# YannDubs/disentangling-vae

Measured on AMD Instinct MI355X. Metric: images/sec (whole node) at 64x64x3, btcvae loss, higher is better.
Workload: dtype f32; 1 GPU; btcvae_celeba (BASELINE.json configs[3]): Burgess VAE 64x64x3, btcvae loss, z=10, tensor handed to _train_iteration B=1024 global (1024 per GPU), Adam lr 0.0005, n_data=202599, fwd+loss+bwd+Adam; batch_per_gpu=1024, global_batch=1024, parallelism=dp1

## Files before the change

disentangling-vae_amd/csrc/capi.hip:

```cpp
#include <mutex>
#include <stdlib.h>
#include "common.h"
#include "last_error.h"

namespace dvae {

bool use_generic_only() {
  const char* e = getenv("DVAE_FORCE_GENERIC");
  return e && e[0] == '1';
}

static int check_layout(int l) { return l == DVAE_NCHW || l == DVAE_NHWC; }

static int run_down(const ConvArgs& a, hipStream_t s) {
  if (!use_generic_only()) {
    int r = launch_down_mfma32(a, s);
    if (r <= 0) return r;
    r = launch_down_thin(a, s);
    if (r <= 0) return r;
  }
  return launch_down_generic(a, s);
}
static int run_up(const ConvArgs& a, hipStream_t s) {
  if (!use_generic_only()) {
    int r = 1;
    static const bool no_ws = env_off("DVAE_UP_WS");
    if (!no_ws) {
      r = launch_up_mfma32_ws(a, s);
      if (r <= 0) return r;
    }
    r = launch_up_mfma32(a, s);
    if (r <= 0) return r;
    r = launch_up_thin(a, s);
    if (r <= 0) return r;
  }
  return launch_up_generic(a, s);
}
static int run_wgrad(const float* big, int big_layout, const float* small, int small_layout, float* dw, float* db,
                     int bias_from_big, int N, int Cb, int Cs, int Hs, int Ws, float* ws, hipStream_t s) {
  if (!use_generic_only() && ws != nullptr && Hs == Ws && Cs == 32 && Cb == 32 && big_layout == DVAE_NHWC && Hs == 4 &&
      small_layout == DVAE_NCHW)
    return launch_wgrad_mfma32(big, small, dw, db, bias_from_big, N, Hs, ws, s, 1);
  if (!use_generic_only() && ws != nullptr && Hs == Ws && Cs == 32 && small_layout == DVAE_NHWC) {
    if (Cb == 32 && big_layout == DVAE_NHWC && (Hs == 4 || Hs == 8 || Hs == 16))
      return launch_wgrad_mfma32(big, small, dw, db, bias_from_big, N, Hs, ws, s, 0);
    if ((Cb == 1 || Cb == 3) && Hs == 32 && big_layout == DVAE_NCHW)
      return launch_wgrad_thin(big, small, dw, db, bias_from_big, N, Cb, Hs, ws, s);
  }
  return launch_wgrad_generic(big, big_layout, small, small_layout, dw, db, bias_from_big, N, Cb, Cs, Hs, Ws, ws,
                              dvae_conv_wgrad_ws_floats(), s);
}

}

using namespace dvae;

extern "C" {

int dvae_version(void) { return DVAE_VERSION; }
const char* dvae_last_error(void) { return last_error(); }

int dvae_conv4s2_fwd(const float* x, int x_layout, const float* w, const float* b, float* y, int y_layout, int N,
                     int Cin, int H, int W, int Cout, int act, void* stream) {
  DVAE_CHECK_ARG(x && w && y && N > 0 && Cin > 0 && Cout > 0 && H > 0 && W > 0 && (H % 2 == 0) && (W % 2 == 0));
  DVAE_CHECK_ARG(check_layout(x_layout) && check_layout(y_layout));
  ConvArgs a{x, x_layout, nullptr, 0, w, b, nullptr, y, y_layout, N, Cin, Cout, H / 2, W / 2, act};
  return run_down(a, (hipStream_t)stream);
}

int dvae_conv4s2_dgrad(const float* dy, int dy_layout, const float* w, const float* x_act, float* dx, int dx_layout,
                       int N, int Cin, int H, int W, int Cout, void* stream) {
  DVAE_CHECK_ARG(dy && w && dx && N > 0 && Cin > 0 && Cout > 0 && (H % 2 == 0) && (W % 2 == 0));
  DVAE_CHECK_ARG(check_layout(dy_layout) && check_layout(dx_layout));
  ConvArgs a{nullptr, 0, dy, dy_layout, w, nullptr, x_act, dx, dx_layout, N, Cin, Cout, H / 2, W / 2, DVAE_ACT_NONE};
  return run_up(a, (hipStream_t)stream);
}

int dvae_conv4s2_wgrad(const float* x, int x_layout, const float* dy, int dy_layout, float* dw, float* db, int N,
                       int Cin, int H, int W, int Cout, float* ws, void* stream) {
  DVAE_CHECK_ARG(x && dy && dw && N > 0 && (H % 2 == 0) && (W % 2 == 0));
  const int rc = run_wgrad(x, x_layout, dy, dy_layout, dw, db, 0, N, Cin, Cout, H / 2, W / 2, ws,
                   (hipStream_t)stream);
  return rc;
}

int dvae_convT4s2_fwd(const float* x, int x_layout, const float* w, const float* b, float* y, int y_layout, int N,
                      int Cin, int H, int W, int Cout, int act, void* stream) {
  DVAE_CHECK_ARG(x && w && y && N > 0 && Cin > 0 && Cout > 0 && H > 0 && W > 0);
  DVAE_CHECK_ARG(check_layout(x_layout) && check_layout(y_layout));
  ConvArgs a{nullptr, 0, x, x_layout, w, b, nullptr, y, y_layout, N, Cout, Cin, H, W, act};
  return run_up(a, (hipStream_t)stream);
}

int dvae_convT4s2_dgrad(const float* dy, int dy_layout, const float* w, const float* x_act, float* dx, int dx_layout,
                        int N, int Cin, int H, int W, int Cout, void* stream) {
  DVAE_CHECK_ARG(dy && w && dx && N > 0 && Cin > 0 && Cout > 0);
  DVAE_CHECK_ARG(check_layout(dy_layout) && check_layout(dx_layout));
  ConvArgs a{dy, dy_layout, nullptr, 0, w, nullptr, x_act, dx, dx_layout, N, Cout, Cin, H, W, DVAE_ACT_NONE};
  return run_down(a, (hipStream_t)stream);
}

int dvae_convT4s2_wgrad(const float* x, int x_layout, const float* dy, int dy_layout, float* dw, float* db, int N,
                        int Cin, int H, int W, int Cout, float* ws, void* stream) {
  DVAE_CHECK_ARG(x && dy && dw && N > 0);
  const int rc = run_wgrad(dy, dy_layout, x, x_layout, dw, db, 1, N, Cout, Cin, H, W, ws,
                   (hipStream_t)stream);
  return rc;
}

int dvae_convT4s2_sigmoid_recon_fwd(const float* x, int x_layout, const float* w, const float* b, const float* target,
                                    float* recon, float* g, int dist, const float* coef, float* partials, int N,
                                    int Cin, int H, int W, int Cout, void* stream) {
  DVAE_CHECK_ARG(x && w && target && recon && g && coef && partials && N > 0 && Cin > 0 && Cout > 0 && H > 0 && W > 0);
  DVAE_CHECK_ARG(check_layout(x_layout));
  DVAE_CHECK_ARG(dist == DVAE_REC_BERNOULLI || dist == DVAE_REC_GAUSSIAN || dist == DVAE_REC_LAPLACE);
  ConvArgs a{nullptr, 0, x, x_layout, w, b, nullptr, recon, DVAE_NCHW, N, Cout, Cin, H, W, DVAE_ACT_SIGMOID};
  static const bool two_pass = env_on("DVAE_RECON_TWO_PASS");
  if (!use_generic_only() && !two_pass) {
    int r = launch_up_thin_recon(a, target, g, dist, coef, partials, (hipStream_t)stream);
    if (r <= 0) return r;
  }
  int r = run_up(a, (hipStream_t)stream);
  if (r) return r;
  const long n = (long)N * Cout * 4 * H * W;
  DVAE_CHECK_ARG(n % 4 == 0);
  return launch_recon_loss(recon, target, n, dist, coef, partials, g, 1, (hipStream_t)stream);
}

static bool u8_fused_shape(int C, int H, int W, int Cout) { return (C == 1 || C == 3) && H == 64 && W == 64 && Cout == 32; }

int dvae_u8_to_f32(const uint8_t* src, float* dst, long n, void* stream) {
  DVAE_CHECK_ARG(src && dst && n > 0 && (((uintptr_t)src & 15) == 0) && (((uintptr_t)dst & 15) == 0));
  return launch_u8_to_f32(src, dst, n, (hipStream_t)stream);
}

int dvae_image_grid_u8(const float* imgs, long n, int C, int H, int W, int nrow, int padding, float pad_value, int upsample,
                       uint8_t* out, void* stream) {
  DVAE_CHECK_ARG(imgs && out && n > 0 && (C == 1 || C == 3) && H > 0 && W > 0 && nrow > 0 && padding >= 0 && upsample >= 1);
  return launch_image_grid_u8(imgs, n, C, H, W, nrow, padding, pad_value, upsample, out, (hipStream_t)stream);
}

int dvae_image_grid_shape(long n, int H, int W, int nrow, int padding, int upsample, long* height, long* width) {
  DVAE_CHECK_ARG(height && width && n > 0 && H > 0 && W > 0 && nrow > 0 && padding >= 0 && upsample >= 1);
  long gh, gw;
  int xmaps, pad;
  if (image_grid_geom(n, H, W, nrow, padding, upsample, &gh, &gw, &xmaps, &pad) != 0) {
    set_error("dvae_image_grid_shape: grid of %ld images of %dx%d (nrow %d, padding %d, upsample %d) is too large", n, H, W,
              nrow, padding, upsample);
    return -1;
  }
  *height = gh;
  *width = gw;
  return 0;
}

int dvae_recon_rows_ws_floats(long n_img, int K, long row_elems, long* floats) {
  DVAE_CHECK_ARG(floats && n_img > 0 && K > 0 && row_elems > 0 && row_elems % 4 == 0);
  *floats = recon_rows_ws_floats(n_img, K, row_elems);
  return 0;
}

int dvae_recon_rows(const float* recon, const void* target, int target_u8, long n_img, int K, long row_elems, int dist,
                    float* ws, float* rec_rows, void* stream) {
  DVAE_CHECK_ARG(recon && target && rec_rows && n_img > 0 && K > 0 && row_elems > 0 && row_elems % 4 == 0);
  DVAE_CHECK_ARG(dist == DVAE_REC_BERNOULLI || dist == DVAE_REC_GAUSSIAN || dist == DVAE_REC_LAPLACE);
  DVAE_CHECK_ARG(((uintptr_t)recon & 15) == 0 && ((uintptr_t)target & (target_u8 ? 3 : 15)) == 0);
  return launch_recon_rows(recon, target, target_u8 ? 1 : 0, n_img, K, row_elems, dist, ws, rec_rows, (hipStream_t)stream);
}

int dvae_iw_loglik(const float* mu, const float* logvar, const float* z, const float* eps, const float* rec_rows, long n_img,
                   int nk, int D, int K, int first, int last, float* state, float* loglik, float* kl, void* stream) {
  DVAE_CHECK_ARG(mu && logvar && n_img > 0 && D > 0 && (state || kl));
  DVAE_CHECK_ARG(!state || (z && eps && rec_rows && nk > 0 && K >= nk && (!last || loglik)));
  return launch_iw_loglik(mu, logvar, z, eps, rec_rows, n_img, nk, D, K, first ? 1 : 0, last ? 1 : 0, state, loglik, kl,
                          (hipStream_t)stream);
}

int dvae_u8_fused_supported(int C, int H, int W) { return u8_fused_shape(C, H, W, 32) ? 1 : 0; }

int dvae_conv4s2_fwd_u8(const uint8_t* x, const float* w, const float* b, float* y, int N, int Cin, int H, int W,
                        int Cout, int act, void* stream) {
  DVAE_CHECK_ARG(x && w && y && N > 0);
  DVAE_CHECK_ARG(u8_fused_shape(Cin, H, W, Cout));
  DVAE_CHECK_ARG(act == DVAE_ACT_NONE || act == DVAE_ACT_RELU);
  return launch_down_thin_u8(x, w, b, y, nullptr, N, Cin, act, (hipStream_t)stream);
}

int dvae_conv4s2_wgrad_u8(const uint8_t* x, const float* dy, float* dw, float* db, int N, int Cin, int H, int W,
                          int Cout, float* ws, void* stream) {
  DVAE_CHECK_ARG(x && dy && dw && ws && N > 0);
  DVAE_CHECK_ARG(u8_fused_shape(Cin, H, W, Cout));
  return launch_wgrad_thin_u8(x, dy, dw, db, N, Cin, ws, (hipStream_t)stream);
}

int dvae_convT4s2_sigmoid_recon_fwd_u8(const float* x, const float* w, const float* b, const uint8_t* target,
                                       float* recon, float* g, int dist, const float* coef, float* partials, int N,
                                       int Cin, int H, int W, int Cout, void* stream) {
  DVAE_CHECK_ARG(x && w && target && recon && g && coef && partials && N > 0);
  DVAE_CHECK_ARG(Cin == 32 && u8_fused_shape(Cout, 2 * H, 2 * W, 32));
  DVAE_CHECK_ARG(dist == DVAE_REC_BERNOULLI || dist == DVAE_REC_GAUSSIAN || dist == DVAE_REC_LAPLACE);
  ConvArgs a{nullptr, 0, x, DVAE_NHWC, w, b, nullptr, recon, DVAE_NCHW, N, Cout, Cin, H, W, DVAE_ACT_SIGMOID};
  return launch_up_thin_recon_u8(a, target, g, dist, coef, partials, (hipStream_t)stream);
}

size_t dvae_conv_wgrad_ws_floats(void) {
  size_t a = wgrad32_ws_floats(), b = wgrad_thin_ws_floats();
  return a > b ? a : b;
}

int dvae_relayout(const float* src, int src_layout, float* dst, int N, int C, int H, int W, void* stream) {
  DVAE_CHECK_ARG(src && dst && check_layout(src_layout) && N > 0 && C > 0 && H > 0 && W > 0);
  return launch_relayout(src, src_layout, dst, N, C, H, W, (hipStream_t)stream);
}

int dvae_linear_fwd(const float* x, const float* w, const float* b, float* y, int M, int K, int N, int act, float* ws,
                    void* stream) {
  DVAE_CHECK_ARG(x && w && y && M > 0 && K > 0 && N > 0);
  DVAE_CHECK_ARG(act == DVAE_ACT_NONE || act == DVAE_ACT_RELU || act == DVAE_ACT_LEAKY02);
  return launch_linear_fwd(x, w, b, y, M, K, N, act, ws, dvae_conv_wgrad_ws_floats(), (hipStream_t)stream);
}

int dvae_linear_dgrad(const float* dy, const float* w, const float* x_act, int act, float* dx, int M, int K, int N,
                      float* ws, void* stream) {
  DVAE_CHECK_ARG(dy && w && dx && M > 0 && K > 0 && N > 0);
  return launch_linear_dgrad(dy, w, x_act, act, dx, M, K, N, ws, dvae_conv_wgrad_ws_floats(), (hipStream_t)stream);
}

int dvae_linear_wgrad(const float* x, const float* dy, float* dw, float* db, int M, int K, int N, float* ws,
                      void* stream) {
  DVAE_CHECK_ARG(x && dy && dw && M > 0 && K > 0 && N > 0);
  return launch_linear_wgrad(x, dy, dw, db, M, K, N, ws, dvae_conv_wgrad_ws_floats(), (hipStream_t)stream);
}

int dvae_linear_wgrad_grouped(const dvae_linear_wgrad_desc* descs, int n, void* stream) {
  DVAE_CHECK_ARG(descs && n >= 1 && n <= DVAE_FCW_MAX);
  for (int q = 0; q < n; ++q)
    DVAE_CHECK_ARG(descs[q].x && descs[q].dy && descs[q].dw && descs[q].M > 0 && descs[q].K > 0 && descs[q].N > 0);
  return launch_linear_wgrad_grouped(descs, n, (hipStream_t)stream);
}

size_t dvae_latent_entropy_ws_floats(long N, int D, int S) {
  if (N <= 0 || D <= 0 || S <= 0) return 0;
  return latent_entropy_ws_floats(N, D, S);
}

int dvae_latent_entropy(const float* z_ds, const float* mean, const float* logvar, long N, int D, int S, float* ws,
                        float* H, void* stream) {
  DVAE_CHECK_ARG(z_ds && mean && logvar && ws && H && N > 0 && D > 0 && D <= 65535 && S > 0);
  return launch_latent_entropy(z_ds, mean, logvar, N, D, S, ws, H, (hipStream_t)stream);
}

int dvae_reparam_kl_fwd(const float* ml, const float* eps, float* mu, float* logvar, float* z, float* kl_dim,
                        const float* coef, int B, int D, void* stream) {
  DVAE_CHECK_ARG(ml && mu && logvar && z && B > 0 && D > 0);
  DVAE_CHECK_ARG(D <= DVAE_MAX_D || ((!kl_dim || coef) && D <= DVAE_KL_FLOATS));
  return launch_reparam_kl_fwd(ml, eps, mu, logvar, z, kl_dim, coef, B, D, (hipStream_t)stream);
}

int dvae_reparam_kl_bwd(const float* dz, const float* dz2, const float* dz3, const float* dmu_x, const float* dlv_x,
                        const float* mu, const float* logvar, const float* eps, const float* scal, const float* coef,
                        float* dml, int B, int D, void* stream) {
  DVAE_CHECK_ARG(mu && logvar && scal && coef && dml && B > 0 && D > 0);
  return launch_reparam_kl_bwd(dz, dz2, dz3, dmu_x, dlv_x, mu, logvar, eps, scal, coef, dml, B, D, (hipStream_t)stream);
}

int dvae_kl_normal_bwd(const float* g_dim, const float* mu, const float* logvar, float* dmu, float* dlogvar, int B, int D,
                       void* stream) {
  DVAE_CHECK_ARG(g_dim && mu && logvar && dmu && dlogvar && B > 0 && D > 0);
  return launch_kl_normal_bwd(g_dim, mu, logvar, dmu, dlogvar, B, D, (hipStream_t)stream);
}

int dvae_reduce_sum(const float* src, long n, float scale, float* dst, void* stream) {
  DVAE_CHECK_ARG(src && dst && n > 0);
  return launch_reduce_sum(src, n, scale, dst, (hipStream_t)stream);
}

int dvae_recon_loss(const float* recon, const float* target, long n, int dist, const float* coef, float* partials,
                    float* g, int wrt_logit, void* stream) {
  DVAE_CHECK_ARG(recon && target && coef && partials && n > 0 && (n % 4 == 0));
  DVAE_CHECK_ARG(dist == DVAE_REC_BERNOULLI || dist == DVAE_REC_GAUSSIAN || dist == DVAE_REC_LAPLACE);
  return launch_recon_loss(recon, target, n, dist, coef, partials, g, wrt_logit, (hipStream_t)stream);
}

int dvae_sigmoid_bwd(const float* grad_y, const float* y, float* out, long n, void* stream) {
  DVAE_CHECK_ARG(grad_y && y && out && n > 0);
  return launch_sigmoid_bwd(grad_y, y, out, n, (hipStream_t)stream);
}

int dvae_btcvae_fwd(const float* z, const float* mu, const float* logvar, int Bg, int D, int row0, int Bl, int is_mss,
                    const float* log_w, float* tmp, float* rowstats, void* stream) {
  DVAE_CHECK_ARG(z && mu && logvar && tmp && rowstats && Bg > 1 && D >= 1 && row0 >= 0 && Bl > 0 && row0 + Bl <= Bg);
  DVAE_CHECK_ARG(D <= DVAE_WIDE_MAX_D );
  DVAE_CHECK_ARG(!is_mss || log_w);
  return launch_btcvae_fwd(z, mu, logvar, Bg, D, row0, Bl, is_mss, log_w, tmp, rowstats, (hipStream_t)stream);
}

int dvae_btcvae_bwd(const float* z, const float* mu, const float* logvar, const float* rowstats, int Bg, int D,
                    int row0, int Bl, int is_mss, const float* log_w, const float* coef, const float* tmp, float* dz,
                    float* dmu_all, float* dlv_all, void* stream) {
  DVAE_CHECK_ARG(z && mu && logvar && rowstats && coef && tmp && dz && dmu_all && dlv_all && Bg > 1 && D >= 1);
  DVAE_CHECK_ARG(D <= DVAE_WIDE_MAX_D );
  DVAE_CHECK_ARG(row0 >= 0 && Bl > 0 && row0 + Bl <= Bg && (!is_mss || log_w));
  return launch_btcvae_bwd(z, mu, logvar, rowstats, Bg, D, row0, Bl, is_mss, log_w, coef, tmp, dz, dmu_all, dlv_all,
                           (hipStream_t)stream);
}

int dvae_permute_dims(const float* z, const int64_t* perm, float* out, int B, int D, void* stream) {
  DVAE_CHECK_ARG(z && perm && out && B > 0 && D > 0);
  return launch_permute_dims(z, perm, out, B, D, (hipStream_t)stream);
}

int dvae_disc_losses(const float* dlogits, int Bh, const float* coef, float* sums, float* g_dtc, float* g_tc,
                     void* stream) {
  DVAE_CHECK_ARG(dlogits && coef && sums && g_dtc && Bh > 0);
  return launch_disc_losses(dlogits, Bh, coef, sums, g_dtc, g_tc, (hipStream_t)stream);
}

int dvae_loss_pack(const float* rec_partials, const float* kl_dim, int D, const float* rowstats, int Bl,
                   const float* disc_sums, float* packed, void* stream) {
  DVAE_CHECK_ARG(rec_partials && packed && D >= 0);
  return launch_loss_pack(rec_partials, kl_dim, D, rowstats, Bl, disc_sums, packed, (hipStream_t)stream);
}

int dvae_loss_epilogue(int kind, const float* rec_partials, const float* kl_dim, int kl_blocks, int D, const float* rowstats,
                       int Bl, const float* disc_sums, int Bg, const float* coef, float* packed, float* scal,
                       void* stream) {
  DVAE_CHECK_ARG(rec_partials && packed && coef && D >= 0 && Bl >= 0 && Bg > 0);
  DVAE_CHECK_ARG(kl_blocks >= 0 && kl_blocks <= DVAE_KL_MAX_BLOCKS && (D <= DVAE_MAX_D || kl_blocks == 0));
  DVAE_CHECK_ARG(kind >= DVAE_LOSS_BETAH && kind <= DVAE_LOSS_FACTOR);
  return launch_loss_epilogue(kind, rec_partials, kl_dim, kl_blocks, D, rowstats, Bl, disc_sums, Bg, coef, packed, scal,
                              (hipStream_t)stream);
}

int dvae_reparam_kl_blocks(int B) { return B > 0 ? reparam_kl_blocks(B) : 0; }

int dvae_kl_finish(float* kl_dim, int kl_blocks, const float* coef, int D, void* stream) {
  DVAE_CHECK_ARG(kl_dim && coef && kl_blocks > 0 && kl_blocks <= DVAE_KL_MAX_BLOCKS && D > 0 && D <= DVAE_MAX_D);
  return launch_kl_finish(kl_dim, kl_blocks, coef, D, (hipStream_t)stream);
}

int dvae_stage_weights(const dvae_conv_image_desc* conv, int n_conv, const dvae_fc_image_desc* fc, int n_fc,
                       const dvae_thin_image_desc* thin, float* coef, const float* coef_vals, void* stream) {
  DVAE_CHECK_ARG(n_conv >= 0 && n_conv <= DVAE_STAGE_MAX_CONV && n_fc >= 0 && n_fc <= DVAE_STAGE_MAX_FC);
  DVAE_CHECK_ARG((n_conv == 0 || conv) && (n_fc == 0 || fc));
  for (int q = 0; q < n_conv; ++q) DVAE_CHECK_ARG(conv[q].w);
  for (int q = 0; q < n_fc; ++q) DVAE_CHECK_ARG(fc[q].w && fc[q].N > 0 && fc[q].K > 0);
  if (thin) DVAE_CHECK_ARG(thin->w && (thin->C == 1 || thin->C == 3));
  return launch_stage_weights(conv, n_conv, fc, n_fc, thin, coef, coef_vals, (hipStream_t)stream);
}

int dvae_convT3_fwd_staged(const float* x, const float* img_pairs, const float* b, const void* target, int target_is_u8,
                           float* recon, float* g, int dist, const float* coef, float* partials, int N, int C,
                           void* stream) {
  DVAE_CHECK_ARG(x && img_pairs && recon && N > 0 && (C == 1 || C == 3));
  if (target) {
    DVAE_CHECK_ARG(g && coef && partials);
    DVAE_CHECK_ARG(dist == DVAE_REC_BERNOULLI || dist == DVAE_REC_GAUSSIAN || dist == DVAE_REC_LAPLACE);
  }
  return launch_up_thin_staged(x, img_pairs, b, target, target_is_u8, recon, g, dist, coef, partials, N, C, DVAE_ACT_SIGMOID,
                               (hipStream_t)stream);
}

int dvae_conv32_down(const float* big, const float* img_down, const float* bias, const float* mask, float* out,
                     int out_layout, int N, int Hs, int act, void* stream) {
  DVAE_CHECK_ARG(big && img_down && out && N > 0 && (Hs == 4 || Hs == 8 || Hs == 16) && check_layout(out_layout));
  DVAE_CHECK_ARG(out_layout == DVAE_NHWC || Hs == 4);
  DVAE_CHECK_ARG(act == DVAE_ACT_NONE || act == DVAE_ACT_RELU);
  ConvArgs a{big, DVAE_NHWC, nullptr, 0, img_down, bias, mask, out, out_layout, N, 32, 32, Hs, Hs, act, 1};
  const int r = launch_down_mfma32(a, (hipStream_t)stream);
  if (r > 0) { set_error("dvae_conv32_down: geometry not covered"); return -1; }
  return r;
}

int dvae_conv32_up(const float* small, int small_layout, const float* img_up, const float* bias, const float* mask,
                   float* out, int N, int Hs, int act, void* stream) {
  DVAE_CHECK_ARG(small && img_up && out && N > 0 && (Hs == 4 || Hs == 8 || Hs == 16) && check_layout(small_layout));
  DVAE_CHECK_ARG(small_layout == DVAE_NHWC || Hs == 4);
  DVAE_CHECK_ARG(act == DVAE_ACT_NONE || act == DVAE_ACT_RELU);
  ConvArgs a{nullptr, 0, small, small_layout, img_up, bias, mask, out, DVAE_NHWC, N, 32, 32, Hs, Hs, act, 1};
  int r = launch_up_mfma32_ws(a, (hipStream_t)stream);
  if (r > 0) r = launch_up_mfma32(a, (hipStream_t)stream);
  if (r > 0) { set_error("dvae_conv32_up: geometry not covered"); return -1; }
  return r;
}

int dvae_conv1_fwd_bits(const void* x, int x_is_u8, const float* w, const float* b, float* y, uint32_t* y_bits, int N,
                        int Cin, void* stream) {
  DVAE_CHECK_ARG(x && w && y && y_bits && N > 0 && (Cin == 1 || Cin == 3));
  if (x_is_u8) return launch_down_thin_u8((const uint8_t*)x, w, b, y, y_bits, N, Cin, DVAE_ACT_RELU, (hipStream_t)stream);
  ConvArgs a{(const float*)x, DVAE_NCHW, nullptr, 0, w, b, nullptr, y, DVAE_NHWC, N, Cin, 32, 32, 32, DVAE_ACT_RELU, 0};
  a.out_bits = y_bits;
  const int r = launch_down_thin(a, (hipStream_t)stream);
  if (r > 0) { set_error("dvae_conv1_fwd_bits: geometry not covered"); return -1; }
  return r;
}

int dvae_conv32_up_bits(const float* small, const float* img_up, const float* bias, const uint32_t* mask_bits, float* out,
                        uint32_t* out_bits, int N, int act, void* stream) {
  DVAE_CHECK_ARG(small && img_up && out && N > 0 && (mask_bits != nullptr) != (out_bits != nullptr));
  DVAE_CHECK_ARG(act == DVAE_ACT_NONE || act == DVAE_ACT_RELU);
  DVAE_CHECK_ARG(!out_bits || act == DVAE_ACT_RELU);
  ConvArgs a{nullptr, 0, small, DVAE_NHWC, img_up, bias, nullptr, out, DVAE_NHWC, N, 32, 32, 16, 16, act, 1};
  a.mask_bits = mask_bits;
  a.out_bits = out_bits;
  const int r = launch_up_mfma32_ws(a, (hipStream_t)stream);
  if (r > 0) { set_error("dvae_conv32_up_bits: geometry not covered"); return -1; }
  return r;
}

int dvae_convT3_dgrad_bits(const float* dy, const float* w, const uint32_t* x_act_bits, float* dx, int N, int Cout,
                           void* stream) {
  DVAE_CHECK_ARG(dy && w && x_act_bits && dx && N > 0 && (Cout == 1 || Cout == 3));
  ConvArgs a{dy, DVAE_NCHW, nullptr, 0, w, nullptr, nullptr, dx, DVAE_NHWC, N, Cout, 32, 32, 32, DVAE_ACT_NONE, 0};
  a.mask_bits = x_act_bits;
  const int r = launch_down_thin(a, (hipStream_t)stream);
  if (r > 0) { set_error("dvae_convT3_dgrad_bits: geometry not covered"); return -1; }
  return r;
}

int dvae_fc_chain_fwd(const dvae_fc_chain_fwd_args* a, void* stream) {
  DVAE_CHECK_ARG(a && a->a_flat && a->w_e1 && a->w_e2 && a->w_ml && a->b_e1 && a->b_e2 && a->b_ml);
  DVAE_CHECK_ARG(a->h1 && a->h2 && a->ml && a->mu && a->logvar && a->z);
  DVAE_CHECK_ARG(a->D >= 1 && a->D <= DVAE_MAX_D && a->n_enc > 0 && a->n_enc <= 8 * DVAE_KL_MAX_BLOCKS);
  DVAE_CHECK_ARG(a->n_kl >= 0 && a->n_kl <= a->n_enc && a->n_dec >= 0 && a->n_dec <= a->n_enc);
  if (a->n_dec > 0) DVAE_CHECK_ARG(a->w_d1 && a->w_d2 && a->w_d3 && a->b_d1 && a->b_d2 && a->b_d3 && a->d1 && a->d2 && a->d3);
  if (a->conv_in) DVAE_CHECK_ARG(a->conv_w && a->conv_b && ((((uintptr_t)a->conv_in | (uintptr_t)a->conv_w) & 15) == 0));
  if (a->convT_w) DVAE_CHECK_ARG(a->conv_in && a->convT_b && a->convT_out && a->n_dec > 0 && (((uintptr_t)a->convT_w & 15) == 0));
  return launch_fc_chain_fwd(a, (hipStream_t)stream);
}

int dvae_fc_chain_rows(int n) { return fc_chain_rows(n); }

int dvae_fc_chain_bwd(const dvae_fc_chain_bwd_args* a, void* stream) {
  DVAE_CHECK_ARG(a && a->gd3 && a->w_d3 && a->w_d2 && a->w_d1 && a->w_ml && a->w_e2 && a->w_e1);
  DVAE_CHECK_ARG(a->d2 && a->d1 && a->h2 && a->h1 && a->a_flat && a->mu && a->logvar && a->scal && a->coef);
  DVAE_CHECK_ARG(a->gd2 && a->gd1 && a->dml && a->gh2 && a->gh1 && a->ga_flat);
  DVAE_CHECK_ARG(a->D >= 1 && a->D <= DVAE_MAX_D && a->n > 0);
  if (a->convT_gout) DVAE_CHECK_ARG(a->convT_w && a->d3 && ((((uintptr_t)a->convT_gout | (uintptr_t)a->convT_w) & 15) == 0));
  if (a->conv_w) DVAE_CHECK_ARG(a->convT_gout && a->conv_act && a->conv_gin && (((uintptr_t)a->conv_w & 15) == 0));
  return launch_fc_chain_bwd(a, (hipStream_t)stream);
}

int dvae_loss_finalize(int kind, const float* packed, int D, int Bg, const float* coef, float* scal, void* stream) {
  DVAE_CHECK_ARG(packed && coef && scal && D >= 0 && Bg > 0);
  DVAE_CHECK_ARG(kind >= DVAE_LOSS_BETAH && kind <= DVAE_LOSS_FACTOR);
  return launch_loss_finalize(kind, packed, D, Bg, coef, scal, (hipStream_t)stream);
}

int dvae_set_coef(float* coef, float c0, float c1, float c2, float c3, float c4, float c5, float c6, float c7,
                  void* stream) {
  DVAE_CHECK_ARG(coef);
  const float v[8] = {c0, c1, c2, c3, c4, c5, c6, c7};
  return launch_set_coef(coef, v, (hipStream_t)stream);
}

int dvae_stream_create(void** stream) {
  DVAE_CHECK_ARG(stream);
  hipStream_t s = nullptr;
  if (hipStreamCreateWithFlags(&s, hipStreamNonBlocking) != hipSuccess) {
    set_error("dvae_stream_create: %s", hipGetErrorString(hipGetLastError()));
    return -2;
  }
  *stream = (void*)s;
  return 0;
}

int dvae_stream_order(void* earlier, void* later) {
  constexpr int NEV = 256, NDEV = 32;
  static hipEvent_t pool[NDEV][NEV];
  static int made[NDEV] = {}, next[NDEV] = {};
  static std::mutex mu;
  std::lock_guard<std::mutex> lock(mu);
  int d = 0;
  if (hipGetDevice(&d) != hipSuccess || d < 0 || d >= NDEV) { set_error("dvae_stream_order: no current device"); return -2; }
  if (!made[d]) {
    for (int k = 0; k < NEV; ++k)
      if (hipEventCreateWithFlags(&pool[d][k], hipEventDisableTiming | hipEventReleaseToDevice) != hipSuccess) {
        set_error("dvae_stream_order: hipEventCreateWithFlags failed");
        return -2;
      }
    made[d] = 1;
  }
  hipEvent_t ev = pool[d][next[d]];
  next[d] = (next[d] + 1) % NEV;
  if (hipEventRecord(ev, (hipStream_t)earlier) != hipSuccess || hipStreamWaitEvent((hipStream_t)later, ev, 0) != hipSuccess) {
    set_error("dvae_stream_order: %s", hipGetErrorString(hipGetLastError()));
    return -2;
  }
  return 0;
}

static hipEvent_t* event_slot(int slot, const char* who) {
  constexpr int NDEV = 32;
  static hipEvent_t pool[NDEV][DVAE_EVENT_SLOTS];
  static int made[NDEV] = {};
  static std::mutex mu;
  std::lock_guard<std::mutex> lock(mu);
  int d = 0;
  if (hipGetDevice(&d) != hipSuccess || d < 0 || d >= NDEV) { set_error("%s: no current device", who); return nullptr; }
  if (slot < 0 || slot >= DVAE_EVENT_SLOTS) { set_error("%s: slot %d outside [0, %d)", who, slot, DVAE_EVENT_SLOTS); return nullptr; }
  if (!made[d]) {
    for (int k = 0; k < DVAE_EVENT_SLOTS; ++k)
      if (hipEventCreateWithFlags(&pool[d][k], hipEventDisableTiming | hipEventReleaseToDevice) != hipSuccess) {
        set_error("%s: hipEventCreateWithFlags failed", who);
        return nullptr;
      }
    made[d] = 1;
  }
  return &pool[d][slot];
}

int dvae_event_record(int slot, void* stream) {
  hipEvent_t* ev = event_slot(slot, "dvae_event_record");
  if (!ev) return -2;
  if (hipEventRecord(*ev, (hipStream_t)stream) != hipSuccess) { set_error("dvae_event_record: %s", hipGetErrorString(hipGetLastError())); return -2; }
  return 0;
}

int dvae_event_wait(int slot, void* stream) {
  hipEvent_t* ev = event_slot(slot, "dvae_event_wait");
  if (!ev) return -2;
  if (hipStreamWaitEvent((hipStream_t)stream, *ev, 0) != hipSuccess) { set_error("dvae_event_wait: %s", hipGetErrorString(hipGetLastError())); return -2; }
  return 0;
}

int dvae_add(const float* a, const float* b, float* out, long n, void* stream) {
  DVAE_CHECK_ARG(a && b && out && n > 0);
  return launch_add(a, b, out, n, (hipStream_t)stream);
}

int dvae_adam_step(const dvae_adam_tensor* tensors, int nt, float step_new, double lr, double beta1, double beta2,
                   double eps, double weight_decay, void* stream) {
  DVAE_CHECK_ARG(tensors && nt > 0 && step_new >= 1.f && lr >= 0. && beta1 >= 0. && beta1 < 1. && beta2 >= 0. && beta2 < 1.);
  DVAE_CHECK_ARG(eps >= 0. && weight_decay >= 0.);
  for (int i = 0; i < nt; ++i) DVAE_CHECK_ARG(tensors[i].p && tensors[i].g && tensors[i].m && tensors[i].v && tensors[i].n >= 0);
  return launch_adam(tensors, nt, step_new, lr, beta1, beta2, eps, weight_decay, (hipStream_t)stream);
}

int dvae_axpby(float* out, const float* a, float alpha, const float* b, float beta, long n, void* stream) {
  DVAE_CHECK_ARG(out && a && n > 0);
  return launch_axpby(out, a, alpha, b, beta, n, (hipStream_t)stream);
}

int dvae_swap_outer(const float* src, float* dst, int A, int Bn, long inner, void* stream) {
  DVAE_CHECK_ARG(src && dst && src != dst && A > 0 && Bn > 0 && inner > 0 && inner < (1L << 31) && (long)A * Bn < (1L << 31));
  return launch_swap_outer(src, dst, A, Bn, inner, (hipStream_t)stream);
}

}
```

disentangling-vae_amd/csrc/common.h:

```cpp
#pragma once
#include <hip/hip_runtime.h>
#include <stdint.h>
#include <stdio.h>
#include <stdlib.h>
#include <string.h>
#include "../../include/dvae_hip.h"
#include "wave_spec.h"

namespace dvae {

void set_error(const char* fmt, ...);

#define DVAE_CHECK_ARG(cond)                                                            \
  do {                                                                                  \
    if (!(cond)) {                                                                      \
      dvae::set_error("%s:%d: invalid argument: %s", __FILE__, __LINE__, #cond);        \
      return -1;                                                                        \
    }                                                                                   \
  } while (0)

#define DVAE_CHECK_LAUNCH()                                                             \
  do {                                                                                  \
    hipError_t e__ = hipGetLastError();                                                 \
    if (e__ != hipSuccess) {                                                            \
      dvae::set_error("%s:%d: launch failed: %s", __FILE__, __LINE__,                   \
                      hipGetErrorString(e__));                                          \
      return -2;                                                                        \
    }                                                                                   \
  } while (0)

struct Strides {
  long n, c, h, w;
};
static inline Strides make_strides(int layout, int C, int H, int W) {
  Strides s;
  if (layout == DVAE_NHWC) {
    s.n = (long)H * W * C; s.h = (long)W * C; s.w = C; s.c = 1;
  } else {
    s.n = (long)C * H * W; s.c = (long)H * W; s.h = W; s.w = 1;
  }
  return s;
}

struct DeviceOnce {
  bool done[32] = {};
  bool first() {
    int d = 0;
    if (hipGetDevice(&d) != hipSuccess || d < 0 || d >= 32) return true;
    if (done[d]) return false;
    done[d] = true;
    return true;
  }
};

typedef float f32x4 __attribute__((ext_vector_type(4)));
typedef float f32x16 __attribute__((ext_vector_type(16)));

__device__ __forceinline__ float wave_sum(float v) {
#pragma unroll
  for (int o = 32; o > 0; o >>= 1) v += __shfl_xor(v, o, 64);
  return v;
}
__device__ __forceinline__ float wave_max(float v) {
#pragma unroll
  for (int o = 32; o > 0; o >>= 1) v = fmaxf(v, __shfl_xor(v, o, 64));
  return v;
}

__device__ __forceinline__ float recon_elem(float p, float x, int dist, float* gl, float* gr) {
  const float q1 = 1.f - p;
  const float qq = q1 * p;
  float term;
  if (dist == DVAE_REC_BERNOULLI) {
    const float lp = p < 1e-30f ? logf(p) : __logf(p);
    term = (x - 1.f) * fmaxf(__logf(q1), -100.f) - x * fmaxf(lp, -100.f);
    const float d = p - x;
    *gl = qq >= 1e-12f ? d : d * 1e12f * qq;
    *gr = d / fmaxf(qq, 1e-12f);
  } else if (dist == DVAE_REC_GAUSSIAN) {
    const float d = p * 255.f - x * 255.f;
    term = d * d / 255.f;
    *gr = 2.f * d;
    *gl = *gr * qq;
  } else {
    const float d = p - x;
    term = 3.f * fabsf(d);
    *gr = d > 0.f ? 3.f : (d < 0.f ? -3.f : 0.f);
    *gl = *gr * qq;
  }
  return term;
}

#define DVAE_SIGMOID_ZERO_BELOW (-88.72283935546875f)
__device__ __forceinline__ float sigmoid_aten(float v) {
  const float e = __expf(-fabsf(v));
  const float s = 1.f + e;
  const float r = __builtin_amdgcn_rcpf(s);
  float p = v >= 0.f ? fmaf(1.f - s, r, 1.f) : e * r;
  if (v < -87.f)
    p = v < DVAE_SIGMOID_ZERO_BELOW ? 0.f : ldexpf(__expf(v + 17.328679513998633f), -25);
  return p;
}

__device__ __forceinline__ float sigmoid_bce_logit(float v, float x, float* p_out, float* gl) {
  const float e = __expf(-fabsf(v));
  const float s = 1.f + e;
  const float r = __builtin_amdgcn_rcpf(s);
  const float q = s - 1.f;
  const bool pos = v >= 0.f, zero = v < DVAE_SIGMOID_ZERO_BELOW;
  float p = pos ? fmaf(-q, r, 1.f) : e * r;
  if (__builtin_expect(v < -87.f, 0))
    p = zero ? 0.f : ldexpf(__expf(v + 17.328679513998633f), -25);
  const float ls = fmaf(__builtin_amdgcn_logf(s), 0.69314718056f, (e - q) * r);
  const float om = 1.f - p;
  const float l1 = fminf(__builtin_amdgcn_logf(om) * -0.69314718056f, 100.f);
  const float t0 = pos ? l1 : ls;
  const float dx = pos ? ls - l1 : (zero ? 100.f : -v);
  const float qq = om * p, d = p - x;
  *gl = qq >= 1e-12f ? d : d * 1e12f * qq;
  *p_out = p;
  return fmaf(x, dx, t0);
}

struct ConvArgs {
  const float* big; int big_layout;
  const float* small; int small_layout;
  const float* w; const float* bias; const float* mask;
  float* out; int out_layout;
  int N, Cb, Cs, Hs, Ws;
  int act;
  int w_staged;
  const uint32_t* mask_bits = nullptr;
  uint32_t* out_bits = nullptr;
};
int launch_down_generic(const ConvArgs& a, hipStream_t s);
int launch_up_generic(const ConvArgs& a, hipStream_t s);
int launch_wgrad_generic(const float* big, int big_layout, const float* small, int small_layout,
                         float* dw, float* db, int bias_from_big, int N, int Cb, int Cs, int Hs, int Ws, float* ws,
                         size_t ws_floats, hipStream_t s);
int launch_down_mfma32(const ConvArgs& a, hipStream_t s);
int launch_up_mfma32(const ConvArgs& a, hipStream_t s);
int launch_down_mfma32_dma(const ConvArgs& a, hipStream_t s);
int launch_wgrad_mfma32_ws(const float* big, const float* small, float* dw, float* db, int bias_from_big, int N, int Hs,
                           float* ws, hipStream_t s);
int launch_wgrad32_reduce(const float* ws, float* dw, float* db, int bias_from_big, int nblk, hipStream_t s, int N);
int launch_up_mfma32_ws(const ConvArgs& a, hipStream_t s);
int launch_wgrad_mfma32(const float* big, const float* small, float* dw, float* db, int bias_from_big,
                        int N, int Hs, float* ws, hipStream_t s, int small_nchw = 0);
int launch_down_thin(const ConvArgs& a, hipStream_t s);
int launch_down_thin_ws(const ConvArgs& a, hipStream_t s);
int launch_up_thin(const ConvArgs& a, hipStream_t s);
int launch_up_thin_recon(const ConvArgs& a, const float* target, float* g, int dist, const float* coef,
                         float* partials, hipStream_t s);
int launch_wgrad_thin_ws(const float* big, const float* small, float* ws, int bias_from_big, int N, int Cb, int* grid_out,
                         hipStream_t s);
int launch_wgrad_thin(const float* big, const float* small, float* dw, float* db, int bias_from_big,
                      int N, int Cb, int Hs, float* ws, hipStream_t s);
int launch_down_thin_u8(const uint8_t* x, const float* w, const float* bias, float* out, uint32_t* out_bits, int N, int C, int act,
                        hipStream_t s);
int launch_up_thin_recon_u8(const ConvArgs& a, const uint8_t* target, float* g, int dist, const float* coef,
                            float* partials, hipStream_t s);
int launch_wgrad_thin_u8(const uint8_t* x, const float* small, float* dw, float* db, int N, int C, float* ws, hipStream_t s);
int launch_kl_normal_bwd(const float* g, const float* mu, const float* lv, float* dmu, float* dlv, int B, int D, hipStream_t s);
int launch_reduce_sum(const float* src, long n, float scale, float* dst, hipStream_t s);
int launch_u8_to_f32(const uint8_t* src, float* dst, long n, hipStream_t s);
int image_grid_geom(long n, int H, int W, int nrow, int padding, int upsample, long* gh, long* gw, int* xmaps, int* pad);
int launch_image_grid_u8(const float* imgs, long n, int C, int H, int W, int nrow, int padding, float pad_value, int upsample,
                         uint8_t* out, hipStream_t s);
long recon_rows_ws_floats(long n_img, int K, long row_elems);
int launch_recon_rows(const float* recon, const void* target, int target_u8, long n_img, int K, long row_elems, int dist,
                      float* ws, float* rec_rows, hipStream_t s);
int launch_iw_loglik(const float* mu, const float* logvar, const float* z, const float* eps, const float* rec_rows, long n_img,
                     int nk, int D, int K, int first, int last, float* state, float* loglik, float* kl, hipStream_t s);

size_t wgrad32_ws_floats();
size_t wgrad_thin_ws_floats();
int launch_relayout(const float* src, int src_layout, float* dst, int N, int C, int H, int W, hipStream_t s);

int launch_linear_fwd(const float* x, const float* w, const float* b, float* y, int M, int K, int N, int act, float* ws,
                      size_t ws_floats, hipStream_t s);
int launch_linear_dgrad(const float* dy, const float* w, const float* x_act, int act, float* dx, int M, int K, int N,
                        float* ws, size_t ws_floats, hipStream_t s);
int launch_linear_wgrad(const float* x, const float* dy, float* dw, float* db, int M, int K, int N, float* ws,
                        size_t ws_floats, hipStream_t s);

bool try_gdma(bool b_jfast, const float* a, long lda, const float* b, long ldb, float* c, long ldc, int M, int N, int Kc,
              const float* bias, int act, const float* mask, int mask_act, hipStream_t s);
bool try_gdma_wgrad(const float* x, const float* dy, float* dw, float* db, int M, int K, int N, hipStream_t s);

bool try_narrow_fwd(const float* x, const float* w, const float* b, float* y, int M, int K, int N, int act, hipStream_t s);
bool try_narrow_dgrad(const float* dy, const float* w, const float* x_act, int act, float* dx, int M, int K, int N,
                      hipStream_t s);

size_t latent_entropy_ws_floats(long N, int D, int S);
int launch_latent_entropy(const float* z_ds, const float* mean, const float* logvar, long N, int D, int S, float* ws,
                          float* H, hipStream_t s);
int launch_linear_wgrad_grouped(const dvae_linear_wgrad_desc* d, int n, hipStream_t s);
int fc_chain_rows(int n);
int launch_fc_chain_fwd(const dvae_fc_chain_fwd_args* a, hipStream_t s);
int launch_fc_chain_bwd(const dvae_fc_chain_bwd_args* a, hipStream_t s);
int reparam_kl_blocks(int B);
int launch_kl_finish(float* kl_dim, int kl_blocks, const float* coef, int D, hipStream_t s);
int launch_stage_weights(const dvae_conv_image_desc* conv, int n_conv, const dvae_fc_image_desc* fc, int n_fc,
                         const dvae_thin_image_desc* thin, float* coef, const float* coef_vals, hipStream_t s);
static __host__ __device__ __forceinline__ int thin_pair_source(int idx, int C, int* cb) {
  const int taps[16] = {5, 6, 9, 10, 13, 14, 1, 2, 7, 11, 4, 8, 0, 3, 12, 15};
  if (C == 3 && idx < 32) {
    const int a = idx >> 1, t = a >> 2, cls = a & 3;
    const int py = cls >> 1, px = cls & 1, ty = t >> 1, tx = t & 1;
    *cb = idx & 1;
    return (1 - py + 2 * ty) * 4 + (1 - px + 2 * tx);
  }
  *cb = C - 1;
  return taps[C == 3 ? idx - 32 : idx];
}
int launch_up_thin_mm(const float* small, const float* wimg, const float* bias, const void* target, int target_u8, float* out,
                      float* g, int dist, const float* coef, float* partials, int N, int act, hipStream_t s);
int launch_up_thin_staged(const float* small, const float* wrec, const float* bias, const void* target, int target_u8,
                          float* out, float* g, int dist, const float* coef, float* partials, int N, int C, int act,
                          hipStream_t s);

int launch_reparam_kl_fwd(const float* ml, const float* eps, float* mu, float* logvar, float* z, float* kl_dim,
                          const float* coef, int B, int D, hipStream_t s);
int launch_reparam_kl_bwd(const float* dz, const float* dz2, const float* dz3, const float* dmu_x, const float* dlv_x, const float* mu, const float* logvar,
                          const float* eps, const float* scal, const float* coef, float* dml, int B, int D,
                          hipStream_t s);
int launch_recon_loss(const float* recon, const float* target, long n, int dist, const float* coef, float* partials,
                      float* g, int wrt_logit, hipStream_t s);
int launch_sigmoid_bwd(const float* gy, const float* y, float* out, long n, hipStream_t s);
int launch_btcvae_fwd(const float* z, const float* mu, const float* lv, int Bg, int D, int row0, int Bl, int is_mss,
                      const float* log_w, float* tmp, float* rowstats, hipStream_t s);
int launch_btcvae_bwd(const float* z, const float* mu, const float* lv, const float* rowstats, int Bg, int D, int row0,
                      int Bl, int is_mss, const float* log_w, const float* coef, const float* tmp, float* dz, float* dmu,
                      float* dlv, hipStream_t s);
int launch_reparam_kl_fwd_wide(const float* ml, const float* eps, float* mu, float* logvar, float* z, float* kl_dim,
                               const float* coef, int B, int D, hipStream_t s);
int launch_btcvae_fwd_wide(const float* z, const float* mu, const float* lv, int Bg, int D, int row0, int Bl, int is_mss,
                           const float* log_w, float* tmp, float* rowstats, hipStream_t s);
int launch_btcvae_bwd_wide(const float* z, const float* mu, const float* lv, const float* rowstats, int Bg, int D, int row0,
                           int Bl, int is_mss, const float* log_w, const float* coef, const float* tmp, float* dz, float* dmu,
                           float* dlv, hipStream_t s);
int launch_permute_dims(const float* z, const int64_t* perm, float* out, int B, int D, hipStream_t s);
int launch_disc_losses(const float* lg, int Bh, const float* coef, float* sums, float* g_dtc, float* g_tc,
                       hipStream_t s);
int launch_loss_pack(const float* rec_partials, const float* kl_dim, int D, const float* rowstats, int Bl,
                     const float* disc_sums, float* packed, hipStream_t s);
int launch_loss_finalize(int kind, const float* packed, int D, int Bg, const float* coef, float* scal, hipStream_t s);
int launch_loss_epilogue(int kind, const float* rec_partials, const float* kl_dim, int kl_blocks, int D, const float* rowstats,
                         int Bl, const float* disc_sums, int Bg, const float* coef, float* packed, float* scal,
                         hipStream_t s);
int launch_set_coef(float* coef, const float* v, hipStream_t s);
int launch_adam(const dvae_adam_tensor* ts, int nt, float step_new, double lr, double beta1, double beta2, double eps,
                double weight_decay, hipStream_t s);
int launch_add(const float* a, const float* b, float* out, long n, hipStream_t s);
int launch_axpby(float* out, const float* a, float alpha, const float* b, float beta, long n, hipStream_t s);
int launch_swap_outer(const float* src, float* dst, int A, int Bn, long inner, hipStream_t s);

bool use_generic_only();

#ifdef DVAE_DEBUG_SWITCHES
static inline bool env_on(const char* name) { const char* e = getenv(name); return e && e[0] == '1' && e[1] == 0; }
static inline bool env_off(const char* name) { const char* e = getenv(name); return e && e[0] == '0' && e[1] == 0; }
static inline int env_int(const char* name, int dflt) { const char* e = getenv(name); return e ? atoi(e) : dflt; }
#else
static inline constexpr bool env_on(const char*) { return false; }
static inline constexpr bool env_off(const char*) { return false; }
static inline constexpr int env_int(const char*, int dflt) { return dflt; }
#endif

}

#include "latent_math.h"
```

disentangling-vae_amd/csrc/conv_mfma.hip:

```cpp
#include <stdlib.h>
#include "common.h"
#include "conv_mfma_common.h"
#include "wgrad_reduce.h"

namespace dvae {

typedef float f32x4v __attribute__((ext_vector_type(4)));

#define SEL4(v, g, j) ((g) == 0 ? (v)[j] : (g) == 1 ? (v)[4 + (j)] : (g) == 2 ? (v)[8 + (j)] : (v)[12 + (j)])
template <int HS, bool MASK>
__global__ __launch_bounds__(512) void k_down32(const float* __restrict__ big, const float* __restrict__ w,
                                                const float* __restrict__ bias, const float* __restrict__ mask,
                                                float* __restrict__ out, int N, int act, int n_units,
                                                int out_nchw, int w_staged) {
  using G = Geo<HS>;
  extern __shared__ __attribute__((aligned(16))) float smem[];
  float* wl = smem;
  float* bt = smem + 16384;
  float* red = bt + G::BIG_FLOATS;
  const int tid = threadIdx.x, lane = tid & 63, wv = tid >> 6;
  const int mt = wv & 1, kh = wv >> 1;
  const int i = lane & 31, h = lane >> 5;
  const int p = mt * 32 + i;
  const int img_l = p / (G::R * HS), sy_l = (p / HS) % G::R, sx = p % HS;
  const int r = 2 * sy_l + kh;

  SlotDesc<G::BIG_NPF> sd;
  init_big_slots<HS>(sd, tid);
  f32x4 pf[G::BIG_NPF];
  int unit = blockIdx.x;
  if (unit < n_units) load_big<HS>(pf, sd, big, unit, N);
  if (w_staged) copy_weight_image(w, wl, tid);
  else stage_weights<true>(w, wl, tid);
  const float bv = bias ? bias[i] : 0.f;
  const long npix = (long)N * HS * HS;

  for (; unit < n_units; unit += gridDim.x) {
    store_big<HS>(pf, sd, bt);
    __syncthreads();
    if (unit + (int)gridDim.x < n_units) load_big<HS>(pf, sd, big, unit + gridDim.x, N);

    f32x16 acc;
#pragma unroll
    for (int e = 0; e < 16; ++e) acc[e] = 0.f;
#pragma unroll
    for (int kw = 0; kw < 4; ++kw) {
      const int par = kw & 1, cw = sx + (kw >> 1);
      const float* arow = bt + (((img_l * G::BROWS + r) * 2 + par) * G::CW + cw) * 32;
      const int sw = swz_big<HS>(r, cw);
      const float* brow = wl + ((kh * 4 + kw) * 8) * 128 + i * 4;
#pragma unroll
      for (int q = 0; q < 4; ++q) {
        const int chunk = 2 * q + h;
        f32x4 a = *reinterpret_cast<const f32x4*>(arow + ((chunk ^ sw) << 2));
        f32x4 b = *reinterpret_cast<const f32x4*>(brow + chunk * 128);
        MFMA4(acc, a, b)
      }
    }
#pragma unroll
    for (int e = 0; e < 16; ++e) red[(((mt * 4 + (e >> 2)) * 4 + kh) * 4 + (e & 3)) * 64 + lane] = acc[e];
    __syncthreads();
    const long P0 = (long)unit * G::U + mt * 32 + 8 * kh + 4 * h;
    auto oidx = [&](long pix) -> long {
      constexpr int PP = HS * HS;
      return out_nchw ? ((pix / PP) * 32 + i) * PP + (pix % PP) : pix * 32 + i;
    };
    float vals[4], mv[4];
#pragma unroll
    for (int j = 0; j < 4; ++j) {
      float v = SEL4(acc, kh, j);
#pragma unroll
      for (int s = 0; s < 4; ++s)
        if (s != kh) v += red[(((mt * 4 + kh) * 4 + s) * 4 + j) * 64 + lane];
      vals[j] = v;
    }
    const bool full = P0 - 4 * h - 8 * kh - mt * 32 + G::U <= npix;
    if (full) {
      if (MASK) {
#pragma unroll
        for (int j = 0; j < 4; ++j) mv[j] = mask[oidx(P0 + j)];
      }
#pragma unroll
      for (int j = 0; j < 4; ++j) {
        float v = epilogue_act(vals[j] + bv, act);
        if (MASK) v = mv[j] > 0.f ? v : 0.f;
        out[oidx(P0 + j)] = v;
      }
    } else {
#pragma unroll
      for (int j = 0; j < 4; ++j) {
        const long pix = P0 + j;
        if (pix < npix) {
          float v = epilogue_act(vals[j] + bv, act);
          if (MASK) v = mask[oidx(pix)] > 0.f ? v : 0.f;
          out[oidx(pix)] = v;
        }
      }
    }
  }
}


template <int HS>
__device__ __forceinline__ void up_offsets(long (&offs)[16], int unit, int mt, int py, int px, int h, int i) {
  using G = Geo<HS>;
  const long P0 = (long)unit * G::U;
  const int n0 = (int)(P0 / (HS * HS));
  const int sy0 = (int)(P0 % (HS * HS)) / HS;
#pragma unroll
  for (int e = 0; e < 16; ++e) {
    const int rowp = (e & 3) + 8 * (e >> 2) + 4 * h;
    const int pp = mt * 32 + rowp;
    const int im = pp / (G::R * HS), mm = (pp / HS) % G::R, ll = pp % HS;
    const int by = 2 * (sy0 + mm) + py, bx = 2 * ll + px;
    offs[e] = (((long)(n0 + im) * G::HB + by) * G::HB + bx) * 32 + i;
  }
}

template <int HS>
__device__ __forceinline__ void up_store(const float (&vals)[16], float* __restrict__ out, int unit, int N, int mt,
                                         int py, int px, int h, int i) {
  using G = Geo<HS>;
  long offs[16];
  up_offsets<HS>(offs, unit, mt, py, px, h, i);
  const int n0 = (int)(((long)unit * G::U) / (HS * HS));
  if (n0 + G::IMGS <= N) {
#pragma unroll
    for (int e = 0; e < 16; ++e) out[offs[e]] = vals[e];
  } else {
#pragma unroll
    for (int e = 0; e < 16; ++e) {
      const int im = (mt * 32 + (e & 3) + 8 * (e >> 2) + 4 * h) / (G::R * HS);
      if (n0 + im < N) out[offs[e]] = vals[e];
    }
  }
}

template <int HS, bool MASK>
__global__ __launch_bounds__(512) void k_up32(const float* __restrict__ small, const float* __restrict__ w,
                                              const float* __restrict__ bias, const float* __restrict__ mask,
                                              float* __restrict__ out, int N, int act, int n_units,
                                              int small_nchw, int w_staged) {
  using G = Geo<HS>;
  extern __shared__ __attribute__((aligned(16))) float smem[];
  float* wl = smem;
  float* st = smem + 16384;
  const int tid = threadIdx.x, lane = tid & 63, wv = tid >> 6;
  const int cls = wv & 3, mt = wv >> 2;
  const int py = cls >> 1, px = cls & 1;
  const int i = lane & 31, h = lane >> 5;
  const int p = mt * 32 + i;
  const int img_l = p / (G::R * HS), m = (p / HS) % G::R, l = p % HS;

  SlotDesc<G::SH_NPF> sd;
  init_small_slots<HS>(sd, tid, small_nchw);
  f32x4 pf[G::SH_NPF];
  int unit = blockIdx.x;
  if (unit < n_units) load_small_halo<HS>(pf, sd, small, unit, N, small_nchw);
  if (w_staged) copy_weight_image(w, wl, tid);
  else stage_weights<false>(w, wl, tid);
  const float bv = bias ? bias[i] : 0.f;
  float vals[16];
  int prev_unit = -1;

  for (; unit < n_units; unit += gridDim.x) {
    __syncthreads();
    store_small_halo<HS>(pf, sd, st);
    __syncthreads();
    if (unit + (int)gridDim.x < n_units) load_small_halo<HS>(pf, sd, small, unit + gridDim.x, N, small_nchw);
    float mv[16];
    if (MASK) {
      long offs[16];
      up_offsets<HS>(offs, unit, mt, py, px, h, i);
      const int n0 = (int)(((long)unit * G::U) / (HS * HS));
#pragma unroll
      for (int e = 0; e < 16; ++e) {
        const int im = (mt * 32 + (e & 3) + 8 * (e >> 2) + 4 * h) / (G::R * HS);
        mv[e] = (G::IMGS == 1 || n0 + im < N) ? mask[offs[e]] : 0.f;
      }
    }
    if (prev_unit >= 0) up_store<HS>(vals, out, prev_unit, N, mt, py, px, h, i);

    f32x16 accs[4];
#pragma unroll
    for (int c = 0; c < 4; ++c)
#pragma unroll
      for (int e = 0; e < 16; ++e) accs[c][e] = 0.f;
    f32x4 Av[2], Bv[2];
    auto rd = [&](int g, int slot) {
      const int ty = g >> 3, tx = (g >> 2) & 1, q = g & 3;
      const int kh = 1 - py + 2 * ty, kw = 1 - px + 2 * tx;
      const int row = m + (py - ty) + 1, col = l + (px - tx) + 1;
      const float* arow = st + ((img_l * G::SROWS + row) * G::SCOLS + col) * 32;
      const int sw = swz_small<HS>(row, col);
      const float* brow = wl + ((kh * 4 + kw) * 8) * 128 + i * 4;
      const int chunk = 2 * q + h;
      Av[slot] = *reinterpret_cast<const f32x4*>(arow + ((chunk ^ sw) << 2));
      Bv[slot] = *reinterpret_cast<const f32x4*>(brow + chunk * 128);
    };
    rd(0, 0);
    __builtin_amdgcn_sched_group_barrier(0x100, 2, 0);
#pragma unroll
    for (int g = 0; g < 16; ++g) {
      const int cur = g & 1;
      if (g + 1 < 16) rd(g + 1, cur ^ 1);
#pragma unroll
      for (int j = 0; j < 4; ++j) accs[j] = __builtin_amdgcn_mfma_f32_32x32x2f32(Av[cur][j], Bv[cur][j], accs[j], 0, 0, 0);
      __builtin_amdgcn_sched_group_barrier(0x100, 2, 0);
      __builtin_amdgcn_sched_group_barrier(0x008, 4, 0);
    }
    const f32x16 acc = (accs[0] + accs[1]) + (accs[2] + accs[3]);
#pragma unroll
    for (int e = 0; e < 16; ++e) {
      float v = epilogue_act(acc[e] + bv, act);
      if (MASK) v = mv[e] > 0.f ? v : 0.f;
      vals[e] = v;
    }
    prev_unit = unit;
  }
  if (prev_unit >= 0) up_store<HS>(vals, out, prev_unit, N, mt, py, px, h, i);
}

template <int HS>
__global__ __launch_bounds__(512) void k_wgrad32(const float* __restrict__ big, const float* __restrict__ small,
                                                 float* __restrict__ ws, int N, int n_units, int small_nchw) {
  using G = Geo<HS>;
  extern __shared__ __attribute__((aligned(16))) float smem[];
  float* bt = smem;
  float* sp = smem + G::BIG_FLOATS;
  const int tid = threadIdx.x, lane = tid & 63, wv = tid >> 6;
  const int kh = wv >> 1, kwb = wv & 1;
  const int i = lane & 31, h = lane >> 5;

  SlotDesc<G::BIG_NPF> sd;
  init_big_slots<HS>(sd, tid);
  f32x4 pf[G::BIG_NPF];
  f32x4 pfs;
  f32x16 acc0, acc1, acc2, acc3;
#pragma unroll
  for (int e = 0; e < 16; ++e) { acc0[e] = 0.f; acc1[e] = 0.f; acc2[e] = 0.f; acc3[e] = 0.f; }
  float sumS = 0.f, sumB0 = 0.f, sumB1 = 0.f;

  int unit = blockIdx.x;
  const long npix = (long)N * HS * HS;
  auto load_sp = [&](int u) {
    long e0 = (long)u * G::U * 32 + tid * 4;
    f32x4 v = {0.f, 0.f, 0.f, 0.f};
    if (e0 < npix * 32) {
      if (small_nchw) {
        const long pg = e0 >> 5;
        const float* src = small + ((pg / (HS * HS)) * 32 + (e0 & 31)) * (HS * HS) + pg % (HS * HS);
#pragma unroll
        for (int u2 = 0; u2 < 4; ++u2) v[u2] = src[u2 * HS * HS];
      } else {
        v = *reinterpret_cast<const f32x4*>(small + e0);
      }
    }
    pfs = v;
  };
  if (unit < n_units) { load_big<HS>(pf, sd, big, unit, N); load_sp(unit); }

  for (; unit < n_units; unit += gridDim.x) {
    __syncthreads();
    store_big<HS>(pf, sd, bt);
    *reinterpret_cast<f32x4*>(sp + tid * 4) = pfs;
    __syncthreads();
    if (unit + (int)gridDim.x < n_units) { load_big<HS>(pf, sd, big, unit + gridDim.x, N); load_sp(unit + gridDim.x); }

    float av[2][2], b0v[2][2], b1v[2][2];
    auto rd = [&](int g, int slot) {
#pragma unroll
      for (int u = 0; u < 2; ++u) {
        const int p = 2 * (2 * g + u) + h;
        const int img_l = p / (G::R * HS), sy_l = (p / HS) % G::R, sx = p % HS;
        av[slot][u] = sp[p * 32 + i];
        const int r = 2 * sy_l + kh;
        const int cw = sx + kwb;
        const float* b0p = bt + (((img_l * G::BROWS + r) * 2 + 0) * G::CW + cw) * 32;
        const int sw = swz_big<HS>(r, cw);
        const int off = (((i >> 2) ^ sw) << 2) + (i & 3);
        b0v[slot][u] = b0p[off];
        b1v[slot][u] = b0p[G::CW * 32 + off];
      }
    };
    rd(0, 0);
    __builtin_amdgcn_sched_group_barrier(0x100, 6, 0);
#pragma unroll
    for (int g = 0; g < 16; ++g) {
      const int cur = g & 1;
      if (g + 1 < 16) rd(g + 1, cur ^ 1);
      acc0 = __builtin_amdgcn_mfma_f32_32x32x2f32(av[cur][0], b0v[cur][0], acc0, 0, 0, 0);
      acc1 = __builtin_amdgcn_mfma_f32_32x32x2f32(av[cur][0], b1v[cur][0], acc1, 0, 0, 0);
      acc2 = __builtin_amdgcn_mfma_f32_32x32x2f32(av[cur][1], b0v[cur][1], acc2, 0, 0, 0);
      acc3 = __builtin_amdgcn_mfma_f32_32x32x2f32(av[cur][1], b1v[cur][1], acc3, 0, 0, 0);
      sumS += av[cur][0] + av[cur][1]; sumB0 += b0v[cur][0] + b0v[cur][1]; sumB1 += b1v[cur][0] + b1v[cur][1];
      __builtin_amdgcn_sched_group_barrier(0x100, 6, 0);
      __builtin_amdgcn_sched_group_barrier(0x008, 4, 0);
    }
  }
  acc0 += acc2; acc1 += acc3;
  float* wsw = ws + (long)blockIdx.x * WG_STRIDE;
  const int tap0 = kh * 4 + 2 * kwb;
#pragma unroll
  for (int e = 0; e < 16; ++e) {
    const int cs = (e & 3) + 8 * (e >> 2) + 4 * h;
    wsw[(tap0 * 32 + cs) * 32 + i] = acc0[e];
    wsw[((tap0 + 1) * 32 + cs) * 32 + i] = acc1[e];
  }
  float* wsb = wsw + 16384;
  sumS += __shfl_xor(sumS, 32, 64);
  sumB0 += __shfl_xor(sumB0, 32, 64);
  sumB1 += __shfl_xor(sumB1, 32, 64);
  if (h == 0) {
    if (wv == 0) wsb[i] = sumS;
    if (wv == 2) wsb[32 + i] = sumB1;
    if (wv == 3) wsb[64 + i] = sumB0;
    if (wv == 4) wsb[96 + i] = sumB1;
    if (wv == 5) wsb[128 + i] = sumB0;
  }
}

template <bool LEAN>
__global__ __launch_bounds__(256) void k_wgrad32_reduce(const float* __restrict__ ws, float* __restrict__ dw,
                                                        float* __restrict__ db, int bias_from_big, int nblk) {
  wgrad32_reduce_body<LEAN>(blockIdx.x, ws, dw, db, bias_from_big, nblk);
}

size_t wgrad32_ws_floats() { return (size_t)WG_MAX_BLOCKS * WG_STRIDE; }

int launch_wgrad32_reduce(const float* ws, float* dw, float* db, int bias_from_big, int nblk, hipStream_t s, int N) {
  if (N >= WGR_LEAN_MIN_IMAGES)
    hipLaunchKernelGGL(k_wgrad32_reduce<true>, dim3(WG_REDUCE_BLOCKS), dim3(256), 0, s, ws, dw, db, bias_from_big, nblk);
  else
    hipLaunchKernelGGL(k_wgrad32_reduce<false>, dim3(WG_REDUCE_BLOCKS), dim3(256), 0, s, ws, dw, db, bias_from_big, nblk);
  DVAE_CHECK_LAUNCH();
  return 0;
}

static int units_for(int N, int HS) { return (int)(((long)N * HS * HS + 63) / 64); }

template <int HS>
static int launch_down_t(const ConvArgs& a, hipStream_t s) {
  using G = Geo<HS>;
  const int n_units = units_for(a.N, HS);
  const int grid = n_units < 256 ? n_units : 256;
  const size_t lds = (16384 + G::BIG_FLOATS + 8192) * sizeof(float);
  static DeviceOnce attr;
  if (attr.first()) {
    (void)hipFuncSetAttribute((const void*)k_down32<HS, false>, hipFuncAttributeMaxDynamicSharedMemorySize, (int)lds);
    (void)hipFuncSetAttribute((const void*)k_down32<HS, true>, hipFuncAttributeMaxDynamicSharedMemorySize, (int)lds);
  }
  const int out_nchw = a.out_layout == DVAE_NCHW;
  if (a.mask) hipLaunchKernelGGL((k_down32<HS, true>), dim3(grid), dim3(512), lds, s, a.big, a.w, a.bias, a.mask, a.out, a.N, a.act, n_units, out_nchw, a.w_staged);
  else hipLaunchKernelGGL((k_down32<HS, false>), dim3(grid), dim3(512), lds, s, a.big, a.w, a.bias, a.mask, a.out, a.N, a.act, n_units, out_nchw, a.w_staged);
  DVAE_CHECK_LAUNCH();
  return 0;
}

template <int HS>
static int launch_up_t(const ConvArgs& a, hipStream_t s) {
  using G = Geo<HS>;
  const int n_units = units_for(a.N, HS);
  const int grid = n_units < 256 ? n_units : 256;
  const size_t lds = (16384 + G::SH_FLOATS) * sizeof(float);
  static DeviceOnce attr;
  if (attr.first()) {
    (void)hipFuncSetAttribute((const void*)k_up32<HS, false>, hipFuncAttributeMaxDynamicSharedMemorySize, (int)lds);
    (void)hipFuncSetAttribute((const void*)k_up32<HS, true>, hipFuncAttributeMaxDynamicSharedMemorySize, (int)lds);
  }
  const int small_nchw = a.small_layout == DVAE_NCHW;
  if (a.mask) hipLaunchKernelGGL((k_up32<HS, true>), dim3(grid), dim3(512), lds, s, a.small, a.w, a.bias, a.mask, a.out, a.N, a.act, n_units, small_nchw, a.w_staged);
  else hipLaunchKernelGGL((k_up32<HS, false>), dim3(grid), dim3(512), lds, s, a.small, a.w, a.bias, a.mask, a.out, a.N, a.act, n_units, small_nchw, a.w_staged);
  DVAE_CHECK_LAUNCH();
  return 0;
}

template <int HS>
static int launch_wgrad_t(const float* big, const float* small, float* dw, float* db, int bias_from_big, int N,
                          float* ws, hipStream_t s, int small_nchw) {
  using G = Geo<HS>;
  const int n_units = units_for(N, HS);
  int grid = n_units < WG_MAX_BLOCKS ? n_units : WG_MAX_BLOCKS;
  {
    static const int cap = env_int("DVAE_WGRAD_GRID", WG_MAX_BLOCKS);
    if (cap > 0 && cap < grid) grid = cap;
  }
  const size_t lds = (G::BIG_FLOATS + 64 * 32) * sizeof(float);
  static DeviceOnce attr;
  if (attr.first()) { (void)hipFuncSetAttribute((const void*)k_wgrad32<HS>, hipFuncAttributeMaxDynamicSharedMemorySize, (int)lds); }
  hipLaunchKernelGGL(k_wgrad32<HS>, dim3(grid), dim3(512), lds, s, big, small, ws, N, n_units, small_nchw);
  DVAE_CHECK_LAUNCH();
  return launch_wgrad32_reduce(ws, dw, db, bias_from_big, grid, s, N);
}

static bool mfma32_applicable(int Cb, int Cs, int Hs, int Ws, int l0, int l1, int l2) {
  return Cb == 32 && Cs == 32 && Hs == Ws && (Hs == 4 || Hs == 8 || Hs == 16) && l0 == DVAE_NHWC &&
         l1 == DVAE_NHWC && l2 == DVAE_NHWC;
}

int launch_down_mfma32(const ConvArgs& a, hipStream_t s) {
  const int out_l = (a.Hs == 4 && a.out_layout == DVAE_NCHW) ? DVAE_NHWC : a.out_layout;
  if (!mfma32_applicable(a.Cb, a.Cs, a.Hs, a.Ws, a.big_layout, out_l, DVAE_NHWC)) return 1;
  if (a.act != DVAE_ACT_NONE && a.act != DVAE_ACT_RELU) return 1;
  if (a.Hs == 16 || a.Hs == 8) return launch_down_mfma32_dma(a, s);
  return launch_down_t<4>(a, s);
}

int launch_up_mfma32(const ConvArgs& a, hipStream_t s) {
  const int small_l = (a.Hs == 4 && a.small_layout == DVAE_NCHW) ? DVAE_NHWC : a.small_layout;
  if (!mfma32_applicable(a.Cb, a.Cs, a.Hs, a.Ws, small_l, a.out_layout, DVAE_NHWC)) return 1;
  if (a.act != DVAE_ACT_NONE && a.act != DVAE_ACT_RELU) return 1;
  switch (a.Hs) {
    case 16: return launch_up_t<16>(a, s);
    case 8: return launch_up_t<8>(a, s);
    default: return launch_up_t<4>(a, s);
  }
}

int launch_wgrad_mfma32(const float* big, const float* small, float* dw, float* db, int bias_from_big, int N,
                        int Hs, float* ws, hipStream_t s, int small_nchw) {
  static const bool no_ws = env_off("DVAE_WGRAD_WS");
  if (!no_ws && !small_nchw && (Hs == 16 || Hs == 8))
    return launch_wgrad_mfma32_ws(big, small, dw, db, bias_from_big, N, Hs, ws, s);
  switch (Hs) {
    case 16: return launch_wgrad_t<16>(big, small, dw, db, bias_from_big, N, ws, s, small_nchw);
    case 8: return launch_wgrad_t<8>(big, small, dw, db, bias_from_big, N, ws, s, small_nchw);
    case 4: return launch_wgrad_t<4>(big, small, dw, db, bias_from_big, N, ws, s, small_nchw);
    default: return 1;
  }
}

}
```

disentangling-vae_amd/csrc/conv_thin.hip:

```cpp
#include <stdlib.h>
#include "recon_epilogue.h"
#include "wgrad_reduce.h"

namespace dvae {

#define TB_ROWS 10
#define TB_PAR 34
#define TB_ROW 68
#define TB_PLANE (TB_ROWS * TB_ROW + 16)

template <int C, typename TB = float>
struct BigThinRegs {
  TB v[(C * TB_ROWS + 3) / 4];
  unsigned ok;
};

struct UnitLut {
  float t[256];
  __device__ __forceinline__ void init(int tid, int nthr) {
    for (int k = tid; k < 256; k += nthr) t[k] = (float)k / 255.0f;
  }
};
__device__ __forceinline__ float to_unit(float v, const UnitLut*) { return v; }
__device__ __forceinline__ float to_unit(uint8_t v, const UnitLut* lut) { return lut->t[v]; }

template <int C, typename TB>
__device__ __forceinline__ void load_big_thin(BigThinRegs<C, TB>& r, const TB* __restrict__ big, int n, int sy0,
                                              bool valid, int tid) {
  const int tx = tid & 63, ty = tid >> 6;
  unsigned okm = 0;
#pragma unroll
  for (int k = 0; k < (C * TB_ROWS + 3) / 4; ++k) {
    const int pr = ty + 4 * k;
    const int cb = pr / TB_ROWS, rr = pr - cb * TB_ROWS;
    const int by = 2 * sy0 - 1 + rr;
    const bool ok = valid && pr < C * TB_ROWS && by >= 0 && by < 64;
    const long off = ok ? ((((long)n * C + cb) * 64 + by) * 64 + tx) : 0;
    r.v[k] = big[off];
    okm |= ok ? (1u << k) : 0u;
  }
  r.ok = okm;
}

template <int C, typename TB>
__device__ __forceinline__ void store_big_thin(const BigThinRegs<C, TB>& r, float* bt, int tid, const UnitLut* lut) {
  const int tx = tid & 63, ty = tid >> 6;
  const int pc = tx + 1;
  const int dst_col = (pc & 1) * TB_PAR + (pc >> 1);
#pragma unroll
  for (int k = 0; k < (C * TB_ROWS + 3) / 4; ++k) {
    const int pr = ty + 4 * k;
    if (pr < C * TB_ROWS) {
      const int cb = pr / TB_ROWS, rr = pr - cb * TB_ROWS;
      bt[cb * TB_PLANE + rr * TB_ROW + dst_col] = ((r.ok >> k) & 1u) ? to_unit(r.v[k], lut) : 0.f;
    }
  }
  if (tid < C * TB_ROWS * 2) {
    const int pr = tid >> 1, side = tid & 1;
    const int cb = pr / TB_ROWS, rr = pr - cb * TB_ROWS;
    bt[cb * TB_PLANE + rr * TB_ROW + (side ? (TB_PAR + 32) : 0)] = 0.f;
  }
}

template <int C, int MODE, typename TB = float>
__global__ __launch_bounds__(256, (MODE == 1 && C == 3) ? 3 : 4) void k_down_thin(const TB* __restrict__ big, const float* __restrict__ w,
                                                   const float* __restrict__ bias, const float* __restrict__ mask,
                                                   float* __restrict__ out, int N, int act, int n_units,
                                                   uint32_t* __restrict__ bits) {
  constexpr bool MASK = MODE == 1;
  __shared__ float bt[C * TB_PLANE];
  __shared__ float wT[16 * C * 32];
  __shared__ UnitLut lut_s[1];
  const UnitLut* lut = lut_s;
  const int tid = threadIdx.x, lane = tid & 63, wv = tid >> 6;
  const int i = lane & 31, h = lane >> 5;
  if (sizeof(TB) == 1) { lut_s[0].init(tid, 256); __syncthreads(); }
  {
    float wv[2 * C];
#pragma unroll
    for (int r = 0; r < 2 * C; ++r) wv[r] = w[tid + r * 256];
#pragma unroll
    for (int r = 0; r < 2 * C; ++r) {
      const int e = tid + r * 256;
      const int cs = e / (16 * C), k = e - cs * (16 * C);
      wT[k * 32 + cs] = wv[r];
    }
  }
  BigThinRegs<C, TB> pfa, pfb;
  int unit = blockIdx.x;
  const int gstep = gridDim.x;
  if (unit < n_units) load_big_thin<C, TB>(pfa, big, unit >> 3, (unit & 7) * 4, true, tid);
  if (unit + gstep < n_units) load_big_thin<C, TB>(pfb, big, (unit + gstep) >> 3, ((unit + gstep) & 7) * 4, true, tid);
  __syncthreads();
  float wreg[8 * C];
#pragma unroll
  for (int kk = 0; kk < 8 * C; ++kk) wreg[kk] = wT[(2 * kk + h) * 32 + i];
  const float bv = bias ? bias[i] : 0.f;
  const int sy_l = wv;

  auto body = [&](BigThinRegs<C, TB>& pf, int u) {
    const int n = u >> 3, sy0 = (u & 7) * 4;
    __syncthreads();
    store_big_thin<C, TB>(pf, bt, tid, lut);
    __syncthreads();
    const int nu = u + 2 * gstep;
    if (nu < n_units) load_big_thin<C, TB>(pf, big, nu >> 3, (nu & 7) * 4, true, tid);
    const long rowbase = ((((long)n * 32 + sy0 + sy_l) * 32)) * 32 + i;
    float mv[16];
    if (MASK) {
#pragma unroll
      for (int e = 0; e < 16; ++e) mv[e] = mask[rowbase + ((e & 3) + 8 * (e >> 2) + 4 * h) * 32];
    }
    const long pixbase = ((long)n * 32 + sy0 + sy_l) * 32;
    uint32_t word = 0;
    if (MODE == 2) word = bits[pixbase + i];
    f32x16 acc;
#pragma unroll
    for (int e = 0; e < 16; ++e) acc[e] = 0.f;
#pragma unroll
    for (int kk = 0; kk < 8 * C; ++kk) {
      const int kwb = (kk & 1);
      const int kh = (kk >> 1) & 3, cb = kk >> 3;
      const float a = bt[cb * TB_PLANE + (2 * sy_l + kh) * TB_ROW + h * TB_PAR + i + kwb];
      acc = __builtin_amdgcn_mfma_f32_32x32x2f32(a, wreg[kk], acc, 0, 0, 0);
    }
#pragma unroll
    for (int e = 0; e < 16; ++e) {
      const int sx0 = (e & 3) + 8 * (e >> 2);
      const int sx = sx0 + 4 * h;
      float v = acc[e] + bv;
      if (act == DVAE_ACT_RELU) v = v > 0.f ? v : 0.f;
      if (MASK) v = mv[e] > 0.f ? v : 0.f;
      if (MODE == 2) {
        const unsigned long long m = ((unsigned long long)(uint32_t)__builtin_amdgcn_readlane(word, sx0 + 4) << 32) |
                                     (uint32_t)__builtin_amdgcn_readlane(word, sx0);
        v = __builtin_amdgcn_inverse_ballot_w64(m) ? v : 0.f;
      }
      if (MODE == 3) {
        const unsigned long long b = __builtin_amdgcn_ballot_w64(v > 0.f);
        word = __builtin_amdgcn_inverse_ballot_w64(0x0000000100000001ull << sx0) ? (uint32_t)b : word;
        word = __builtin_amdgcn_inverse_ballot_w64(0x0000000100000001ull << (sx0 + 4)) ? (uint32_t)(b >> 32) : word;
      }
      out[rowbase + sx * 32] = v;
    }
    if (MODE == 3 && h == 0) bits[pixbase + i] = word;
  };
  while (unit < n_units) {
    body(pfa, unit);
    unit += gstep;
    if (unit >= n_units) break;
    body(pfb, unit);
    unit += gstep;
  }
}

#define UT_ROWS 6
#define UT_COLS 34
template <int C, bool FUSE, typename TT = float>
__global__ __launch_bounds__(128) void k_up_thin(const float* __restrict__ small, const float* __restrict__ w,
                                                 const float* __restrict__ bias, float* __restrict__ out, int N,
                                                 int act, int n_units, const TT* __restrict__ target,
                                                 float* __restrict__ g, int dist, const float* __restrict__ coef,
                                                 float* __restrict__ partials) {
  __shared__ __attribute__((aligned(16))) float st[UT_ROWS * UT_COLS * 32];
  __shared__ float redl[2];
  const int tid = threadIdx.x;
  const int m = tid >> 5, l = tid & 31;
  const float gs = FUSE ? coef[DVAE_C_INV_B] : 0.f;
  float lsum = 0.f;
  const bool xmap = (gridDim.x & 63) == 0;
  const int upi = xmap ? 8 * (int)(gridDim.x >> 3) : (int)gridDim.x;
  const int unit0 = xmap ? 8 * (int)((blockIdx.x & 7) + 8 * (blockIdx.x >> 6)) + (int)((blockIdx.x >> 3) & 7) : (int)blockIdx.x;
  for (int unit = unit0; unit < n_units; unit += upi) {
    const int n = unit >> 3, sy0 = (unit & 7) * 4;
    __syncthreads();
    {
      const int chunk = tid & 7, cg = tid >> 3;
      f32x4 tv[UT_ROWS * 3];
#pragma unroll
      for (int row = 0; row < UT_ROWS; ++row) {
        const int sy = sy0 - 1 + row;
#pragma unroll
        for (int cp = 0; cp < 3; ++cp) {
          const int col = cp * 16 + cg;
          const int sx = col - 1;
          const bool ok = n < N && col < UT_COLS && sy >= 0 && sy < 32 && sx >= 0 && sx < 32;
          const long off = ok ? (((((long)n * 32 + sy) * 32) + sx) * 32 + chunk * 4) : 0;
          f32x4 v = *reinterpret_cast<const f32x4*>(small + off);
          if (!ok) v = f32x4{0.f, 0.f, 0.f, 0.f};
          tv[row * 3 + cp] = v;
        }
      }
#pragma unroll
      for (int row = 0; row < UT_ROWS; ++row)
#pragma unroll
        for (int cp = 0; cp < 3; ++cp) {
          const int col = cp * 16 + cg;
          if (col < UT_COLS)
            *reinterpret_cast<f32x4*>(st + (row * UT_COLS + col) * 32 + ((chunk ^ ((col >> 1) & 7)) << 2)) = tv[row * 3 + cp];
        }
    }
    __syncthreads();
    float acc[4][C];
#pragma unroll
    for (int c = 0; c < 4; ++c)
#pragma unroll
      for (int cb = 0; cb < C; ++cb) acc[c][cb] = 0.f;

#pragma unroll 1
    for (int q = 0; q < 8; ++q) {
      f32x4 x[3][3];
#pragma unroll
      for (int dy = 0; dy < 3; ++dy)
#pragma unroll
        for (int dx = 0; dx < 3; ++dx) {
          const int row = m + dy, col = l + dx;
          x[dy][dx] = *reinterpret_cast<const f32x4*>(st + (row * UT_COLS + col) * 32 + ((q ^ ((col >> 1) & 7)) << 2));
        }
#pragma unroll
      for (int j = 0; j < 4; ++j) {
        const int cs = q * 4 + j;
#pragma unroll
        for (int cb = 0; cb < C; ++cb) {
          const float* wp = w + (cs * C + cb) * 16;
#pragma unroll
          for (int kh = 0; kh < 4; ++kh) {
            const int py = (kh + 1) & 1;
            const int dsy = (py + 1 - kh) / 2;
#pragma unroll
            for (int kw = 0; kw < 4; ++kw) {
              const int px = (kw + 1) & 1;
              const int dsx = (px + 1 - kw) / 2;
              acc[py * 2 + px][cb] = fmaf(x[dsy + 1][dsx + 1][j], wp[kh * 4 + kw], acc[py * 2 + px][cb]);
            }
          }
        }
      }
    }
    if (n < N) {
      const int sy = sy0 + m;
#pragma unroll
      for (int cb = 0; cb < C; ++cb) {
        const float bv = bias ? bias[cb] : 0.f;
#pragma unroll
        for (int py = 0; py < 2; ++py) {
          float v0 = acc[py * 2 + 0][cb] + bv, v1 = acc[py * 2 + 1][cb] + bv;
          if (act == DVAE_ACT_SIGMOID) { v0 = 1.f / (1.f + expf(-v0)); v1 = 1.f / (1.f + expf(-v1)); }
          else if (act == DVAE_ACT_RELU) { v0 = v0 > 0.f ? v0 : 0.f; v1 = v1 > 0.f ? v1 : 0.f; }
          const long o = ((((long)n * C + cb) * 64) + 2 * sy + py) * 64 + 2 * l;
          *reinterpret_cast<float2*>(out + o) = make_float2(v0, v1);
          if (FUSE) {
            float xt0, xt1;
            if constexpr (sizeof(TT) == 4) {
              const float2 xt = *reinterpret_cast<const float2*>(target + o);
              xt0 = xt.x; xt1 = xt.y;
            } else {
              const uchar2 xt = *reinterpret_cast<const uchar2*>(target + o);
              xt0 = to_unit(xt.x); xt1 = to_unit(xt.y);
            }
            float gl0, gl1, gr;
            lsum += recon_elem(v0, xt0, dist, &gl0, &gr);
            lsum += recon_elem(v1, xt1, dist, &gl1, &gr);
            *reinterpret_cast<float2*>(g + o) = make_float2(gs * gl0, gs * gl1);
          }
        }
      }
    }
  }
  if (FUSE) {
    const float v = wave_sum(lsum);
    if ((tid & 63) == 0) redl[tid >> 6] = v;
    __syncthreads();
    if (tid == 0) partials[blockIdx.x] = redl[0] + redl[1];
    for (int k = gridDim.x + blockIdx.x * 128 + tid; k < DVAE_REC_NPART; k += gridDim.x * 128) partials[k] = 0.f;
  }
}


typedef float f32x2 __attribute__((ext_vector_type(2)));

__device__ __forceinline__ float sigmoid_hw(float v) { return sigmoid_aten(v); }

template <int C, bool FUSE, typename TT = float>
__global__ __launch_bounds__(128) void k_up_thin_pk(const float* __restrict__ small, const float* __restrict__ wrec,
                                                    const float* __restrict__ bias, float* __restrict__ out, int N,
                                                    int act, int n_units, const TT* __restrict__ target,
                                                    float* __restrict__ g, int dist, const float* __restrict__ coef,
                                                    float* __restrict__ partials) {
  constexpr int REC = C == 3 ? 48 : 16;
  constexpr int PB = C == 3 ? 32 : 0;
  constexpr int CS = C - 1;
  __shared__ __attribute__((aligned(16))) float st[UT_ROWS * UT_COLS * 32];
  __shared__ float redl[2];
  const int tid = threadIdx.x;
  const int m = tid >> 5, l = tid & 31;
  const float gs = FUSE ? coef[DVAE_C_INV_B] : 0.f;
  const bool bce_logit = FUSE && dist == DVAE_REC_BERNOULLI && act == DVAE_ACT_SIGMOID;
  float lsum = 0.f;
  const bool xmap = (gridDim.x & 63) == 0;
  const int upi = xmap ? 8 * (int)(gridDim.x >> 3) : (int)gridDim.x;
  const int unit0 = xmap ? 8 * (int)((blockIdx.x & 7) + 8 * (blockIdx.x >> 6)) + (int)((blockIdx.x >> 3) & 7) : (int)blockIdx.x;
  for (int unit = unit0; unit < n_units; unit += upi) {
    const int n = unit >> 3, sy0 = (unit & 7) * 4;
    __syncthreads();
    {
      const int chunk = tid & 7, cg = tid >> 3;
      f32x4 tv[UT_ROWS * 3];
#pragma unroll
      for (int row = 0; row < UT_ROWS; ++row) {
        const int sy = sy0 - 1 + row;
#pragma unroll
        for (int cp = 0; cp < 3; ++cp) {
          const int col = cp * 16 + cg;
          const int sx = col - 1;
          const bool ok = n < N && col < UT_COLS && sy >= 0 && sy < 32 && sx >= 0 && sx < 32;
          const long off = ok ? (((((long)n * 32 + sy) * 32) + sx) * 32 + chunk * 4) : 0;
          f32x4 v = *reinterpret_cast<const f32x4*>(small + off);
          if (!ok) v = f32x4{0.f, 0.f, 0.f, 0.f};
          tv[row * 3 + cp] = v;
        }
      }
#pragma unroll
      for (int row = 0; row < UT_ROWS; ++row)
#pragma unroll
        for (int cp = 0; cp < 3; ++cp) {
          const int col = cp * 16 + cg;
          if (col < UT_COLS)
            *reinterpret_cast<f32x4*>(st + (row * UT_COLS + col) * 32 + ((chunk ^ ((col >> 1) & 7)) << 2)) = tv[row * 3 + cp];
        }
    }
    __syncthreads();
    float2 tg[C][2];
    if (FUSE && n < N) {
#pragma unroll
      for (int cb = 0; cb < C; ++cb)
#pragma unroll
        for (int py = 0; py < 2; ++py) {
          const long o = ((((long)n * C + cb) * 64) + 2 * (sy0 + m) + py) * 64 + 2 * l;
          if constexpr (sizeof(TT) == 4) tg[cb][py] = *reinterpret_cast<const float2*>(target + o);
          else {
            const uchar2 xt = *reinterpret_cast<const uchar2*>(target + o);
            tg[cb][py] = make_float2((float)xt.x, (float)xt.y);
          }
        }
    }
    f32x2 accA[4];
    f32x2 h01 = {0.f, 0.f}, h23 = {0.f, 0.f};
    f32x2 v02 = {0.f, 0.f}, v13 = {0.f, 0.f};
    float sc[4] = {0.f, 0.f, 0.f, 0.f};
#pragma unroll
    for (int c = 0; c < 4; ++c) accA[c] = f32x2{0.f, 0.f};

#pragma unroll 1
    for (int q = 0; q < 8; ++q) {
      f32x4 x[3][3];
#pragma unroll
      for (int dy = 0; dy < 3; ++dy)
#pragma unroll
        for (int dx = 0; dx < 3; ++dx) {
          const int row = m + dy, col = l + dx;
          x[dy][dx] = *reinterpret_cast<const f32x4*>(st + (row * UT_COLS + col) * 32 + ((q ^ ((col >> 1) & 7)) << 2));
        }
#pragma unroll
      for (int j = 0; j < 4; ++j) {
        const float* wp = wrec + (q * 4 + j) * REC;
        const f32x2* wp2 = reinterpret_cast<const f32x2*>(wp);
        if (C == 3) {
#pragma unroll
          for (int t = 0; t < 4; ++t) {
            const int ty = t >> 1, tx = t & 1;
#pragma unroll
            for (int cls = 0; cls < 4; ++cls) {
              const int py = cls >> 1, px = cls & 1;
              const float xs = x[py - ty + 1][px - tx + 1][j];
              accA[cls] = __builtin_elementwise_fma(f32x2{xs, xs}, wp2[t * 4 + cls], accA[cls]);
            }
          }
        }
        const f32x2* wb2 = reinterpret_cast<const f32x2*>(wp + PB);
        const float xc = x[1][1][j], xu = x[0][1][j], xd = x[2][1][j], xl = x[1][0][j], xr = x[1][2][j];
        h01 = __builtin_elementwise_fma(f32x2{xc, xc}, wb2[0], h01);
        h23 = __builtin_elementwise_fma(f32x2{xc, xc}, wb2[1], h23);
        h01 = __builtin_elementwise_fma(f32x2{xu, xu}, wb2[2], h01);
        h23 = __builtin_elementwise_fma(f32x2{xd, xd}, wb2[3], h23);
        v02 = __builtin_elementwise_fma(f32x2{xl, xl}, wb2[4], v02);
        v13 = __builtin_elementwise_fma(f32x2{xr, xr}, wb2[5], v13);
        sc[3] = fmaf(x[2][2][j], wp[PB + 12], sc[3]);
        sc[2] = fmaf(x[2][0][j], wp[PB + 13], sc[2]);
        sc[1] = fmaf(x[0][2][j], wp[PB + 14], sc[1]);
        sc[0] = fmaf(x[0][0][j], wp[PB + 15], sc[0]);
      }
    }
    float acc[4][C];
    {
      const float hh[4] = {h01[0], h01[1], h23[0], h23[1]}, vv[4] = {v02[0], v13[0], v02[1], v13[1]};
#pragma unroll
      for (int cls = 0; cls < 4; ++cls) {
        if (C == 3) { acc[cls][0] = accA[cls][0]; acc[cls][1] = accA[cls][1]; }
        acc[cls][CS] = (hh[cls] + vv[cls]) + sc[cls];
      }
    }
    if (n < N) {
      const int sy = sy0 + m;
#pragma unroll
      for (int cb = 0; cb < C; ++cb) {
        const float bv = bias ? bias[cb] : 0.f;
#pragma unroll
        for (int py = 0; py < 2; ++py) {
          float v0 = acc[py * 2 + 0][cb] + bv, v1 = acc[py * 2 + 1][cb] + bv;
          const long o = ((((long)n * C + cb) * 64) + 2 * sy + py) * 64 + 2 * l;
          if (FUSE && bce_logit) {
            const float xt0 = raw_to_unit<TT>(tg[cb][py].x), xt1 = raw_to_unit<TT>(tg[cb][py].y);
            float p0, p1, gl0, gl1;
            lsum += sigmoid_bce_logit(v0, xt0, &p0, &gl0);
            lsum += sigmoid_bce_logit(v1, xt1, &p1, &gl1);
            *reinterpret_cast<float2*>(out + o) = make_float2(p0, p1);
            *reinterpret_cast<float2*>(g + o) = make_float2(gs * gl0, gs * gl1);
            continue;
          }
          if (act == DVAE_ACT_SIGMOID) { v0 = sigmoid_hw(v0); v1 = sigmoid_hw(v1); }
          else if (act == DVAE_ACT_RELU) { v0 = v0 > 0.f ? v0 : 0.f; v1 = v1 > 0.f ? v1 : 0.f; }
          *reinterpret_cast<float2*>(out + o) = make_float2(v0, v1);
          if (FUSE) {
            const float xt0 = raw_to_unit<TT>(tg[cb][py].x), xt1 = raw_to_unit<TT>(tg[cb][py].y);
            float gl0, gl1, gr;
            lsum += recon_elem(v0, xt0, dist, &gl0, &gr);
            lsum += recon_elem(v1, xt1, dist, &gl1, &gr);
            *reinterpret_cast<float2*>(g + o) = make_float2(gs * gl0, gs * gl1);
          }
        }
      }
    }
  }
  if (FUSE) {
    const float v = wave_sum(lsum);
    if ((tid & 63) == 0) redl[tid >> 6] = v;
    __syncthreads();
    if (tid == 0) partials[blockIdx.x] = redl[0] + redl[1];
    for (int k = gridDim.x + blockIdx.x * 128 + tid; k < DVAE_REC_NPART; k += gridDim.x * 128) partials[k] = 0.f;
  }
}

int launch_up_thin_staged(const float* small, const float* wrec, const float* bias, const void* target, int target_u8,
                          float* out, float* g, int dist, const float* coef, float* partials, int N, int C, int act,
                          hipStream_t s) {
  if (C != 1 && C != 3) return 1;
  if (C == 3 && launch_up_thin_mm(small, wrec + 32 * 48, bias, target, target_u8, out, g, dist, coef, partials, N, act, s) == 0)
    return 0;
  const int n_units = N * 8;
  const int grid = n_units < 1536 ? n_units : 1536;
#define UP_PK(CC, FF, TT_) hipLaunchKernelGGL((k_up_thin_pk<CC, FF, TT_>), dim3(grid), dim3(128), 0, s, small, wrec, bias, out, N, act, \
                                             n_units, (const TT_*)target, g, dist, coef, partials)
  if (!target) { if (C == 1) UP_PK(1, false, float); else UP_PK(3, false, float); }
  else if (target_u8) { if (C == 1) UP_PK(1, true, uint8_t); else UP_PK(3, true, uint8_t); }
  else { if (C == 1) UP_PK(1, true, float); else UP_PK(3, true, float); }
#undef UP_PK
  DVAE_CHECK_LAUNCH();
  return 0;
}


template <int C, typename TB = float>
__global__ __launch_bounds__(256) void k_wgrad_thin(const TB* __restrict__ big, const float* __restrict__ small,
                                                    float* __restrict__ ws, int N, int n_units) {
  constexpr int NT = (16 * C + 31) / 32;
  __shared__ __attribute__((aligned(16))) float bt[C * TB_PLANE];
  __shared__ __attribute__((aligned(16))) float sp[8192];
  __shared__ UnitLut lut_s[1];
  const UnitLut* lut = lut_s;
  const int tid = threadIdx.x, lane = tid & 63, wv = tid >> 6;
  const int i = lane & 31, h = lane >> 5;
  if (sizeof(TB) == 1) { lut_s[0].init(tid, 256); __syncthreads(); }
  f32x16 acc[NT];
#pragma unroll
  for (int t = 0; t < NT; ++t)
#pragma unroll
    for (int e = 0; e < 16; ++e) acc[t][e] = 0.f;
  float sumS = 0.f, sumB[NT];
  int boff[NT];
  bool bval[NT];
#pragma unroll
  for (int t = 0; t < NT; ++t) {
    sumB[t] = 0.f;
    const int nidx = t * 32 + i;
    bval[t] = nidx < 16 * C;
    const int cb = bval[t] ? (nidx >> 4) : 0, kh = (nidx >> 2) & 3, kw = nidx & 3;
    boff[t] = cb * TB_PLANE + kh * TB_ROW + (kw & 1) * TB_PAR + (kw >> 1);
  }
  BigThinRegs<C, TB> pfb;
  f32x4 pfs[4];
  auto load_unit = [&](int u) {
    const int n = u >> 3, sy0 = (u & 7) * 4;
    load_big_thin<C, TB>(pfb, big, n, sy0, true, tid);
    const float* src = small + ((((long)n * 32 + sy0) * 32)) * 32;
#pragma unroll
    for (int k = 0; k < 4; ++k) pfs[k] = *reinterpret_cast<const f32x4*>(src + (tid + k * 256) * 4);
  };
  int unit = blockIdx.x;
  if (unit < n_units) load_unit(unit);
  for (; unit < n_units; unit += gridDim.x) {
    __syncthreads();
    store_big_thin<C, TB>(pfb, bt, tid, lut);
#pragma unroll
    for (int k = 0; k < 4; ++k) *reinterpret_cast<f32x4*>(sp + (tid + k * 256) * 4) = pfs[k];
    __syncthreads();
    if (unit + (int)gridDim.x < n_units) load_unit(unit + gridDim.x);
#pragma unroll 4
    for (int t = 0; t < 16; ++t) {
      const int sx = 2 * t + h;
      const float a = sp[(wv * 32 + sx) * 32 + i];
      sumS += a;
      const int base = (2 * wv) * TB_ROW + sx;
#pragma unroll
      for (int nt = 0; nt < NT; ++nt) {
        float b = bt[base + boff[nt]];
        b = bval[nt] ? b : 0.f;
        sumB[nt] += b;
        acc[nt] = __builtin_amdgcn_mfma_f32_32x32x2f32(a, b, acc[nt], 0, 0, 0);
      }
    }
  }
  __syncthreads();
  float* red = sp;
#pragma unroll
  for (int nt = 0; nt < NT; ++nt)
#pragma unroll
    for (int e = 0; e < 16; ++e) red[((wv * NT + nt) * 16 + e) * 64 + lane] = acc[nt][e];
  __syncthreads();
  float* wsw = ws + (long)blockIdx.x * (NT * 1024 + 32 + NT * 32);
  for (int idx = tid; idx < NT * 1024; idx += 256) {
    const int nt = idx >> 10, e = (idx >> 6) & 15, ln = idx & 63;
    float v = red[((0 * NT + nt) * 16 + e) * 64 + ln] + red[((1 * NT + nt) * 16 + e) * 64 + ln] +
              red[((2 * NT + nt) * 16 + e) * 64 + ln] + red[((3 * NT + nt) * 16 + e) * 64 + ln];
    const int cs = (e & 3) + 8 * (e >> 2) + 4 * (ln >> 5);
    const int nidx = nt * 32 + (ln & 31);
    wsw[nt * 1024 + cs * 32 + (ln & 31)] = v;
    (void)nidx;
  }
  __syncthreads();
  sumS += __shfl_xor(sumS, 32, 64);
#pragma unroll
  for (int nt = 0; nt < NT; ++nt) sumB[nt] += __shfl_xor(sumB[nt], 32, 64);
  float* redb = sp;
  if (h == 0) {
    redb[(wv * (1 + NT)) * 32 + i] = sumS;
#pragma unroll
    for (int nt = 0; nt < NT; ++nt) redb[(wv * (1 + NT) + 1 + nt) * 32 + i] = sumB[nt];
  }
  __syncthreads();
  if (tid < (1 + NT) * 32) {
    float v = redb[tid] + redb[(1 + NT) * 32 + tid] + redb[2 * (1 + NT) * 32 + tid] + redb[3 * (1 + NT) * 32 + tid];
    wsw[NT * 1024 + tid] = v;
  }
}

template <int C>
__global__ __launch_bounds__(256) void k_wgrad_thin_reduce(const float* __restrict__ ws, float* __restrict__ dw,
                                                           float* __restrict__ db, int bias_from_big, int nblk) {
  wgrad_thin_reduce_body<C>(blockIdx.x, ws, dw, db, bias_from_big, nblk);
}

size_t wgrad_thin_ws_floats() { return (size_t)WT_MAX_BLOCKS * (2 * 1024 + 32 + 2 * 32); }

static bool thin_applicable(const ConvArgs& a) {
  return (a.Cb == 1 || a.Cb == 3) && a.Cs == 32 && a.Hs == 32 && a.Ws == 32;
}

int launch_down_thin(const ConvArgs& a, hipStream_t s) {
  if (!thin_applicable(a) || a.big_layout != DVAE_NCHW || a.out_layout != DVAE_NHWC) return 1;
  if (a.act != DVAE_ACT_NONE && a.act != DVAE_ACT_RELU) return 1;
  if (launch_down_thin_ws(a, s) == 0) return 0;
  const int n_units = a.N * 8;
  const int grid = n_units < 1536 ? n_units : 1536;
  if ((a.mask_bits && (a.mask || a.out_bits)) || (a.out_bits && a.mask)) return 1;
  uint32_t* bits = a.mask_bits ? const_cast<uint32_t*>(a.mask_bits) : a.out_bits;
#define DVAE_DT(C, MODE) hipLaunchKernelGGL((k_down_thin<C, MODE>), dim3(grid), dim3(256), 0, s, a.big, a.w, a.bias, a.mask, a.out, a.N, a.act, n_units, bits)
  if (a.Cb == 1) {
    if (a.mask_bits) DVAE_DT(1, 2); else if (a.out_bits) DVAE_DT(1, 3); else if (a.mask) DVAE_DT(1, 1); else DVAE_DT(1, 0);
  } else {
    if (a.mask_bits) DVAE_DT(3, 2); else if (a.out_bits) DVAE_DT(3, 3); else if (a.mask) DVAE_DT(3, 1); else DVAE_DT(3, 0);
  }
#undef DVAE_DT
  DVAE_CHECK_LAUNCH();
  return 0;
}

int launch_up_thin(const ConvArgs& a, hipStream_t s) {
  if (!thin_applicable(a) || a.small_layout != DVAE_NHWC || a.out_layout != DVAE_NCHW || a.mask) return 1;
  const int n_units = a.N * 8;
  const int grid = n_units;
  if (a.Cb == 1) hipLaunchKernelGGL((k_up_thin<1, false>), dim3(grid), dim3(128), 0, s, a.small, a.w, a.bias, a.out, a.N, a.act, n_units, (const float*)nullptr, (float*)nullptr, 0, (const float*)nullptr, (float*)nullptr);
  else hipLaunchKernelGGL((k_up_thin<3, false>), dim3(grid), dim3(128), 0, s, a.small, a.w, a.bias, a.out, a.N, a.act, n_units, (const float*)nullptr, (float*)nullptr, 0, (const float*)nullptr, (float*)nullptr);
  DVAE_CHECK_LAUNCH();
  return 0;
}

int launch_up_thin_recon(const ConvArgs& a, const float* target, float* g, int dist, const float* coef,
                         float* partials, hipStream_t s) {
  if (!thin_applicable(a) || a.small_layout != DVAE_NHWC || a.out_layout != DVAE_NCHW || a.mask) return 1;
  const int n_units = a.N * 8;
  const int grid = n_units < 1536 ? n_units : 1536;
  if (a.Cb == 1) hipLaunchKernelGGL((k_up_thin<1, true>), dim3(grid), dim3(128), 0, s, a.small, a.w, a.bias, a.out, a.N, DVAE_ACT_SIGMOID, n_units, target, g, dist, coef, partials);
  else hipLaunchKernelGGL((k_up_thin<3, true>), dim3(grid), dim3(128), 0, s, a.small, a.w, a.bias, a.out, a.N, DVAE_ACT_SIGMOID, n_units, target, g, dist, coef, partials);
  DVAE_CHECK_LAUNCH();
  return 0;
}

int launch_down_thin_u8(const uint8_t* x, const float* w, const float* bias, float* out, uint32_t* out_bits, int N, int C, int act,
                        hipStream_t s) {
  const int n_units = N * 8;
  const int grid = n_units < 1536 ? n_units : 1536;
#define DVAE_DT8(C, MODE) hipLaunchKernelGGL((k_down_thin<C, MODE, uint8_t>), dim3(grid), dim3(256), 0, s, x, w, bias, (const float*)nullptr, out, N, act, n_units, out_bits)
  if (C == 1) { if (out_bits) DVAE_DT8(1, 3); else DVAE_DT8(1, 0); }
  else if (C == 3) { if (out_bits) DVAE_DT8(3, 3); else DVAE_DT8(3, 0); }
  else return 1;
#undef DVAE_DT8
  DVAE_CHECK_LAUNCH();
  return 0;
}

int launch_up_thin_recon_u8(const ConvArgs& a, const uint8_t* target, float* g, int dist, const float* coef,
                            float* partials, hipStream_t s) {
  if (!thin_applicable(a) || a.small_layout != DVAE_NHWC || a.out_layout != DVAE_NCHW || a.mask) return 1;
  const int n_units = a.N * 8;
  const int grid = n_units < 1536 ? n_units : 1536;
  if (a.Cb == 1) hipLaunchKernelGGL((k_up_thin<1, true, uint8_t>), dim3(grid), dim3(128), 0, s, a.small, a.w, a.bias, a.out, a.N, DVAE_ACT_SIGMOID, n_units, target, g, dist, coef, partials);
  else hipLaunchKernelGGL((k_up_thin<3, true, uint8_t>), dim3(grid), dim3(128), 0, s, a.small, a.w, a.bias, a.out, a.N, DVAE_ACT_SIGMOID, n_units, target, g, dist, coef, partials);
  DVAE_CHECK_LAUNCH();
  return 0;
}

template <int C>
static int wgrad_thin_reduce(const float* ws, float* dw, float* db, int bias_from_big, int grid, hipStream_t s) {
  hipLaunchKernelGGL(k_wgrad_thin_reduce<C>, dim3(WT_REDUCE_BLOCKS(C)), dim3(256), 0, s, ws, dw, db, bias_from_big, grid);
  DVAE_CHECK_LAUNCH();
  return 0;
}
template <int C, typename TB>
static int wgrad_thin_two_pass(const TB* big, const float* small, float* dw, float* db, int bias_from_big, int N, int n_units,
                               int grid, float* ws, hipStream_t s) {
  hipLaunchKernelGGL((k_wgrad_thin<C, TB>), dim3(grid), dim3(256), 0, s, big, small, ws, N, n_units);
  DVAE_CHECK_LAUNCH();
  return wgrad_thin_reduce<C>(ws, dw, db, bias_from_big, grid, s);
}

int launch_wgrad_thin_u8(const uint8_t* x, const float* small, float* dw, float* db, int N, int C, float* ws, hipStream_t s) {
  const int n_units = N * 8;
  const int grid = n_units < WT_MAX_BLOCKS ? n_units : WT_MAX_BLOCKS;
  if (C == 1) return wgrad_thin_two_pass<1>(x, small, dw, db, 0, N, n_units, grid, ws, s);
  if (C == 3) return wgrad_thin_two_pass<3>(x, small, dw, db, 0, N, n_units, grid, ws, s);
  return 1;
}

int launch_wgrad_thin(const float* big, const float* small, float* dw, float* db, int bias_from_big, int N, int Cb,
                      int Hs, float* ws, hipStream_t s) {
  if (!(Cb == 1 || Cb == 3) || Hs != 32) return 1;
  {
    int wgrid = 0;
    if (launch_wgrad_thin_ws(big, small, ws, bias_from_big, N, Cb, &wgrid, s) == 0)
      return Cb == 1 ? wgrad_thin_reduce<1>(ws, dw, db, bias_from_big, wgrid, s) : wgrad_thin_reduce<3>(ws, dw, db, bias_from_big, wgrid, s);
  }
  const int n_units = N * 8;
  int grid = n_units < WT_MAX_BLOCKS ? n_units : WT_MAX_BLOCKS;
  {
    static const int cap = env_int("DVAE_WGRAD_THIN_GRID", WT_MAX_BLOCKS);
    if (cap > 0 && cap < grid) grid = cap;
  }
  return Cb == 1 ? wgrad_thin_two_pass<1>(big, small, dw, db, bias_from_big, N, n_units, grid, ws, s)
                 : wgrad_thin_two_pass<3>(big, small, dw, db, bias_from_big, N, n_units, grid, ws, s);
}

}
```

disentangling-vae_amd/csrc/conv_wgrad_ws.hip:

```cpp
#include "common.h"
#include "conv_mfma_common.h"
#include "wgrad_reduce.h"

namespace dvae {

#define WGW_MAX_BLOCKS WG_MAX_BLOCKS
#define WGW_STRIDE WG_STRIDE

template <int HS>
struct WGeo {
  using G = Geo<HS>;
  static constexpr int NQ = HS / 4;
  static constexpr int CWP = HS + 4;
  static constexpr int BCH = G::BROWS * 2 * CWP;
  static constexpr int SCH = 64 + 16;
  static constexpr int BT_FLOATS = 31 * BCH + 28 + BCH;
  static constexpr int ST_FLOATS = 31 * SCH + 28 + 64;
  static constexpr int STORED_ROWS = HS == 16 ? G::BROWS : G::BROWS - 2;
  static constexpr int NBIG = STORED_ROWS * 2 * NQ * 8;
  static constexpr int BUF_FLOATS = BT_FLOATS + ST_FLOATS;
  static_assert(BT_FLOATS % 4 == 0 && ST_FLOATS % 4 == 0 && NBIG % 128 == 0 && NBIG + 128 <= 768, "slot plan");
};

template <int HS>
__global__ __launch_bounds__(512) void k_wgrad32ws(const float* __restrict__ big, const float* __restrict__ small,
                                                   float* __restrict__ ws, int n_units
#ifdef DVAE_DEBUG_SWITCHES
                                                   , int abl
#endif
                                                   ) {
#ifndef DVAE_DEBUG_SWITCHES
  constexpr int abl = 0;
#endif
  using G = Geo<HS>;
  using W = WGeo<HS>;
  static_assert(G::IMGS == 1, "one image per unit");
  constexpr int HB = 2 * HS;
  extern __shared__ __attribute__((aligned(16))) float smem[];
  const int tid = threadIdx.x, lane = tid & 63;
  const int wv = __builtin_amdgcn_readfirstlane(tid >> 6);
  const bool is_compute = wv < 4;
  const int stride = gridDim.x;
  const int unit0 = blockIdx.x;

  for (int e = tid; e < 2 * W::BUF_FLOATS / 4; e += 512) reinterpret_cast<f32x4*>(smem)[e] = f32x4{0.f, 0.f, 0.f, 0.f};
  __syncthreads();

  if (is_compute) {
    const int kh = wv;
    const int i = lane & 31, h = lane >> 5;
    f32x16 acc[4];
#pragma unroll
    for (int t = 0; t < 4; ++t)
#pragma unroll
      for (int e = 0; e < 16; ++e) acc[t][e] = 0.f;
    float sumS = 0.f, sumK1 = 0.f, sumK2 = 0.f;
    const int abase = i * W::SCH + 4 * (i >> 2) + 4 * h;
    const int bbase = i * W::BCH + 4 * (i >> 2) + kh * 2 * W::CWP + 4 * h;
    __builtin_amdgcn_s_setprio(1);
    __syncthreads();
    int buf = 0;
    for (int unit = unit0; unit < n_units; unit += stride) {
      const float* bt = smem + buf * W::BUF_FLOATS;
      const float* st = bt + W::BT_FLOATS;
      constexpr int NG = 64 / 8;
      constexpr int GPR = HS / 8;
      f32x4 A[2], P0a[2], P0b[2], P1a[2], P1b[2];
      if (abl & 16) {
#pragma unroll
        for (int c = 0; c < 2; ++c) { A[c] = f32x4{1.f, 2.f, 3.f, 4.f}; P0a[c] = A[c]; P0b[c] = A[c]; P1a[c] = A[c]; P1b[c] = A[c]; }
      }
      auto rd = [&](int g, int slot) {
        if (abl & 16) return;
        const int sy = g / GPR, gx = g % GPR;
        A[slot] = *reinterpret_cast<const f32x4*>(st + abase + sy * HS + 8 * gx);
        const float* bp = bt + bbase + (4 * sy) * W::CWP + 8 * gx;
        P0a[slot] = *reinterpret_cast<const f32x4*>(bp);
        P0b[slot] = *reinterpret_cast<const f32x4*>(bp + 4);
        P1a[slot] = *reinterpret_cast<const f32x4*>(bp + W::CWP);
        P1b[slot] = *reinterpret_cast<const f32x4*>(bp + W::CWP + 4);
      };
      rd(0, 0);
      __builtin_amdgcn_sched_group_barrier(0x100, 5, 0);
      if (!(abl & 8)) {
#pragma unroll
      for (int g = 0; g < NG; ++g) {
        const int c = g & 1;
        if (g + 1 < NG) rd(g + 1, c ^ 1);
#pragma unroll
        for (int j = 0; j < 4; ++j) {
          const float a = A[c][j];
          const float b0 = j > 0 ? P0b[c][j - 1] : P0a[c][3];
          const float b1 = P1a[c][j];
          const float b2 = P0b[c][j];
          const float b3 = j < 3 ? P1a[c][j + 1] : P1b[c][0];
          acc[0] = __builtin_amdgcn_mfma_f32_32x32x2f32(a, b0, acc[0], 0, 0, 0);
          acc[1] = __builtin_amdgcn_mfma_f32_32x32x2f32(a, b1, acc[1], 0, 0, 0);
          acc[2] = __builtin_amdgcn_mfma_f32_32x32x2f32(a, b2, acc[2], 0, 0, 0);
          acc[3] = __builtin_amdgcn_mfma_f32_32x32x2f32(a, b3, acc[3], 0, 0, 0);
          sumS += a; sumK1 += b1; sumK2 += b2;
        }
        __builtin_amdgcn_sched_group_barrier(0x100, 5, 0);
        __builtin_amdgcn_sched_group_barrier(0x008, 16, 0);
      }
      }
      if (!(abl & 32)) __syncthreads();
      buf ^= 1;
    }
    float* wsw = ws + (long)blockIdx.x * WGW_STRIDE;
#pragma unroll
    for (int t = 0; t < 4; ++t) {
      const int tap = kh * 4 + t;
#pragma unroll
      for (int e = 0; e < 16; ++e) {
        const int cs = (e & 3) + 8 * (e >> 2) + 4 * h;
        wsw[(tap * 32 + cs) * 32 + i] = acc[t][e];
      }
    }
    float* wsb = wsw + 16384;
    sumS += __shfl_xor(sumS, 32, 64);
    sumK1 += __shfl_xor(sumK1, 32, 64);
    sumK2 += __shfl_xor(sumK2, 32, 64);
    if (h == 0) {
      if (kh == 0) wsb[i] = sumS;
      if (kh == 1) { wsb[32 + i] = sumK1; wsb[64 + i] = sumK2; }
      if (kh == 2) { wsb[96 + i] = sumK1; wsb[128 + i] = sumK2; }
    }
  } else {
    const int lt = tid - 256;
    const int lw = wv - 4;
    const bool k2_big = HS == 16 && lw < 2, k2_small = HS == 16 ? lw >= 2 : lw < 2;
    unsigned g_of[3];
    int l_of[2][3][4];
#pragma unroll
    for (int k = 0; k < 3; ++k) {
      const int s = lt + 256 * k;
      int l0 = 0, ch = 0;
      g_of[k] = 0;
      if (s < W::NBIG) {
        const int chunk = s & 7, q = s >> 3;
        const int q4 = q % W::NQ, par = (q / W::NQ) & 1, r = q / (2 * W::NQ) + (HS == 16 ? 0 : 1);
        g_of[k] = (unsigned)((r * HB + 8 * q4 + (1 - par)) * 32 + 4 * chunk);
        l0 = chunk * (4 * W::BCH + 4) + (r * 2 + par) * W::CWP + (par == 0 ? 4 : 0) + 4 * q4;
        ch = W::BCH;
      } else {
        const int sp = (s - W::NBIG) & 127, chunk = sp & 7, pq = sp >> 3;
        g_of[k] = (unsigned)(pq * 128 + 4 * chunk);
        l0 = W::BT_FLOATS + chunk * (4 * W::SCH + 4) + 4 * pq;
        ch = W::SCH;
      }
#pragma unroll
      for (int b_ = 0; b_ < 2; ++b_)
#pragma unroll
        for (int u = 0; u < 4; ++u) l_of[b_][k][u] = b_ * W::BUF_FLOATS + l0 + u * ch;
    }
    f32x4 pA[3][4], pB[3][4];
    constexpr unsigned UPI = HS * HS / G::U;
    const unsigned last_unit = (unsigned)(n_units - 1);
    auto load_unit = [&](int u_, f32x4 (&p)[3][4]) {
      if (abl & 2) return;
      const unsigned u = (unsigned)u_ < last_unit ? (unsigned)u_ : last_unit;
      const unsigned n0 = u / UPI, sy0 = (u % UPI) * G::R;
      const bool top = HS == 16 && sy0 == 0, bot = HS == 16 && sy0 + G::R == HS;
      const float* bg = big + ((size_t)n0 * HB + 2 * sy0) * (HB * 32) - HB * 32;
      const float* s0 = bg + ((top && lw == 0) ? HB * 32 : 0) + g_of[0];
      const float* s1 = bg + g_of[1];
      const float* s2 = (k2_big ? bg - ((bot && lw == 1) ? HB * 32 : 0) : small + (size_t)u * (G::U * 32)) + g_of[2];
#pragma unroll
      for (int t = 0; t < 4; ++t) p[0][t] = *reinterpret_cast<const f32x4*>(s0 + 64 * t);
#pragma unroll
      for (int t = 0; t < 4; ++t) p[1][t] = *reinterpret_cast<const f32x4*>(s1 + 64 * t);
      if (k2_big) {
#pragma unroll
        for (int t = 0; t < 4; ++t) p[2][t] = *reinterpret_cast<const f32x4*>(s2 + 64 * t);
      } else {
#pragma unroll
        for (int t = 0; t < 4; ++t) p[2][t] = *reinterpret_cast<const f32x4*>(s2 + 32 * t);
      }
    };
    auto store_unit = [&](int b, int u_, const f32x4 (&p)[3][4]) {
      if (abl & 1) return;
      const unsigned sy0 = ((unsigned)u_ % UPI) * G::R;
      const bool top = HS == 16 && sy0 == 0, bot = HS == 16 && sy0 + G::R == HS;
#pragma unroll
      for (int k = 0; k < 3; ++k) {
        if (k == 2 && !k2_big && !k2_small) continue;
        const bool outside = (k == 0 && lw == 0 && top) || (k == 2 && k2_big && lw == 1 && bot);
        if (outside) {
#pragma unroll
          for (int u = 0; u < 4; ++u)
#pragma unroll
            for (int t = 0; t < 4; ++t) smem[l_of[b][k][u] + t] = 0.f;
        } else {
#pragma unroll
          for (int u = 0; u < 4; ++u)
#pragma unroll
            for (int t = 0; t < 4; ++t) smem[l_of[b][k][u] + t] = p[k][t][u];
        }
      }
    };
    if (unit0 < n_units) { load_unit(unit0, pA); store_unit(0, unit0, pA); }
    load_unit(unit0 + stride, pA);
    load_unit(unit0 + 2 * stride, pB);
    __syncthreads();
    int unit = unit0;
    while (unit < n_units) {
      if (unit + stride < n_units) store_unit(1, unit + stride, pA);
      load_unit(unit + 3 * stride, pA);
      if (!(abl & 32)) __syncthreads();
      unit += stride;
      if (unit >= n_units) break;
      if (unit + stride < n_units) store_unit(0, unit + stride, pB);
      load_unit(unit + 3 * stride, pB);
      if (!(abl & 32)) __syncthreads();
      unit += stride;
    }
  }
}

template <int HS>
static int launch_wgrad_ws_t(const float* big, const float* small, float* dw, float* db, int bias_from_big, int N,
                             float* ws, hipStream_t s) {
  using W = WGeo<HS>;
  const int n_units = (int)(((long)N * HS * HS) / 64);
#ifdef WGW_FULL_GRID
  const int full = WGW_MAX_BLOCKS;
#else
  const int full = (N > 128 && N <= 320) ? 192 : WGW_MAX_BLOCKS;
#endif
  int grid = n_units < full ? n_units : full;
  {
    static const int cap = env_int("DVAE_WGRAD_GRID", WGW_MAX_BLOCKS);
    if (cap > 0 && cap < grid) grid = cap;
  }
  const size_t lds = (size_t)2 * W::BUF_FLOATS * sizeof(float);
  static DeviceOnce attr;
  if (attr.first()) { (void)hipFuncSetAttribute((const void*)k_wgrad32ws<HS>, hipFuncAttributeMaxDynamicSharedMemorySize, (int)lds); }
#ifdef DVAE_DEBUG_SWITCHES
  static const int abl = env_int("DVAE_WGWS_ABLATE", 0);
  hipLaunchKernelGGL(k_wgrad32ws<HS>, dim3(grid), dim3(512), lds, s, big, small, ws, n_units, abl);
#else
  hipLaunchKernelGGL(k_wgrad32ws<HS>, dim3(grid), dim3(512), lds, s, big, small, ws, n_units);
#endif
  DVAE_CHECK_LAUNCH();
  return launch_wgrad32_reduce(ws, dw, db, bias_from_big, grid, s, N);
}

int launch_wgrad_mfma32_ws(const float* big, const float* small, float* dw, float* db, int bias_from_big, int N, int Hs,
                           float* ws, hipStream_t s) {
  if (Hs == 16) return launch_wgrad_ws_t<16>(big, small, dw, db, bias_from_big, N, ws, s);
  if (Hs == 8) return launch_wgrad_ws_t<8>(big, small, dw, db, bias_from_big, N, ws, s);
  return 1;
}

}
```

disentangling-vae_amd/csrc/plan.hip:

```cpp
#include <string.h>
#include <type_traits>
#include <utility>
#include "common.h"

namespace dvae {

template <typename T>
static inline T plan_arg(uint64_t v) {
  if constexpr (std::is_pointer_v<T>) {
    return reinterpret_cast<T>(v);
  } else if constexpr (std::is_floating_point_v<T>) {
    float f;
    const uint32_t u = (uint32_t)v;
    memcpy(&f, &u, sizeof(f));
    return (T)f;
  } else {
    return static_cast<T>((int64_t)v);
  }
}
template <typename... A, size_t... I>
static inline int plan_invoke(int (*fn)(A...), const uint64_t* a, std::index_sequence<I...>) {
  return fn(plan_arg<A>(a[I])...);
}
template <typename... A>
static inline int plan_call(int (*fn)(A...), const uint64_t* a, int nargs) {
  static_assert(sizeof...(A) <= DVAE_PLAN_MAX_ARGS, "raise DVAE_PLAN_MAX_ARGS");
  if (nargs != (int)sizeof...(A)) return -100;
  return plan_invoke(fn, a, std::index_sequence_for<A...>{});
}

struct PlanOp {
  const char* name;
  int (*run)(const uint64_t*, int);
};
#define DVAE_OP(f) {#f, [](const uint64_t* a, int n) { return plan_call(f, a, n); }}
static const PlanOp OPS[] = {
    DVAE_OP(dvae_conv4s2_fwd), DVAE_OP(dvae_conv4s2_dgrad), DVAE_OP(dvae_conv4s2_wgrad), DVAE_OP(dvae_convT4s2_fwd),
    DVAE_OP(dvae_convT4s2_dgrad), DVAE_OP(dvae_convT4s2_wgrad), DVAE_OP(dvae_convT4s2_sigmoid_recon_fwd),
    DVAE_OP(dvae_stage_weights), DVAE_OP(dvae_convT3_fwd_staged), DVAE_OP(dvae_conv32_down), DVAE_OP(dvae_conv32_up),
    DVAE_OP(dvae_conv1_fwd_bits), DVAE_OP(dvae_conv32_up_bits), DVAE_OP(dvae_convT3_dgrad_bits),
    DVAE_OP(dvae_u8_to_f32), DVAE_OP(dvae_conv4s2_fwd_u8), DVAE_OP(dvae_conv4s2_wgrad_u8),
    DVAE_OP(dvae_convT4s2_sigmoid_recon_fwd_u8), DVAE_OP(dvae_relayout), DVAE_OP(dvae_linear_fwd), DVAE_OP(dvae_linear_dgrad),
    DVAE_OP(dvae_linear_wgrad), DVAE_OP(dvae_linear_wgrad_grouped), DVAE_OP(dvae_fc_chain_fwd), DVAE_OP(dvae_fc_chain_bwd),
    DVAE_OP(dvae_reparam_kl_fwd), DVAE_OP(dvae_kl_finish), DVAE_OP(dvae_reparam_kl_bwd), DVAE_OP(dvae_kl_normal_bwd),
    DVAE_OP(dvae_reduce_sum), DVAE_OP(dvae_recon_loss), DVAE_OP(dvae_sigmoid_bwd), DVAE_OP(dvae_btcvae_fwd),
    DVAE_OP(dvae_btcvae_bwd), DVAE_OP(dvae_permute_dims), DVAE_OP(dvae_disc_losses), DVAE_OP(dvae_latent_entropy),
    DVAE_OP(dvae_loss_pack), DVAE_OP(dvae_loss_finalize), DVAE_OP(dvae_loss_epilogue), DVAE_OP(dvae_set_coef), DVAE_OP(dvae_add),
    DVAE_OP(dvae_axpby), DVAE_OP(dvae_swap_outer),
    DVAE_OP(dvae_image_grid_u8), DVAE_OP(dvae_image_grid_shape), DVAE_OP(dvae_recon_rows_ws_floats), DVAE_OP(dvae_recon_rows), DVAE_OP(dvae_iw_loglik),
    DVAE_OP(dvae_stream_order), DVAE_OP(dvae_event_record), DVAE_OP(dvae_event_wait), DVAE_OP(dvae_comm_allreduce), DVAE_OP(dvae_comm_allgather), DVAE_OP(dvae_comm_reducescatter),
    DVAE_OP(dvae_comm_broadcast), DVAE_OP(dvae_comm_group_start), DVAE_OP(dvae_comm_group_end),
};
#undef DVAE_OP
constexpr int N_OPS = (int)(sizeof(OPS) / sizeof(OPS[0]));

}

extern "C" {

int dvae_plan_op(const char* name) {
  if (!name) return -1;
  for (int i = 0; i < dvae::N_OPS; ++i)
    if (strcmp(dvae::OPS[i].name, name) == 0) return i;
  return -1;
}

int dvae_plan_run(const dvae_plan_entry* entries, int n) {
  if (!entries || n < 0) {
    dvae::set_error("dvae_plan_run: invalid argument");
    return -1;
  }
  for (int i = 0; i < n; ++i) {
    const dvae_plan_entry& e = entries[i];
    if (e.op < 0 || e.op >= dvae::N_OPS) {
      dvae::set_error("dvae_plan_run: entry %d: unknown op %d", i, e.op);
      return -1;
    }
    const int rc = dvae::OPS[e.op].run(e.args, e.nargs);
    if (rc == -100) {
      dvae::set_error("dvae_plan_run: entry %d (%s): %d arguments recorded", i, dvae::OPS[e.op].name, e.nargs);
      return -1;
    }
    if (rc != 0) return rc;
  }
  return 0;
}

}
```

disentangling-vae_amd/csrc/wgrad_reduce.h:

```cpp
#pragma once
#include "common.h"

namespace dvae {

#define WG_MAX_BLOCKS 256
#define WG_STRIDE (16384 + 320)
#define WG_REDUCE_BLOCKS (256 + 4)
#define WT_MAX_BLOCKS 512
#define WT_REDUCE_BLOCKS(C) ((((16 * (C) + 31) / 32) * (1024 + 32) + 32) / 16)

template <bool LEAN>
__device__ __forceinline__ void wgrad32_bias_reduce(const float* __restrict__ ws, float* __restrict__ db,
                                                    int bias_from_big, int nblk, int blk) {
  __shared__ float redb[32][8];
  const int o = threadIdx.x & 7, gq = threadIdx.x >> 3;
  const int c = blk * 8 + o;
  const float* wsb = ws + 16384 + c;
  float v[8];
  if (LEAN) {
    float e = 0.f, pr = 0.f, pp = 0.f, q0 = 0.f, q1 = 0.f;
#pragma unroll
    for (int u = 0; u < 8; ++u) {
      const int g = gq + 32 * u;
      const float* q = wsb + (long)(g < nblk ? g : nblk - 1) * WG_STRIDE;
      float t;
      if (bias_from_big) t = (q[32] + q[64]) + (q[96] + q[128]);
      else t = q[0];
      if (g >= nblk) t = 0.f;
      if ((u & 1) == 0) e = t; else pr = e + t;
      if ((u & 3) == 1) pp = pr;
      if ((u & 3) == 3) { if (u == 3) q0 = pp + pr; else q1 = pp + pr; }
      __builtin_amdgcn_sched_barrier(0);
    }
    redb[gq][o] = q0 + q1;
  } else if (bias_from_big) {
    float a[8][4];
#pragma unroll
    for (int u = 0; u < 8; ++u) {
      const int g = gq + 32 * u;
      const float* q = wsb + (long)(g < nblk ? g : nblk - 1) * WG_STRIDE;
      a[u][0] = q[32]; a[u][1] = q[64]; a[u][2] = q[96]; a[u][3] = q[128];
    }
#pragma unroll
    for (int u = 0; u < 8; ++u) v[u] = (a[u][0] + a[u][1]) + (a[u][2] + a[u][3]);
  } else {
#pragma unroll
    for (int u = 0; u < 8; ++u) {
      const int g = gq + 32 * u;
      v[u] = wsb[(long)(g < nblk ? g : nblk - 1) * WG_STRIDE];
    }
  }
  if (!LEAN) {
#pragma unroll
    for (int u = 0; u < 8; ++u)
      if (gq + 32 * u >= nblk) v[u] = 0.f;
    redb[gq][o] = ((v[0] + v[1]) + (v[2] + v[3])) + ((v[4] + v[5]) + (v[6] + v[7]));
  }
  __syncthreads();
  if (threadIdx.x < 8) {
    float t = 0.f;
    if (LEAN) {
#pragma unroll 4
      for (int k = 0; k < 32; ++k) t += redb[k][o];
    } else {
#pragma unroll
      for (int k = 0; k < 32; ++k) t += redb[k][o];
    }
    db[c] = t;
  }
}

#define WGR_LEAN_MIN_IMAGES 768
template <bool LEAN>
__device__ __forceinline__ void wgrad32_reduce_body(int blk_x, const float* __restrict__ ws, float* __restrict__ dw,
                                                    float* __restrict__ db, int bias_from_big, int nblk) {
  if (blk_x >= 256) {
    if (db) wgrad32_bias_reduce<LEAN>(ws, db, bias_from_big, nblk, blk_x - 256);
    return;
  }
  __shared__ __attribute__((aligned(16))) float red[16][64];
  const int p = threadIdx.x & 15, gq = threadIdx.x >> 4;
  const float* src = ws + (blk_x * 16 + p) * 4;
  if constexpr (LEAN) {
  f32x4 pair[2];
#pragma unroll
  for (int pp = 0; pp < 2; ++pp) {
    f32x4 qa;
#pragma unroll
    for (int hq = 0; hq < 2; ++hq) {
      const int hh = 2 * pp + hq;
      f32x4 v[4];
#pragma unroll
      for (int u = 0; u < 4; ++u) {
        const int g = gq + 16 * (4 * hh + u);
        v[u] = *reinterpret_cast<const f32x4*>(src + (long)(g < nblk ? g : nblk - 1) * WG_STRIDE);
      }
#pragma unroll
      for (int u = 0; u < 4; ++u)
        if (gq + 16 * (4 * hh + u) >= nblk) v[u] = f32x4{0.f, 0.f, 0.f, 0.f};
      const f32x4 q = (v[0] + v[1]) + (v[2] + v[3]);
      if (hq == 0) qa = q; else pair[pp] = qa + q;
      __builtin_amdgcn_sched_barrier(0);
    }
  }
  *reinterpret_cast<f32x4*>(&red[gq][p * 4]) = pair[0] + pair[1];
  } else {
  f32x4 v[16];
#pragma unroll
  for (int u = 0; u < 16; ++u) {
    const int g = gq + 16 * u;
    v[u] = *reinterpret_cast<const f32x4*>(src + (long)(g < nblk ? g : nblk - 1) * WG_STRIDE);
  }
#pragma unroll
  for (int u = 0; u < 16; ++u)
    if (gq + 16 * u >= nblk) v[u] = f32x4{0.f, 0.f, 0.f, 0.f};
#pragma unroll
  for (int w = 1; w < 16; w *= 2)
#pragma unroll
    for (int u = 0; u < 16; u += 2 * w) v[u] += v[u + w];
  *reinterpret_cast<f32x4*>(&red[gq][p * 4]) = v[0];
  }
  __syncthreads();
  if (threadIdx.x < 64) {
    const int o = threadIdx.x;
    float t = 0.f;
    if (LEAN) {
#pragma unroll 4
      for (int k = 0; k < 16; ++k) t += red[k][o];
    } else {
#pragma unroll
      for (int k = 0; k < 16; ++k) t += red[k][o];
    }
    const int idx = blk_x * 64 + o;
    const int tap = idx >> 10, cs = (idx >> 5) & 31, cb = idx & 31;
    dw[(cs * 32 + cb) * 16 + tap] = t;
  }
}


template <int C>
__device__ __forceinline__ void wgrad_thin_reduce_body(int blk_x, const float* __restrict__ ws, float* __restrict__ dw,
                                                       float* __restrict__ db, int bias_from_big, int nblk) {
  constexpr int NT = (16 * C + 31) / 32;
  constexpr int STRIDE = NT * 1024 + 32 + NT * 32;
  constexpr int QB = NT * 1024;
  __shared__ __attribute__((aligned(16))) float red[64][16];
  __shared__ float red2[8][16];
  __shared__ float fin[16];
  const int p = threadIdx.x & 3, gq = threadIdx.x >> 2;
  const float* src = ws + (blk_x * 4 + p) * 4;
  f32x4 v[8];
#pragma unroll
  for (int u = 0; u < 8; ++u) {
    const int g = gq + 64 * u;
    v[u] = *reinterpret_cast<const f32x4*>(src + (long)(g < nblk ? g : nblk - 1) * STRIDE);
  }
#pragma unroll
  for (int u = 0; u < 8; ++u)
    if (gq + 64 * u >= nblk) v[u] = f32x4{0.f, 0.f, 0.f, 0.f};
#pragma unroll
  for (int w = 1; w < 8; w *= 2)
#pragma unroll
    for (int u = 0; u < 8; u += 2 * w) v[u] += v[u + w];
  *reinterpret_cast<f32x4*>(&red[gq][p * 4]) = v[0];
  __syncthreads();
  if (threadIdx.x < 128) {
    const int o = threadIdx.x & 15, part = threadIdx.x >> 4;
    float t = 0.f;
#pragma unroll
    for (int k = 0; k < 8; ++k) t += red[part * 8 + k][o];
    red2[part][o] = t;
  }
  __syncthreads();
  float t = 0.f;
  const int o = threadIdx.x & 15;
  if (threadIdx.x < 16) {
#pragma unroll
    for (int k = 0; k < 8; ++k) t += red2[k][o];
  }
  const int q0 = blk_x * 16;
  if (q0 < QB) {
    if (threadIdx.x < 16) {
      const int q = q0 + o;
      const int nt = q >> 10, cs = (q >> 5) & 31, nidx = nt * 32 + (q & 31);
      if (nidx < 16 * C) dw[cs * 16 * C + nidx] = t;
    }
    return;
  }
  if (!db) return;
  const int k = (q0 - QB) >> 4;
  if (!bias_from_big) {
    if (k < 2 && threadIdx.x < 16) db[k * 16 + o] = t;
    return;
  }
  if (k < 2 || k - 2 >= C) return;
  if (threadIdx.x < 16) fin[o] = t;
  __syncthreads();
  if (threadIdx.x == 0) db[k - 2] = (fin[5] + fin[6]) + (fin[9] + fin[10]);
}


}
```

disentangling-vae_amd/disvae_amd/_lib.py:

```python
import ctypes
import os

_HERE = os.path.dirname(os.path.abspath(__file__))
LIB_PATH = os.environ.get("DVAE_HIP_LIB", os.path.join(_HERE, "..", "lib", "libdvae_hip.so"))

NCHW, NHWC = 0, 1
ACT_NONE, ACT_RELU, ACT_LEAKY02, ACT_SIGMOID = 0, 1, 2, 3
REC = {"bernoulli": 0, "gaussian": 1, "laplace": 2}
LOSS_BETAH, LOSS_BETAB, LOSS_BTCVAE, LOSS_FACTOR = 0, 1, 2, 3
S_LOSS, S_REC, S_KL, S_KL0, S_MI, S_TC, S_DWKL, S_KLW, S_DTC, NSCAL = 0, 1, 2, 3, 19, 20, 21, 22, 23, 32
C_INV_B, C_ANNEAL, C_BETA, C_ALPHA, C_GAMMA, C_CAP, NCOEF = 0, 1, 2, 3, 4, 5, 8
REC_NPART = 2048
NPACK = 32
MAX_LATENT_DIM = 16
ROWSTATS = 32
WIDE_KL0 = 32


def wide(D):
    return D > MAX_LATENT_DIM


def rowstats_stride(D):
    return ROWSTATS if D <= MAX_LATENT_DIM else (D + 4 + 3) & ~3


def btcvae_tmp_floats(Bg, Bl, D):
    return 3 * D * Bg + (0 if D <= MAX_LATENT_DIM else Bl * Bg)


def npack(D):
    return NPACK if D <= MAX_LATENT_DIM else NPACK + D


def nscal(D):
    return NSCAL if D <= MAX_LATENT_DIM else NSCAL + D


def kl0(D):
    return S_KL0 if D <= MAX_LATENT_DIM else WIDE_KL0

_p = ctypes.c_void_p
_i = ctypes.c_int
_l = ctypes.c_long

SIGNATURES = {
    "dvae_version": [],
    "dvae_last_error": [],
    "dvae_conv4s2_fwd": [_p, _i, _p, _p, _p, _i, _i, _i, _i, _i, _i, _i, _p],
    "dvae_conv4s2_dgrad": [_p, _i, _p, _p, _p, _i, _i, _i, _i, _i, _i, _p],
    "dvae_conv4s2_wgrad": [_p, _i, _p, _i, _p, _p, _i, _i, _i, _i, _i, _p, _p],
    "dvae_convT4s2_fwd": [_p, _i, _p, _p, _p, _i, _i, _i, _i, _i, _i, _i, _p],
    "dvae_convT4s2_dgrad": [_p, _i, _p, _p, _p, _i, _i, _i, _i, _i, _i, _p],
    "dvae_convT4s2_wgrad": [_p, _i, _p, _i, _p, _p, _i, _i, _i, _i, _i, _p, _p],
    "dvae_convT4s2_sigmoid_recon_fwd": [_p, _i, _p, _p, _p, _p, _p, _i, _p, _p, _i, _i, _i, _i, _i, _p],
    "dvae_conv_wgrad_ws_floats": [],
    "dvae_stage_weights": [_p, _i, _p, _i, _p, _p, _p, _p],
    "dvae_convT3_fwd_staged": [_p, _p, _p, _p, _i, _p, _p, _i, _p, _p, _i, _i, _p],
    "dvae_conv32_down": [_p, _p, _p, _p, _p, _i, _i, _i, _i, _p],
    "dvae_conv32_up": [_p, _i, _p, _p, _p, _p, _i, _i, _i, _p],
    "dvae_conv1_fwd_bits": [_p, _i, _p, _p, _p, _p, _i, _i, _p],
    "dvae_conv32_up_bits": [_p, _p, _p, _p, _p, _p, _i, _i, _p],
    "dvae_convT3_dgrad_bits": [_p, _p, _p, _p, _i, _i, _p],
    "dvae_fc_chain_fwd": [_p, _p],
    "dvae_fc_chain_bwd": [_p, _p],
    "dvae_fc_chain_rows": [_i],
    "dvae_reparam_kl_blocks": [_i],
    "dvae_kl_finish": [_p, _i, _p, _i, _p],
    "dvae_u8_to_f32": [_p, _p, _l, _p],
    "dvae_u8_fused_supported": [_i, _i, _i],
    "dvae_conv4s2_fwd_u8": [_p, _p, _p, _p, _i, _i, _i, _i, _i, _i, _p],
    "dvae_conv4s2_wgrad_u8": [_p, _p, _p, _p, _i, _i, _i, _i, _i, _p, _p],
    "dvae_convT4s2_sigmoid_recon_fwd_u8": [_p, _p, _p, _p, _p, _p, _i, _p, _p, _i, _i, _i, _i, _i, _p],
    "dvae_relayout": [_p, _i, _p, _i, _i, _i, _i, _p],
    "dvae_linear_fwd": [_p, _p, _p, _p, _i, _i, _i, _i, _p, _p],
    "dvae_linear_dgrad": [_p, _p, _p, _i, _p, _i, _i, _i, _p, _p],
    "dvae_linear_wgrad": [_p, _p, _p, _p, _i, _i, _i, _p, _p],
    "dvae_linear_wgrad_grouped": [_p, _i, _p],
    "dvae_reparam_kl_fwd": [_p, _p, _p, _p, _p, _p, _p, _i, _i, _p],
    "dvae_reparam_kl_bwd": [_p, _p, _p, _p, _p, _p, _p, _p, _p, _p, _p, _i, _i, _p],
    "dvae_recon_loss": [_p, _p, _l, _i, _p, _p, _p, _i, _p],
    "dvae_kl_normal_bwd": [_p, _p, _p, _p, _p, _i, _i, _p],
    "dvae_reduce_sum": [_p, _l, ctypes.c_float, _p, _p],
    "dvae_sigmoid_bwd": [_p, _p, _p, _l, _p],
    "dvae_btcvae_fwd": [_p, _p, _p, _i, _i, _i, _i, _i, _p, _p, _p, _p],
    "dvae_btcvae_bwd": [_p, _p, _p, _p, _i, _i, _i, _i, _i, _p, _p, _p, _p, _p, _p, _p],
    "dvae_permute_dims": [_p, _p, _p, _i, _i, _p],
    "dvae_latent_entropy_ws_floats": [_l, _i, _i],
    "dvae_latent_entropy": [_p, _p, _p, _l, _i, _i, _p, _p, _p],
    "dvae_disc_losses": [_p, _i, _p, _p, _p, _p, _p],
    "dvae_loss_pack": [_p, _p, _i, _p, _i, _p, _p, _p],
    "dvae_loss_finalize": [_i, _p, _i, _i, _p, _p, _p],
    "dvae_loss_epilogue": [_i, _p, _p, _i, _i, _p, _i, _p, _i, _p, _p, _p, _p],
    "dvae_set_coef": [_p] + [ctypes.c_float] * 8 + [_p],
    "dvae_comm_load": [ctypes.c_char_p],
    "dvae_comm_unique_id": [_p],
    "dvae_comm_init": [_p, _p, _i, _i],
    "dvae_comm_destroy": [_p],
    "dvae_comm_world": [_p],
    "dvae_comm_rank": [_p],
    "dvae_comm_allreduce": [_p, _p, _l, _p],
    "dvae_comm_allgather": [_p, _p, _p, _l, _p],
    "dvae_comm_reducescatter": [_p, _p, _p, _l, _p],
    "dvae_comm_broadcast": [_p, _p, _l, _i, _p],
    "dvae_comm_group_start": [],
    "dvae_comm_group_end": [],
    "dvae_add": [_p, _p, _p, _l, _p],
    "dvae_adam_step": [_p, _i, ctypes.c_float, ctypes.c_double, ctypes.c_double, ctypes.c_double, ctypes.c_double,
                       ctypes.c_double, _p],
    "dvae_axpby": [_p, _p, ctypes.c_float, _p, ctypes.c_float, _l, _p],
    "dvae_swap_outer": [_p, _p, _i, _i, _l, _p],
    "dvae_image_grid_u8": [_p, _l, _i, _i, _i, _i, _i, ctypes.c_float, _i, _p, _p],
    "dvae_image_grid_shape": [_l, _i, _i, _i, _i, _i, _p, _p],
    "dvae_recon_rows_ws_floats": [_l, _i, _l, _p],
    "dvae_recon_rows": [_p, _p, _i, _l, _i, _l, _i, _p, _p, _p],
    "dvae_iw_loglik": [_p, _p, _p, _p, _p, _l, _i, _i, _i, _i, _i, _p, _p, _p, _p],
    "dvae_stream_order": [_p, _p],
    "dvae_stream_create": [_p],
    "dvae_event_record": [_i, _p],
    "dvae_event_wait": [_i, _p],
    "dvae_plan_op": [ctypes.c_char_p],
    "dvae_plan_run": [_p, _i],
}
_RESTYPE = {"dvae_last_error": ctypes.c_char_p, "dvae_conv_wgrad_ws_floats": ctypes.c_size_t,
            "dvae_latent_entropy_ws_floats": ctypes.c_size_t}


FCW_MAX = 8
KL_MAX_BLOCKS = 8192
KL_FLOATS = 16 + KL_MAX_BLOCKS * 16
FC_CHAIN_MAX_ROWS = 8 * KL_MAX_BLOCKS


def fc_chain_rows(n):
    return int(lib().dvae_fc_chain_rows(int(n)))



class ConvImageDesc(ctypes.Structure):
    _fields_ = [("w", _p), ("img_down", _p), ("img_up", _p)]


class FcImageDesc(ctypes.Structure):
    _fields_ = [("w", _p), ("img_fwd", _p), ("img_bwd", _p), ("N", _i), ("K", _i)]


class ThinImageDesc(ctypes.Structure):
    _fields_ = [("w", _p), ("img_pairs", _p), ("C", _i)]


def thin_pair_floats(C):
    return 112 if C == 3 else 16


class FcChainFwdArgs(ctypes.Structure):
    _fields_ = [(n_, _p) for n_ in ("a_flat", "w_e1", "w_e2", "w_ml", "w_d1", "w_d2", "w_d3", "b_e1", "b_e2", "b_ml",
                                    "b_d1", "b_d2", "b_d3", "eps", "h1", "h2", "ml", "mu", "logvar", "z", "kl_part",
                                    "d1", "d2", "d3")] + [(n_, _i) for n_ in ("n_enc", "n_kl", "n_dec", "D")] + \
               [(n_, _p) for n_ in ("conv_in", "conv_w", "conv_b", "convT_w", "convT_b", "convT_out")]


class FcChainBwdArgs(ctypes.Structure):
    _fields_ = [(n_, _p) for n_ in ("gd3", "w_d3", "w_d2", "w_d1", "w_ml", "w_e2", "w_e1", "d2", "d1", "h2", "h1",
                                    "a_flat", "mu", "logvar", "eps", "dz2", "dz3", "dmu_x", "dlv_x", "scal", "coef",
                                    "gd2", "gd1", "dz", "dml", "gh2", "gh1", "ga_flat")] + [("n", _i), ("D", _i)] + \
               [(n_, _p) for n_ in ("convT_gout", "convT_w", "d3", "conv_w", "conv_act", "conv_gin")]


def struct_of(cls, **kw):
    st = cls()
    for k, v in kw.items():
        setattr(st, k, v)
    return st, ctypes.addressof(st)


class AdamTensor(ctypes.Structure):
    _fields_ = [("p", _p), ("g", _p), ("m", _p), ("v", _p), ("step", _p), ("n", _l)]


class LinearWgradDesc(ctypes.Structure):
    _fields_ = [("x", _p), ("dy", _p), ("dw", _p), ("db", _p), ("M", _i), ("K", _i), ("N", _i)]


def wgrad_descs(problems):
    arr = (LinearWgradDesc * len(problems))()
    for d, (x, dy, dw, db, M, K, N) in zip(arr, problems):
        d.x, d.dy, d.dw, d.db, d.M, d.K, d.N = x, dy, dw, db, M, K, N
    return arr, ctypes.addressof(arr)


class DvaeHipError(RuntimeError):
    pass


_lib = None


def lib():
    global _lib
    if _lib is None:
        path = os.path.abspath(LIB_PATH)
        if not os.path.exists(path):
            raise DvaeHipError(
                "libdvae_hip.so not found at %s -- build it with `python disentangling-vae_amd/build.py` "
                "(there is no CPU / PyTorch fallback for the training-step kernels)" % path)
        h = ctypes.CDLL(path)
        for name, argtypes in SIGNATURES.items():
            fn = getattr(h, name)
            fn.argtypes = argtypes
            fn.restype = _RESTYPE.get(name, ctypes.c_int)
        _lib = h
    return _lib


EVENT_SLOTS = 16
_next_slot = [0]


def next_event_slot():
    s = _next_slot[0] % EVENT_SLOTS
    _next_slot[0] += 1
    return s


def new_stream(device):
    import torch
    with torch.cuda.device(device):
        h = ctypes.c_void_p()
        call("dvae_stream_create", ctypes.addressof(h))
        return torch.cuda.ExternalStream(h.value, device=device)


ALLOC_GEN = [0]


def note_alloc():
    ALLOC_GEN[0] += 1


PLAN_MAX_ARGS = 20


class PlanEntry(ctypes.Structure):
    _fields_ = [("op", _i), ("nargs", _i), ("args", ctypes.c_uint64 * PLAN_MAX_ARGS)]


_REC = None
_OPS = {}


def _pack(ctype, v):
    if v is None:
        return 0
    if ctype is ctypes.c_float:
        return ctypes.c_uint32.from_buffer_copy(ctypes.c_float(v)).value
    if ctype not in (_p, _i, _l):
        raise DvaeHipError("arguments of type %s cannot be recorded in a launch plan" % getattr(ctype, "__name__", ctype))
    if isinstance(v, (bytes, float)):
        raise DvaeHipError("%s argument for a %s parameter cannot be recorded" % (type(v).__name__, ctype.__name__))
    return int(v) & 0xFFFFFFFFFFFFFFFF


TRACE = None


def call(name, *args):
    h = lib()
    fn = getattr(h, name)
    if TRACE is not None and name in TRACE["names"] and _REC is None:
        import torch
        st = torch.cuda.ExternalStream(args[-1]) if args[-1] else torch.cuda.current_stream()
        e0, e1 = torch.cuda.Event(enable_timing=True), torch.cuda.Event(enable_timing=True)
        e0.record(st)
        rc = fn(*args)
        e1.record(st)
        TRACE["out"].append((name, args, e0, e1))
        if rc != 0:
            raise DvaeHipError("%s failed (%d): %s" % (name, rc, h.dvae_last_error().decode()))
        return
    if _REC is not None:
        op = _OPS.get(name)
        if op is None:
            op = _OPS[name] = h.dvae_plan_op(name.encode())
        if len(args) != len(fn.argtypes):
            raise DvaeHipError("%s takes %d arguments, got %d" % (name, len(fn.argtypes), len(args)))
        if op >= 0 and len(args) <= PLAN_MAX_ARGS:
            _REC.append(("c", op, tuple(_pack(t, a) for t, a in zip(fn.argtypes, args)), name))
        else:
            _REC.append(("f", fn, tuple(None if a is None else t(a) for t, a in zip(fn.argtypes, args)), name))
    rc = fn(*args)
    if rc != 0:
        raise DvaeHipError("%s failed (%d): %s" % (name, rc, h.dvae_last_error().decode()))


def record_py(fn, *args):
    if _REC is not None:
        _REC.append(("p", fn, args, None))
    return fn(*args)


def record_on_stream(fn, *args):
    if _REC is not None:
        import torch
        st = torch.cuda.current_stream()

        def run():
            with torch.cuda.stream(st):
                fn(*args)
        _REC.append(("p", run, (), None))
    return fn(*args)


def begin_record():
    global _REC
    _REC = []


def end_record():
    global _REC
    rec, _REC = _REC, None
    plan, run = [], []

    def flush():
        if run:
            arr = (PlanEntry * len(run))()
            for e, (_, op, words, _) in zip(arr, run):
                e.op, e.nargs = op, len(words)
                for i, w in enumerate(words):
                    e.args[i] = w
            plan.append(("c", arr, len(run), tuple(r[3] for r in run)))
            del run[:]

    for ent in rec:
        if ent[0] == "c":
            run.append(ent)
        else:
            flush()
            plan.append(ent)
    flush()
    return plan


def replay(plan):
    h = lib()
    for seg in plan:
        kind = seg[0]
        if kind == "c":
            rc = h.dvae_plan_run(ctypes.addressof(seg[1]), seg[2])
            if rc != 0:
                raise DvaeHipError("replay of %d recorded launches failed (%d): %s" % (seg[2], rc, h.dvae_last_error().decode()))
        elif kind == "f":
            rc = seg[1](*seg[2])
            if rc != 0:
                raise DvaeHipError("%s failed (%d): %s" % (seg[3], rc, h.dvae_last_error().decode()))
        else:
            seg[1](*seg[2])


def ptr(t):
    return None if t is None else t.data_ptr()
```

Baseline: 988,600 images/s.

## Defer weight-gradient reductions into the next wgrad kernel's prologue within plans

Weight-gradient kernels can now skip launching their separate cross-block reduction kernel. Instead they record a pending reduction, and the next carry-capable wgrad kernel in the recorded plan performs it in a prologue using its own LDS and threads. Anything else flushes the pending reduction with a standalone launch. The point is to cut kernel launches and tail gaps in the backward pass. In exchange, a double-buffered workspace is needed so consecutive layers do not clobber each other's partials, and the fused kernels carry extra prologue work and register pressure.

Result: no change. 998,300 images/s (median of 6 runs) (+1.0%).

```diff
diff --git a/disentangling-vae_amd/csrc/capi.hip b/disentangling-vae_amd/csrc/capi.hip
--- a/disentangling-vae_amd/csrc/capi.hip
+++ b/disentangling-vae_amd/csrc/capi.hip
@@ -36,16 +36,19 @@
   }
   return launch_up_generic(a, s);
 }
-static int run_wgrad(const float* big, int big_layout, const float* small, int small_layout, float* dw, float* db,
-                     int bias_from_big, int N, int Cb, int Cs, int Hs, int Ws, float* ws, hipStream_t s) {
+int run_wgrad(const float* big, int big_layout, const float* small, int small_layout, float* dw, float* db, int bias_from_big,
+              int N, int Cb, int Cs, int Hs, int Ws, float* ws, hipStream_t s, const WgradPending* carry, WgradPending* defer) {
   if (!use_generic_only() && ws != nullptr && Hs == Ws && Cs == 32 && Cb == 32 && big_layout == DVAE_NHWC && Hs == 4 &&
       small_layout == DVAE_NCHW)
-    return launch_wgrad_mfma32(big, small, dw, db, bias_from_big, N, Hs, ws, s, 1);
+    return launch_wgrad_mfma32(big, small, dw, db, bias_from_big, N, Hs, ws, s, 1, carry, defer);
   if (!use_generic_only() && ws != nullptr && Hs == Ws && Cs == 32 && small_layout == DVAE_NHWC) {
     if (Cb == 32 && big_layout == DVAE_NHWC && (Hs == 4 || Hs == 8 || Hs == 16))
-      return launch_wgrad_mfma32(big, small, dw, db, bias_from_big, N, Hs, ws, s, 0);
+      return launch_wgrad_mfma32(big, small, dw, db, bias_from_big, N, Hs, ws, s, 0, carry, defer);
+  }
+  if (carry && carry->c.fmt != WG_CARRY_NONE && launch_wgrad_flush(*carry, s) != 0) return -2;
+  if (!use_generic_only() && ws != nullptr && Hs == Ws && Cs == 32 && small_layout == DVAE_NHWC) {
     if ((Cb == 1 || Cb == 3) && Hs == 32 && big_layout == DVAE_NCHW)
-      return launch_wgrad_thin(big, small, dw, db, bias_from_big, N, Cb, Hs, ws, s);
+      return launch_wgrad_thin(big, small, dw, db, bias_from_big, N, Cb, Hs, ws, s, defer);
   }
   return launch_wgrad_generic(big, big_layout, small, small_layout, dw, db, bias_from_big, N, Cb, Cs, Hs, Ws, ws,
                               dvae_conv_wgrad_ws_floats(), s);
diff --git a/disentangling-vae_amd/csrc/common.h b/disentangling-vae_amd/csrc/common.h
--- a/disentangling-vae_amd/csrc/common.h
+++ b/disentangling-vae_amd/csrc/common.h
@@ -5,6 +5,7 @@
 #include <stdlib.h>
 #include <string.h>
 #include "../../include/dvae_hip.h"
+#include "plan_carry.h"
 #include "wave_spec.h"
 
 namespace dvae {
@@ -142,11 +143,18 @@
 int launch_up_mfma32(const ConvArgs& a, hipStream_t s);
 int launch_down_mfma32_dma(const ConvArgs& a, hipStream_t s);
 int launch_wgrad_mfma32_ws(const float* big, const float* small, float* dw, float* db, int bias_from_big, int N, int Hs,
-                           float* ws, hipStream_t s);
+                           float* ws, hipStream_t s, const WgradCarry& carry,
+                           WgradPending* defer);
 int launch_wgrad32_reduce(const float* ws, float* dw, float* db, int bias_from_big, int nblk, hipStream_t s, int N);
 int launch_up_mfma32_ws(const ConvArgs& a, hipStream_t s);
 int launch_wgrad_mfma32(const float* big, const float* small, float* dw, float* db, int bias_from_big,
-                        int N, int Hs, float* ws, hipStream_t s, int small_nchw = 0);
+                        int N, int Hs, float* ws, hipStream_t s, int small_nchw = 0, const WgradPending* carry = nullptr,
+                        WgradPending* defer = nullptr);
+int launch_wgrad_flush(const WgradPending& p, hipStream_t s);
+int launch_wgrad_thin_reduce(const float* ws, float* dw, float* db, int bias_from_big, int nblk, int C, hipStream_t s);
+int run_wgrad(const float* big, int big_layout, const float* small, int small_layout, float* dw, float* db,
+              int bias_from_big, int N, int Cb, int Cs, int Hs, int Ws, float* ws, hipStream_t s,
+              const WgradPending* carry = nullptr, WgradPending* defer = nullptr);
 int launch_down_thin(const ConvArgs& a, hipStream_t s);
 int launch_down_thin_ws(const ConvArgs& a, hipStream_t s);
 int launch_up_thin(const ConvArgs& a, hipStream_t s);
@@ -155,7 +163,7 @@
 int launch_wgrad_thin_ws(const float* big, const float* small, float* ws, int bias_from_big, int N, int Cb, int* grid_out,
                          hipStream_t s);
 int launch_wgrad_thin(const float* big, const float* small, float* dw, float* db, int bias_from_big,
-                      int N, int Cb, int Hs, float* ws, hipStream_t s);
+                      int N, int Cb, int Hs, float* ws, hipStream_t s, WgradPending* defer = nullptr);
 int launch_down_thin_u8(const uint8_t* x, const float* w, const float* bias, float* out, uint32_t* out_bits, int N, int C, int act,
                         hipStream_t s);
 int launch_up_thin_recon_u8(const ConvArgs& a, const uint8_t* target, float* g, int dist, const float* coef,
diff --git a/disentangling-vae_amd/csrc/conv_mfma.hip b/disentangling-vae_amd/csrc/conv_mfma.hip
--- a/disentangling-vae_amd/csrc/conv_mfma.hip
+++ b/disentangling-vae_amd/csrc/conv_mfma.hip
@@ -223,7 +223,7 @@
 
 template <int HS>
 __global__ __launch_bounds__(512) void k_wgrad32(const float* __restrict__ big, const float* __restrict__ small,
-                                                 float* __restrict__ ws, int N, int n_units, int small_nchw) {
+                                                 float* __restrict__ ws, int N, int n_units, int small_nchw, WgradCarry carry) {
   using G = Geo<HS>;
   extern __shared__ __attribute__((aligned(16))) float smem[];
   float* bt = smem;
@@ -232,10 +232,10 @@
   const int kh = wv >> 1, kwb = wv & 1;
   const int i = lane & 31, h = lane >> 5;
 
+  wgrad_carry_prologue(carry, smem);
   SlotDesc<G::BIG_NPF> sd;
   init_big_slots<HS>(sd, tid);
-  f32x4 pf[G::BIG_NPF];
-  f32x4 pfs;
+  f32x4 pf[G::BIG_NPF], pfs;
   f32x16 acc0, acc1, acc2, acc3;
 #pragma unroll
   for (int e = 0; e < 16; ++e) { acc0[e] = 0.f; acc1[e] = 0.f; acc2[e] = 0.f; acc3[e] = 0.f; }
@@ -321,9 +321,9 @@
 }
 
 template <bool LEAN>
-__global__ __launch_bounds__(256) void k_wgrad32_reduce(const float* __restrict__ ws, float* __restrict__ dw,
-                                                        float* __restrict__ db, int bias_from_big, int nblk) {
-  wgrad32_reduce_body<LEAN>(blockIdx.x, ws, dw, db, bias_from_big, nblk);
+__global__ __launch_bounds__(256) void k_wgrad32_reduce(const float* __restrict__ ws, float* __restrict__ dw, float* __restrict__ db, int bias_from_big, int nblk) {
+  __shared__ __attribute__((aligned(16))) float lds[WG_CARRY_LDS_FLOATS];
+  wgrad32_reduce_body<LEAN>(blockIdx.x, true, threadIdx.x, lds, ws, dw, db, bias_from_big, nblk);
 }
 
 size_t wgrad32_ws_floats() { return (size_t)WG_MAX_BLOCKS * WG_STRIDE; }
@@ -377,7 +377,7 @@
 
 template <int HS>
 static int launch_wgrad_t(const float* big, const float* small, float* dw, float* db, int bias_from_big, int N,
-                          float* ws, hipStream_t s, int small_nchw) {
+                          float* ws, hipStream_t s, int small_nchw, const WgradCarry& carry, WgradPending* defer) {
   using G = Geo<HS>;
   const int n_units = units_for(N, HS);
   int grid = n_units < WG_MAX_BLOCKS ? n_units : WG_MAX_BLOCKS;
@@ -388,8 +388,10 @@
   const size_t lds = (G::BIG_FLOATS + 64 * 32) * sizeof(float);
   static DeviceOnce attr;
   if (attr.first()) { (void)hipFuncSetAttribute((const void*)k_wgrad32<HS>, hipFuncAttributeMaxDynamicSharedMemorySize, (int)lds); }
-  hipLaunchKernelGGL(k_wgrad32<HS>, dim3(grid), dim3(512), lds, s, big, small, ws, N, n_units, small_nchw);
+  hipLaunchKernelGGL(k_wgrad32<HS>, dim3(grid), dim3(512), lds, s, big, small, ws, N, n_units, small_nchw, carry);
   DVAE_CHECK_LAUNCH();
+  static_assert(G::BIG_FLOATS + 64 * 32 >= 2 * WG_CARRY_LDS_FLOATS, "the carried reduction's scratch fits the tiles' LDS");
+  if (wgrad_defer(defer, ws, dw, db, bias_from_big, grid, WG_CARRY_32, N)) return 0;
   return launch_wgrad32_reduce(ws, dw, db, bias_from_big, grid, s, N);
 }
 
@@ -418,16 +420,24 @@
 }
 
 int launch_wgrad_mfma32(const float* big, const float* small, float* dw, float* db, int bias_from_big, int N,
-                        int Hs, float* ws, hipStream_t s, int small_nchw) {
+                        int Hs, float* ws, hipStream_t s, int small_nchw, const WgradPending* carry, WgradPending* defer) {
   static const bool no_ws = env_off("DVAE_WGRAD_WS");
+  const WgradCarry c = carry ? carry->c : WgradCarry{nullptr, nullptr, nullptr, 0, 0, WG_CARRY_NONE, 0};
   if (!no_ws && !small_nchw && (Hs == 16 || Hs == 8))
-    return launch_wgrad_mfma32_ws(big, small, dw, db, bias_from_big, N, Hs, ws, s);
+    return launch_wgrad_mfma32_ws(big, small, dw, db, bias_from_big, N, Hs, ws, s, c, defer);
   switch (Hs) {
-    case 16: return launch_wgrad_t<16>(big, small, dw, db, bias_from_big, N, ws, s, small_nchw);
-    case 8: return launch_wgrad_t<8>(big, small, dw, db, bias_from_big, N, ws, s, small_nchw);
-    case 4: return launch_wgrad_t<4>(big, small, dw, db, bias_from_big, N, ws, s, small_nchw);
+    case 16: return launch_wgrad_t<16>(big, small, dw, db, bias_from_big, N, ws, s, small_nchw, c, defer);
+    case 8: return launch_wgrad_t<8>(big, small, dw, db, bias_from_big, N, ws, s, small_nchw, c, defer);
+    case 4: return launch_wgrad_t<4>(big, small, dw, db, bias_from_big, N, ws, s, small_nchw, c, defer);
     default: return 1;
   }
 }
 
-}
+int launch_wgrad_flush(const WgradPending& p, hipStream_t s) {
+  const WgradCarry& c = p.c;
+  if (c.fmt == WG_CARRY_32) return launch_wgrad32_reduce(c.ws, c.dw, c.db, c.bias_from_big, c.nblk, s, p.images);
+  if (c.fmt == WG_CARRY_THIN1 || c.fmt == WG_CARRY_THIN3) return launch_wgrad_thin_reduce(c.ws, c.dw, c.db, c.bias_from_big, c.nblk, c.fmt == WG_CARRY_THIN1 ? 1 : 3, s);
+  return 0;
+}
+
+}
diff --git a/disentangling-vae_amd/csrc/conv_thin.hip b/disentangling-vae_amd/csrc/conv_thin.hip
--- a/disentangling-vae_amd/csrc/conv_thin.hip
+++ b/disentangling-vae_amd/csrc/conv_thin.hip
@@ -555,9 +555,9 @@
 }
 
 template <int C>
-__global__ __launch_bounds__(256) void k_wgrad_thin_reduce(const float* __restrict__ ws, float* __restrict__ dw,
-                                                           float* __restrict__ db, int bias_from_big, int nblk) {
-  wgrad_thin_reduce_body<C>(blockIdx.x, ws, dw, db, bias_from_big, nblk);
+__global__ __launch_bounds__(256) void k_wgrad_thin_reduce(const float* __restrict__ ws, float* __restrict__ dw, float* __restrict__ db, int bias_from_big, int nblk) {
+  __shared__ __attribute__((aligned(16))) float lds[WG_CARRY_LDS_FLOATS];
+  wgrad_thin_reduce_body<C>(blockIdx.x, true, threadIdx.x, lds, ws, dw, db, bias_from_big, nblk);
 }
 
 size_t wgrad_thin_ws_floats() { return (size_t)WT_MAX_BLOCKS * (2 * 1024 + 32 + 2 * 32); }
@@ -653,12 +653,12 @@
 }
 
 int launch_wgrad_thin(const float* big, const float* small, float* dw, float* db, int bias_from_big, int N, int Cb,
-                      int Hs, float* ws, hipStream_t s) {
+                      int Hs, float* ws, hipStream_t s, WgradPending* defer) {
   if (!(Cb == 1 || Cb == 3) || Hs != 32) return 1;
   {
     int wgrid = 0;
     if (launch_wgrad_thin_ws(big, small, ws, bias_from_big, N, Cb, &wgrid, s) == 0)
-      return Cb == 1 ? wgrad_thin_reduce<1>(ws, dw, db, bias_from_big, wgrid, s) : wgrad_thin_reduce<3>(ws, dw, db, bias_from_big, wgrid, s);
+      return wgrad_defer(defer, ws, dw, db, bias_from_big, wgrid, Cb == 1 ? WG_CARRY_THIN1 : WG_CARRY_THIN3, N) ? 0 : launch_wgrad_thin_reduce(ws, dw, db, bias_from_big, wgrid, Cb, s);
   }
   const int n_units = N * 8;
   int grid = n_units < WT_MAX_BLOCKS ? n_units : WT_MAX_BLOCKS;
@@ -666,8 +666,18 @@
     static const int cap = env_int("DVAE_WGRAD_THIN_GRID", WT_MAX_BLOCKS);
     if (cap > 0 && cap < grid) grid = cap;
   }
-  return Cb == 1 ? wgrad_thin_two_pass<1>(big, small, dw, db, bias_from_big, N, n_units, grid, ws, s)
-                 : wgrad_thin_two_pass<3>(big, small, dw, db, bias_from_big, N, n_units, grid, ws, s);
-}
-
-}
+  if (!defer)
+    return Cb == 1 ? wgrad_thin_two_pass<1>(big, small, dw, db, bias_from_big, N, n_units, grid, ws, s)
+                   : wgrad_thin_two_pass<3>(big, small, dw, db, bias_from_big, N, n_units, grid, ws, s);
+  if (Cb == 1) hipLaunchKernelGGL((k_wgrad_thin<1, float>), dim3(grid), dim3(256), 0, s, big, small, ws, N, n_units);
+  else hipLaunchKernelGGL((k_wgrad_thin<3, float>), dim3(grid), dim3(256), 0, s, big, small, ws, N, n_units);
+  DVAE_CHECK_LAUNCH();
+  wgrad_defer(defer, ws, dw, db, bias_from_big, grid, Cb == 1 ? WG_CARRY_THIN1 : WG_CARRY_THIN3, N);
+  return 0;
+}
+
+int launch_wgrad_thin_reduce(const float* ws, float* dw, float* db, int bias_from_big, int nblk, int C, hipStream_t s) {
+  return C == 1 ? wgrad_thin_reduce<1>(ws, dw, db, bias_from_big, nblk, s) : wgrad_thin_reduce<3>(ws, dw, db, bias_from_big, nblk, s);
+}
+
+}
diff --git a/disentangling-vae_amd/csrc/conv_wgrad_ws.hip b/disentangling-vae_amd/csrc/conv_wgrad_ws.hip
--- a/disentangling-vae_amd/csrc/conv_wgrad_ws.hip
+++ b/disentangling-vae_amd/csrc/conv_wgrad_ws.hip
@@ -24,7 +24,7 @@
 
 template <int HS>
 __global__ __launch_bounds__(512) void k_wgrad32ws(const float* __restrict__ big, const float* __restrict__ small,
-                                                   float* __restrict__ ws, int n_units
+                                                   float* __restrict__ ws, int n_units, WgradCarry carry
 #ifdef DVAE_DEBUG_SWITCHES
                                                    , int abl
 #endif
@@ -40,9 +40,9 @@
   const int tid = threadIdx.x, lane = tid & 63;
   const int wv = __builtin_amdgcn_readfirstlane(tid >> 6);
   const bool is_compute = wv < 4;
-  const int stride = gridDim.x;
-  const int unit0 = blockIdx.x;
-
+  const int stride = gridDim.x, unit0 = blockIdx.x;
+
+  wgrad_carry_prologue(carry, smem);
   for (int e = tid; e < 2 * W::BUF_FLOATS / 4; e += 512) reinterpret_cast<f32x4*>(smem)[e] = f32x4{0.f, 0.f, 0.f, 0.f};
   __syncthreads();
 
@@ -220,7 +220,7 @@
 
 template <int HS>
 static int launch_wgrad_ws_t(const float* big, const float* small, float* dw, float* db, int bias_from_big, int N,
-                             float* ws, hipStream_t s) {
+                             float* ws, hipStream_t s, const WgradCarry& carry, WgradPending* defer) {
   using W = WGeo<HS>;
   const int n_units = (int)(((long)N * HS * HS) / 64);
 #ifdef WGW_FULL_GRID
@@ -238,18 +238,20 @@
   if (attr.first()) { (void)hipFuncSetAttribute((const void*)k_wgrad32ws<HS>, hipFuncAttributeMaxDynamicSharedMemorySize, (int)lds); }
 #ifdef DVAE_DEBUG_SWITCHES
   static const int abl = env_int("DVAE_WGWS_ABLATE", 0);
-  hipLaunchKernelGGL(k_wgrad32ws<HS>, dim3(grid), dim3(512), lds, s, big, small, ws, n_units, abl);
+  hipLaunchKernelGGL(k_wgrad32ws<HS>, dim3(grid), dim3(512), lds, s, big, small, ws, n_units, carry, abl);
 #else
-  hipLaunchKernelGGL(k_wgrad32ws<HS>, dim3(grid), dim3(512), lds, s, big, small, ws, n_units);
+  hipLaunchKernelGGL(k_wgrad32ws<HS>, dim3(grid), dim3(512), lds, s, big, small, ws, n_units, carry);
 #endif
   DVAE_CHECK_LAUNCH();
+  static_assert(2 * W::BUF_FLOATS >= 2 * WG_CARRY_LDS_FLOATS, "the carried reduction's scratch fits the tiles' LDS");
+  if (wgrad_defer(defer, ws, dw, db, bias_from_big, grid, WG_CARRY_32, N)) return 0;
   return launch_wgrad32_reduce(ws, dw, db, bias_from_big, grid, s, N);
 }
 
 int launch_wgrad_mfma32_ws(const float* big, const float* small, float* dw, float* db, int bias_from_big, int N, int Hs,
-                           float* ws, hipStream_t s) {
-  if (Hs == 16) return launch_wgrad_ws_t<16>(big, small, dw, db, bias_from_big, N, ws, s);
-  if (Hs == 8) return launch_wgrad_ws_t<8>(big, small, dw, db, bias_from_big, N, ws, s);
+                           float* ws, hipStream_t s, const WgradCarry& carry, WgradPending* defer) {
+  if (Hs == 16) return launch_wgrad_ws_t<16>(big, small, dw, db, bias_from_big, N, ws, s, carry, defer);
+  if (Hs == 8) return launch_wgrad_ws_t<8>(big, small, dw, db, bias_from_big, N, ws, s, carry, defer);
   return 1;
 }
 
diff --git a/disentangling-vae_amd/csrc/plan.hip b/disentangling-vae_amd/csrc/plan.hip
--- a/disentangling-vae_amd/csrc/plan.hip
+++ b/disentangling-vae_amd/csrc/plan.hip
@@ -1,7 +1,11 @@
+#include <stdlib.h>
 #include <string.h>
+#include <atomic>
+#include <mutex>
 #include <type_traits>
 #include <utility>
 #include "common.h"
+#include "../../include/dvae_plan_carry.h"
 
 namespace dvae {
 
@@ -54,6 +58,116 @@
 #undef DVAE_OP
 constexpr int N_OPS = (int)(sizeof(OPS) / sizeof(OPS[0]));
 
+static bool carry_enabled() {
+  static const bool on = [] {
+    const char* e = getenv("DVAE_PLAN_CARRY");
+    return !(e && e[0] == '0' && e[1] == 0) && !use_generic_only();
+  }();
+  return on;
+}
+static const carry::Kind* op_kinds() {
+  static const carry::Kind* kinds = [] {
+    static carry::Kind k[N_OPS];
+    for (int i = 0; i < N_OPS; ++i) k[i] = carry::op_kind(OPS[i].name);
+    return k;
+  }();
+  return kinds;
+}
+static std::atomic<int> g_carried{0}, g_flushed{0};
+
+struct Half1 { int dev; uint64_t s; float* buf; };
+constexpr int MAX_HALF1 = 32;
+static Half1 g_half1[MAX_HALF1];
+static int g_n_half1 = 0;
+static std::mutex g_half1_mu;
+
+static int register_half1(uint64_t s, float* buf, size_t floats) {
+  int dev = 0;
+  if (hipGetDevice(&dev) != hipSuccess) { (void)hipGetLastError(); set_error("dvae_plan_carry_workspace: no current device"); return -2; }
+  if (buf && (floats < dvae_conv_wgrad_ws_floats() || ((uintptr_t)buf & 15))) {
+    set_error("dvae_plan_carry_workspace: %zu floats given, dvae_conv_wgrad_ws_floats() = %zu 16-byte aligned floats needed", floats,
+              dvae_conv_wgrad_ws_floats());
+    return -1;
+  }
+  std::lock_guard<std::mutex> lock(g_half1_mu);
+  for (int i = 0; i < g_n_half1; ++i)
+    if (g_half1[i].dev == dev && g_half1[i].s == s) {
+      if (buf) g_half1[i].buf = buf;
+      else g_half1[i] = g_half1[--g_n_half1];
+      return 0;
+    }
+  if (!buf) return 0;
+  if (g_n_half1 == MAX_HALF1) {
+    set_error("dvae_plan_carry_workspace: %d streams are registered already", MAX_HALF1);
+    return -1;
+  }
+  g_half1[g_n_half1++] = Half1{dev, s, buf};
+  return 0;
+}
+
+static int run_planned_wgrad(carry::Kind k, const dvae_plan_entry& e, const WgradPending* in, WgradPending* defer, float* half1) {
+  using namespace carry;
+  const float* x = plan_arg<const float*>(e.args[A_X]);
+  const float* dy = plan_arg<const float*>(e.args[A_DY]);
+  float* dw = plan_arg<float*>(e.args[A_DW]);
+  float* db = plan_arg<float*>(e.args[A_DB]);
+  const int xl = plan_arg<int>(e.args[A_XL]), dyl = plan_arg<int>(e.args[A_DYL]), N = plan_arg<int>(e.args[A_N]);
+  const int Cin = plan_arg<int>(e.args[A_CIN]), H = plan_arg<int>(e.args[A_H]), W = plan_arg<int>(e.args[A_W]);
+  const int Cout = plan_arg<int>(e.args[A_COUT]);
+  hipStream_t s = plan_arg<hipStream_t>(e.args[A_STREAM]);
+  float* ws = half1 ? half1 : plan_arg<float*>(e.args[A_WS]);
+  if (k == OP_CONV_WGRAD) return run_wgrad(x, xl, dy, dyl, dw, db, 0, N, Cin, Cout, H / 2, W / 2, ws, s, in, defer);
+  return run_wgrad(dy, dyl, x, xl, dw, db, 1, N, Cout, Cin, H, W, ws, s, in, defer);
+}
+
+static int run_carried(const dvae_plan_entry* entries, int n) {
+  constexpr int MAX_N = 256;
+  if (n > MAX_N || n < 2) return -100;
+  uint64_t streams[MAX_HALF1];
+  float* bufs[MAX_HALF1];
+  int n_half1 = 0;
+  {
+    int dev = 0;
+    if (hipGetDevice(&dev) != hipSuccess) { (void)hipGetLastError(); return -100; }
+    std::lock_guard<std::mutex> lock(g_half1_mu);
+    for (int i = 0; i < g_n_half1; ++i)
+      if (g_half1[i].dev == dev) { streams[n_half1] = g_half1[i].s; bufs[n_half1++] = g_half1[i].buf; }
+  }
+  const carry::Kind* kinds = op_kinds();
+  carry::Action act[MAX_N];
+  carry::Stats st;
+  if (!carry::plan(entries, n, kinds, N_OPS, carry::default_limits(), streams, n_half1, act, &st)) return -100;
+  if (st.carried == 0) {
+    g_flushed += st.flushed;
+    return -100;
+  }
+  WgradPending pend[MAX_N];
+  for (int i = 0; i < n; ++i) {
+    const dvae_plan_entry& e = entries[i];
+    int rc;
+    if (act[i].carried < 0 && act[i].carrier < 0) {
+      rc = OPS[e.op].run(e.args, e.nargs);
+      if (rc == -100) {
+        set_error("dvae_plan_run: entry %d (%s): %d arguments recorded", i, OPS[e.op].name, e.nargs);
+        return -1;
+      }
+    } else {
+      const WgradPending* in = act[i].carried >= 0 ? &pend[act[i].carried] : nullptr;
+      WgradPending* defer = act[i].carrier >= 0 ? &pend[i] : nullptr;
+      float* half1 = nullptr;
+      if (act[i].half != 0)
+        for (int k = 0; k < n_half1; ++k)
+          if (streams[k] == e.args[carry::A_STREAM]) half1 = bufs[k];
+      if (defer) *defer = WgradPending{WgradCarry{nullptr, nullptr, nullptr, 0, 0, WG_CARRY_NONE, 0}, 0};
+      rc = run_planned_wgrad(kinds[e.op], e, in, defer, half1);
+    }
+    if (rc != 0) return rc;
+  }
+  g_carried += st.carried;
+  g_flushed += st.flushed;
+  return 0;
+}
+
 }
 
 extern "C" {
@@ -70,6 +184,10 @@
     dvae::set_error("dvae_plan_run: invalid argument");
     return -1;
   }
+  if (dvae::carry_enabled()) {
+    const int rc = dvae::run_carried(entries, n);
+    if (rc != -100) return rc;
+  }
   for (int i = 0; i < n; ++i) {
     const dvae_plan_entry& e = entries[i];
     if (e.op < 0 || e.op >= dvae::N_OPS) {
@@ -86,4 +204,15 @@
   return 0;
 }
 
-}
+int dvae_plan_carry_workspace(void* stream, float* buf, size_t floats) {
+  return dvae::register_half1((uint64_t)(uintptr_t)stream, buf, floats);
+}
+
+int dvae_plan_carry_stats(int* carried, int* flushed) {
+  const int c = dvae::g_carried.exchange(0), f = dvae::g_flushed.exchange(0);
+  if (carried) *carried = c;
+  if (flushed) *flushed = f;
+  return 0;
+}
+
+}
diff --git a/disentangling-vae_amd/csrc/plan_carry.h b/disentangling-vae_amd/csrc/plan_carry.h
--- /dev/null
+++ b/disentangling-vae_amd/csrc/plan_carry.h
@@ -0,0 +1,159 @@
+#pragma once
+#include <stdint.h>
+#include <string.h>
+#include "../../include/dvae_hip.h"
+
+namespace dvae {
+
+enum { WG_CARRY_NONE = 0, WG_CARRY_32 = 1, WG_CARRY_THIN1 = 2, WG_CARRY_THIN3 = 3 };
+
+struct WgradCarry {
+  const float* ws;
+  float* dw;
+  float* db;
+  int bias_from_big, nblk, fmt, slices;
+};
+struct WgradPending {
+  WgradCarry c;
+  int images;
+};
+
+namespace carry {
+
+enum Kind : uint8_t {
+  OP_UNKNOWN = 0,
+  OP_PLAIN,
+  OP_CONV_WGRAD,
+  OP_CONVT_WGRAD,
+  OP_FCW_GROUPED,
+  OP_ORDER,
+  OP_EVENT_RECORD,
+  OP_EVENT_WAIT,
+};
+
+static inline Kind op_kind(const char* name) {
+  static const char* const plain[] = {
+      "dvae_conv4s2_fwd", "dvae_conv4s2_dgrad", "dvae_convT4s2_fwd", "dvae_convT4s2_dgrad", "dvae_convT4s2_sigmoid_recon_fwd",
+      "dvae_stage_weights", "dvae_convT3_fwd_staged", "dvae_conv32_down", "dvae_conv32_up", "dvae_conv1_fwd_bits",
+      "dvae_conv32_up_bits", "dvae_convT3_dgrad_bits", "dvae_u8_to_f32", "dvae_conv4s2_fwd_u8", "dvae_conv4s2_wgrad_u8",
+      "dvae_convT4s2_sigmoid_recon_fwd_u8", "dvae_relayout", "dvae_linear_fwd", "dvae_linear_dgrad", "dvae_linear_wgrad",
+      "dvae_fc_chain_fwd", "dvae_fc_chain_bwd", "dvae_reparam_kl_fwd", "dvae_kl_finish", "dvae_reparam_kl_bwd",
+      "dvae_kl_normal_bwd", "dvae_reduce_sum", "dvae_recon_loss", "dvae_sigmoid_bwd", "dvae_btcvae_fwd", "dvae_btcvae_bwd",
+      "dvae_permute_dims", "dvae_disc_losses", "dvae_latent_entropy", "dvae_loss_pack", "dvae_loss_finalize",
+      "dvae_loss_epilogue", "dvae_set_coef", "dvae_add", "dvae_axpby", "dvae_swap_outer", "dvae_image_grid_u8",
+      "dvae_recon_rows", "dvae_iw_loglik",
+      "dvae_comm_allreduce", "dvae_comm_allgather", "dvae_comm_reducescatter", "dvae_comm_broadcast"};
+  if (!name) return OP_UNKNOWN;
+  if (!strcmp(name, "dvae_conv4s2_wgrad")) return OP_CONV_WGRAD;
+  if (!strcmp(name, "dvae_convT4s2_wgrad")) return OP_CONVT_WGRAD;
+  if (!strcmp(name, "dvae_linear_wgrad_grouped")) return OP_FCW_GROUPED;
+  if (!strcmp(name, "dvae_stream_order")) return OP_ORDER;
+  if (!strcmp(name, "dvae_event_record")) return OP_EVENT_RECORD;
+  if (!strcmp(name, "dvae_event_wait")) return OP_EVENT_WAIT;
+  for (const char* p : plain)
+    if (!strcmp(name, p)) return OP_PLAIN;
+  return OP_UNKNOWN;
+}
+
+struct WgradClass {
+  int fmt, carrier, grid, images;
+};
+
+static inline WgradClass classify_wgrad(int Cb, int Cs, int Hs, int Ws, int big_layout, int small_layout, long N, bool has_ws) {
+  WgradClass c = {WG_CARRY_NONE, 0, 0, (int)N};
+  if (!has_ws || N <= 0 || N > (1 << 24) || Hs != Ws || Cs != 32) return c;
+  const bool nchw4 = Cb == 32 && big_layout == DVAE_NHWC && Hs == 4 && small_layout == DVAE_NCHW;
+  if (!nchw4 && small_layout != DVAE_NHWC) return c;
+  if (Cb == 32 && big_layout == DVAE_NHWC && (Hs == 4 || Hs == 8 || Hs == 16)) {
+    c.fmt = WG_CARRY_32;
+    c.carrier = 1;
+    const long units = (N * Hs * Hs + 63) / 64;
+    const long full = (Hs != 4 && N > 128 && N <= 320) ? 192 : 256;
+    c.grid = (int)(units < full ? units : full);
+    return c;
+  }
+  if (!nchw4 && (Cb == 1 || Cb == 3) && Hs == 32 && big_layout == DVAE_NCHW) c.fmt = Cb == 1 ? WG_CARRY_THIN1 : WG_CARRY_THIN3;
+  return c;
+}
+
+enum { A_X = 0, A_XL = 1, A_DY = 2, A_DYL = 3, A_DW = 4, A_DB = 5, A_N = 6, A_CIN = 7, A_H = 8, A_W = 9, A_COUT = 10, A_WS = 11, A_STREAM = 12, WGRAD_NARGS = 13 };
+
+static inline WgradClass classify_entry(Kind k, const dvae_plan_entry& e) {
+  const WgradClass none = {WG_CARRY_NONE, 0, 0, 0};
+  if ((k != OP_CONV_WGRAD && k != OP_CONVT_WGRAD) || e.nargs != WGRAD_NARGS) return none;
+  const int xl = (int)(int64_t)e.args[A_XL], dyl = (int)(int64_t)e.args[A_DYL], Cin = (int)(int64_t)e.args[A_CIN];
+  const int H = (int)(int64_t)e.args[A_H], W = (int)(int64_t)e.args[A_W], Cout = (int)(int64_t)e.args[A_COUT];
+  const long N = (long)(int)(int64_t)e.args[A_N];
+  if (!e.args[A_X] || !e.args[A_DY] || !e.args[A_DW] || H <= 0 || W <= 0) return none;
+  if (k == OP_CONV_WGRAD) {
+    if ((H | W) & 1) return none;
+    return classify_wgrad(Cin, Cout, H / 2, W / 2, xl, dyl, N, e.args[A_WS] != 0);
+  }
+  return classify_wgrad(Cout, Cin, H, W, dyl, xl, N, e.args[A_WS] != 0);
+}
+
+struct Limits {
+  int min_grid;
+};
+static inline Limits default_limits() { return Limits{128}; }
+
+struct Action {
+  int carried;
+  int carrier;
+  uint8_t half;
+  uint8_t fmt;
+};
+
+struct Stats {
+  int carried, flushed;
+};
+
+static inline bool plan(const dvae_plan_entry* e, int n, const Kind* op_kinds, int n_ops, const Limits& lim,
+                        const uint64_t* half1, int n_half1, Action* actions, Stats* stats) {
+  Stats st = {0, 0};
+  for (int i = 0; i < n; ++i) {
+    actions[i] = Action{-1, -1, 0, WG_CARRY_NONE};
+    if (e[i].op < 0 || e[i].op >= n_ops) return false;
+  }
+  for (int i = 0; i < n; ++i) {
+    const Kind k = op_kinds[e[i].op];
+    const WgradClass c = classify_entry(k, e[i]);
+    if (c.fmt == WG_CARRY_NONE) continue;
+    actions[i].fmt = (uint8_t)c.fmt;
+    const uint64_t s = e[i].args[A_STREAM];
+    int next = -1;
+    for (int j = i + 1; j < n && next < 0; ++j) {
+      const Kind kj = op_kinds[e[j].op];
+      const dvae_plan_entry& ej = e[j];
+      bool touches = false;
+      switch (kj) {
+        case OP_UNKNOWN: touches = true; break;
+        case OP_ORDER: touches = ej.nargs != 2 || ej.args[0] == s; break;
+        case OP_EVENT_WAIT: touches = ej.nargs != 2; break;
+        case OP_FCW_GROUPED: touches = ej.nargs != 3; break;
+        default: touches = ej.nargs < 1 || ej.args[ej.nargs - 1] == s; break;
+      }
+      if (touches) next = j;
+    }
+    bool take = false, has_half1 = false;
+    for (int k2 = 0; k2 < n_half1; ++k2) has_half1 = has_half1 || half1[k2] == s;
+    if (next >= 0 && has_half1) {
+      const Kind kn = op_kinds[e[next].op];
+      const WgradClass cn = classify_entry(kn, e[next]);
+      take = cn.carrier && e[next].args[A_STREAM] == s && cn.grid >= lim.min_grid;
+    }
+    if (take) {
+      actions[i].carrier = next;
+      actions[next].carried = i;
+      actions[next].half = actions[i].half ^ 1;
+      ++st.carried;
+    } else {
+      ++st.flushed;
+    }
+  }
+  if (stats) *stats = st;
+  return true;
+}
+
+}
+}
diff --git a/disentangling-vae_amd/csrc/wgrad_reduce.h b/disentangling-vae_amd/csrc/wgrad_reduce.h
--- a/disentangling-vae_amd/csrc/wgrad_reduce.h
+++ b/disentangling-vae_amd/csrc/wgrad_reduce.h
@@ -1,5 +1,6 @@
 #pragma once
 #include "common.h"
+#include "plan_carry.h"
 
 namespace dvae {
 
@@ -9,11 +10,13 @@
 #define WT_MAX_BLOCKS 512
 #define WT_REDUCE_BLOCKS(C) ((((16 * (C) + 31) / 32) * (1024 + 32) + 32) / 16)
 
-template <bool LEAN>
-__device__ __forceinline__ void wgrad32_bias_reduce(const float* __restrict__ ws, float* __restrict__ db,
-                                                    int bias_from_big, int nblk, int blk) {
-  __shared__ float redb[32][8];
-  const int o = threadIdx.x & 7, gq = threadIdx.x >> 3;
+#define WG_CARRY_LDS_FLOATS 1280
+
+template <bool LEAN>
+__device__ __forceinline__ void wgrad32_bias_partial(const float* __restrict__ ws, int bias_from_big, int nblk, int blk, int tl,
+                                                     float* __restrict__ lds) {
+  float (*redb)[8] = reinterpret_cast<float (*)[8]>(lds);
+  const int o = tl & 7, gq = tl >> 3;
   const int c = blk * 8 + o;
   const float* wsb = ws + 16384 + c;
   float v[8];
@@ -56,8 +59,12 @@
       if (gq + 32 * u >= nblk) v[u] = 0.f;
     redb[gq][o] = ((v[0] + v[1]) + (v[2] + v[3])) + ((v[4] + v[5]) + (v[6] + v[7]));
   }
-  __syncthreads();
-  if (threadIdx.x < 8) {
+}
+template <bool LEAN>
+__device__ __forceinline__ void wgrad32_bias_final(float* __restrict__ db, int blk, int tl, const float* __restrict__ lds) {
+  const float (*redb)[8] = reinterpret_cast<const float (*)[8]>(lds);
+  const int o = tl & 7, c = blk * 8 + o;
+  if (tl < 8) {
     float t = 0.f;
     if (LEAN) {
 #pragma unroll 4
@@ -72,14 +79,10 @@
 
 #define WGR_LEAN_MIN_IMAGES 768
 template <bool LEAN>
-__device__ __forceinline__ void wgrad32_reduce_body(int blk_x, const float* __restrict__ ws, float* __restrict__ dw,
-                                                    float* __restrict__ db, int bias_from_big, int nblk) {
-  if (blk_x >= 256) {
-    if (db) wgrad32_bias_reduce<LEAN>(ws, db, bias_from_big, nblk, blk_x - 256);
-    return;
-  }
-  __shared__ __attribute__((aligned(16))) float red[16][64];
-  const int p = threadIdx.x & 15, gq = threadIdx.x >> 4;
+__device__ __forceinline__ void wgrad32_weight_partial(int blk_x, const float* __restrict__ ws, int nblk, int tl,
+                                                       float* __restrict__ lds) {
+  float (*red)[64] = reinterpret_cast<float (*)[64]>(lds);
+  const int p = tl & 15, gq = tl >> 4;
   const float* src = ws + (blk_x * 16 + p) * 4;
   if constexpr (LEAN) {
   f32x4 pair[2];
@@ -98,7 +101,8 @@
 #pragma unroll
       for (int u = 0; u < 4; ++u)
         if (gq + 16 * (4 * hh + u) >= nblk) v[u] = f32x4{0.f, 0.f, 0.f, 0.f};
-      const f32x4 q = (v[0] + v[1]) + (v[2] + v[3]);
+      f32x4 q = (v[0] + v[1]) + (v[2] + v[3]);
+      asm volatile("" : "+v"(q));
       if (hq == 0) qa = q; else pair[pp] = qa + q;
       __builtin_amdgcn_sched_barrier(0);
     }
@@ -120,9 +124,12 @@
     for (int u = 0; u < 16; u += 2 * w) v[u] += v[u + w];
   *reinterpret_cast<f32x4*>(&red[gq][p * 4]) = v[0];
   }
-  __syncthreads();
-  if (threadIdx.x < 64) {
-    const int o = threadIdx.x;
+}
+template <bool LEAN>
+__device__ __forceinline__ void wgrad32_weight_final(int blk_x, float* __restrict__ dw, int tl, const float* __restrict__ lds) {
+  const float (*red)[64] = reinterpret_cast<const float (*)[64]>(lds);
+  if (tl < 64) {
+    const int o = tl;
     float t = 0.f;
     if (LEAN) {
 #pragma unroll 4
@@ -136,36 +143,53 @@
     dw[(cs * 32 + cb) * 16 + tap] = t;
   }
 }
+template <bool LEAN>
+__device__ __forceinline__ void wgrad32_reduce_body(int blk_x, bool active, int tl, float* __restrict__ lds,
+                                                    const float* __restrict__ ws, float* __restrict__ dw,
+                                                    float* __restrict__ db, int bias_from_big, int nblk) {
+  static_assert((WG_REDUCE_BLOCKS - 4) % 2 == 0, "a pair of slices lies on one side of the weight / bias border");
+  if (blk_x >= WG_REDUCE_BLOCKS - 4) {
+    if (active && db) wgrad32_bias_partial<LEAN>(ws, bias_from_big, nblk, blk_x - 256, tl, lds);
+    __syncthreads();
+    if (active && db) wgrad32_bias_final<LEAN>(db, blk_x - 256, tl, lds);
+    return;
+  }
+  if (active) wgrad32_weight_partial<LEAN>(blk_x, ws, nblk, tl, lds);
+  __syncthreads();
+  if (active) wgrad32_weight_final<LEAN>(blk_x, dw, tl, lds);
+}
 
 
 template <int C>
-__device__ __forceinline__ void wgrad_thin_reduce_body(int blk_x, const float* __restrict__ ws, float* __restrict__ dw,
+__device__ __forceinline__ void wgrad_thin_reduce_body(int blk_x, bool active, int tl, float* __restrict__ lds,
+                                                       const float* __restrict__ ws, float* __restrict__ dw,
                                                        float* __restrict__ db, int bias_from_big, int nblk) {
   constexpr int NT = (16 * C + 31) / 32;
   constexpr int STRIDE = NT * 1024 + 32 + NT * 32;
   constexpr int QB = NT * 1024;
-  __shared__ __attribute__((aligned(16))) float red[64][16];
-  __shared__ float red2[8][16];
-  __shared__ float fin[16];
-  const int p = threadIdx.x & 3, gq = threadIdx.x >> 2;
-  const float* src = ws + (blk_x * 4 + p) * 4;
-  f32x4 v[8];
-#pragma unroll
-  for (int u = 0; u < 8; ++u) {
-    const int g = gq + 64 * u;
-    v[u] = *reinterpret_cast<const f32x4*>(src + (long)(g < nblk ? g : nblk - 1) * STRIDE);
-  }
-#pragma unroll
-  for (int u = 0; u < 8; ++u)
-    if (gq + 64 * u >= nblk) v[u] = f32x4{0.f, 0.f, 0.f, 0.f};
-#pragma unroll
-  for (int w = 1; w < 8; w *= 2)
-#pragma unroll
-    for (int u = 0; u < 8; u += 2 * w) v[u] += v[u + w];
-  *reinterpret_cast<f32x4*>(&red[gq][p * 4]) = v[0];
+  float (*red)[16] = reinterpret_cast<float (*)[16]>(lds);
+  float (*red2)[16] = reinterpret_cast<float (*)[16]>(lds + 1024);
+  const int p = tl & 3, gq = tl >> 2;
+  if (active) {
+    const float* src = ws + (blk_x * 4 + p) * 4;
+    f32x4 v[8];
+#pragma unroll
+    for (int u = 0; u < 8; ++u) {
+      const int g = gq + 64 * u;
+      v[u] = *reinterpret_cast<const f32x4*>(src + (long)(g < nblk ? g : nblk - 1) * STRIDE);
+    }
+#pragma unroll
+    for (int u = 0; u < 8; ++u)
+      if (gq + 64 * u >= nblk) v[u] = f32x4{0.f, 0.f, 0.f, 0.f};
+#pragma unroll
+    for (int w = 1; w < 8; w *= 2)
+#pragma unroll
+      for (int u = 0; u < 8; u += 2 * w) v[u] += v[u + w];
+    *reinterpret_cast<f32x4*>(&red[gq][p * 4]) = v[0];
+  }
   __syncthreads();
-  if (threadIdx.x < 128) {
-    const int o = threadIdx.x & 15, part = threadIdx.x >> 4;
+  if (active && tl < 128) {
+    const int o = tl & 15, part = tl >> 4;
     float t = 0.f;
 #pragma unroll
     for (int k = 0; k < 8; ++k) t += red[part * 8 + k][o];
@@ -173,14 +197,16 @@
   }
   __syncthreads();
   float t = 0.f;
-  const int o = threadIdx.x & 15;
-  if (threadIdx.x < 16) {
+  const int o = tl & 15;
+  if (active && tl < 16) {
 #pragma unroll
     for (int k = 0; k < 8; ++k) t += red2[k][o];
   }
+  const float f5 = __shfl(t, 5, 64), f6 = __shfl(t, 6, 64), f9 = __shfl(t, 9, 64), f10 = __shfl(t, 10, 64);
+  if (!active) return;
   const int q0 = blk_x * 16;
   if (q0 < QB) {
-    if (threadIdx.x < 16) {
+    if (tl < 16) {
       const int q = q0 + o;
       const int nt = q >> 10, cs = (q >> 5) & 31, nidx = nt * 32 + (q & 31);
       if (nidx < 16 * C) dw[cs * 16 * C + nidx] = t;
@@ -190,14 +216,40 @@
   if (!db) return;
   const int k = (q0 - QB) >> 4;
   if (!bias_from_big) {
-    if (k < 2 && threadIdx.x < 16) db[k * 16 + o] = t;
+    if (k < 2 && tl < 16) db[k * 16 + o] = t;
     return;
   }
   if (k < 2 || k - 2 >= C) return;
-  if (threadIdx.x < 16) fin[o] = t;
-  __syncthreads();
-  if (threadIdx.x == 0) db[k - 2] = (fin[5] + fin[6]) + (fin[9] + fin[10]);
-}
-
-
-}
+  if (tl == 0) db[k - 2] = (f5 + f6) + (f9 + f10);
+}
+
+__device__ __forceinline__ void wgrad_carry_prologue(const WgradCarry& c, float* __restrict__ lds) {
+  if (c.fmt == WG_CARRY_NONE) return;
+  const int half = threadIdx.x >> 8, tl = threadIdx.x & 255;
+  float* l = lds + half * WG_CARRY_LDS_FLOATS;
+  auto slices = [&](auto body) {
+    for (int base = 2 * blockIdx.x; base < c.slices; base += 2 * gridDim.x) {
+      body(base + half, base + half < c.slices);
+      __syncthreads();
+    }
+  };
+  if (c.fmt == WG_CARRY_32)
+    slices([&](int sl, bool on) { wgrad32_reduce_body<false>(sl, on, tl, l, c.ws, c.dw, c.db, c.bias_from_big, c.nblk); });
+  else if (c.fmt == WG_CARRY_THIN1)
+    slices([&](int sl, bool on) { wgrad_thin_reduce_body<1>(sl, on, tl, l, c.ws, c.dw, c.db, c.bias_from_big, c.nblk); });
+  else
+    slices([&](int sl, bool on) { wgrad_thin_reduce_body<3>(sl, on, tl, l, c.ws, c.dw, c.db, c.bias_from_big, c.nblk); });
+}
+
+static inline int wgrad_carry_slices(int fmt) {
+  return fmt == WG_CARRY_32 ? WG_REDUCE_BLOCKS : fmt == WG_CARRY_THIN1 ? WT_REDUCE_BLOCKS(1) : fmt == WG_CARRY_THIN3 ? WT_REDUCE_BLOCKS(3) : 0;
+}
+static inline bool wgrad_defer(WgradPending* defer, const float* ws, float* dw, float* db, int bias_from_big, int nblk, int fmt,
+                               int images) {
+  if (!defer) return false;
+  *defer = WgradPending{WgradCarry{ws, dw, db, bias_from_big, nblk, fmt, wgrad_carry_slices(fmt)}, images};
+  return true;
+}
+
+
+}
diff --git a/disentangling-vae_amd/disvae_amd/_lib.py b/disentangling-vae_amd/disvae_amd/_lib.py
--- a/disentangling-vae_amd/disvae_amd/_lib.py
+++ b/disentangling-vae_amd/disvae_amd/_lib.py
@@ -213,6 +213,38 @@
     return _lib
 
 
+def _carry_fn(name, argtypes):
+    fn = getattr(lib(), name)
+    fn.argtypes, fn.restype = argtypes, ctypes.c_int
+    return fn
+
+
+def plan_carry_stats():
+    c, f = ctypes.c_int(0), ctypes.c_int(0)
+    _carry_fn("dvae_plan_carry_stats", [_p, _p])(ctypes.addressof(c), ctypes.addressof(f))
+    return c.value, f.value
+
+
+_CARRY_WS = {}
+
+
+def plan_carry_workspace(stream):
+    import torch
+    key = (torch.cuda.current_device(), int(stream or 0))
+    ws = _CARRY_WS.get(key)
+    if ws is None:
+        h = lib()
+        ws = torch.empty(h.dvae_conv_wgrad_ws_floats(), dtype=torch.float32, device=torch.device("cuda", key[0]))
+        rc = _carry_fn("dvae_plan_carry_workspace", [_p, _p, ctypes.c_size_t])(key[1] or None, ws.data_ptr(), ws.numel())
+        if rc != 0:
+            raise DvaeHipError("dvae_plan_carry_workspace failed (%d): %s" % (rc, h.dvae_last_error().decode()))
+        _CARRY_WS[key] = ws
+    return ws
+
+
+_CARRY_OPS = ("dvae_conv4s2_wgrad", "dvae_convT4s2_wgrad")
+
+
 EVENT_SLOTS = 16
 _next_slot = [0]
 
@@ -329,6 +361,9 @@
                 for i, w in enumerate(words):
                     e.args[i] = w
             plan.append(("c", arr, len(run), tuple(r[3] for r in run)))
+            for _, _, words, name in run:
+                if name in _CARRY_OPS:
+                    plan_carry_workspace(words[-1])
             del run[:]
 
     for ent in rec:
diff --git a/include/dvae_plan_carry.h b/include/dvae_plan_carry.h
--- /dev/null
+++ b/include/dvae_plan_carry.h
@@ -0,0 +1,18 @@
+#ifndef DVAE_PLAN_CARRY_H
+#define DVAE_PLAN_CARRY_H
+
+#include <stddef.h>
+
+#ifdef __cplusplus
+extern "C" {
+#endif
+
+int dvae_plan_carry_workspace(void* stream, float* buf, size_t floats);
+
+int dvae_plan_carry_stats(int* carried, int* flushed);
+
+#ifdef __cplusplus
+}
+#endif
+
+#endif
```
